# Quantco/tabmat

Measured on AMD Instinct MI355X. Metric: SplitMatrix.sandwich GFLOP/s + effective HBM GB/s, 10M×1k mixed, higher is better.
Workload: dtype f64; 1 GPU; SplitMatrix.sandwich: dense128 + csr512@5% + cats(256,96,32), 10000000 rows/GPU, p=1024, float64 (BASELINE configs[3]); rows_per_gpu=10000000, p=1024, launch=eager, collective=none

## Files before the change

include/tabmat_hip.h:

```cpp
#ifndef TABMAT_HIP_H
#define TABMAT_HIP_H

#include <stddef.h>
#include <stdint.h>

#ifdef __cplusplus
extern "C" {
#endif

#define TM_OK 0
#define TM_EINVAL (-1)
#define TM_ENOMEM (-2)
#define TM_EUNSUPPORTED (-3)

int tm_version(void);
const char *tm_last_error(void);
int tm_device_count(int *count);
int tm_set_device(int device);
int tm_device_info(char *name, int name_len, int *compute_units, int64_t *hbm_bytes);
int tm_malloc(void **ptr, size_t bytes);
int tm_free(void *ptr);
int tm_memcpy_h2d(void *dst, const void *h_src, size_t bytes, void *stream);
int tm_memcpy_d2h(void *h_dst, const void *src, size_t bytes, void *stream);
int tm_memset(void *dst, int value, size_t bytes, void *stream);
// ... 433 lines not shown
                                          int64_t n_sel, int64_t m, const double *d_sel, double *out,
                                          void *stream);
int tm_multi_cat_sparse_sandwich_rows_u8_f32(const void *const *h_codes, const int64_t *h_ncols,
                                             const int32_t *h_drop_first, int n_cats,
                                             const float *cm_data, const uint8_t *cm_col8,
                                             const int32_t *row_ranges, const int32_t *rows,
                                             int64_t n_sel, int64_t m, const float *d_sel, float *out,
                                             void *stream);
int tm_multi_cat_sparse_sandwich_rows_u8_f64(const void *const *h_codes, const int64_t *h_ncols,
                                             const int32_t *h_drop_first, int n_cats,
                                             const double *cm_data, const uint8_t *cm_col8,
                                             const int32_t *row_ranges, const int32_t *rows,
                                             int64_t n_sel, int64_t m, const double *d_sel, double *out,
                                             void *stream);
int tm_multi_cat_sparse_sandwich_ent_f32(const void *const *h_codes, const int64_t *h_ncols,
                                         const int32_t *h_drop_first, int n_cats, int64_t n, const float *d,
                                         const float *vals, const uint16_t *meta, const uint32_t *bstart,
                                         int64_t n_slots, int64_t mk, float *out, void *stream);
int tm_multi_cat_sparse_sandwich_ent_f64(const void *const *h_codes, const int64_t *h_ncols,
                                         const int32_t *h_drop_first, int n_cats, int64_t n, const double *d,
                                         const double *vals, const uint16_t *meta, const uint32_t *bstart,
                                         int64_t n_slots, int64_t mk, double *out, void *stream);
int tm_multi_cat_pack_codes(const void *const *h_codes, const int64_t *h_ncols, const int32_t *h_drop_first, int n_cats,
                            int64_t n, uint32_t *packed, void *stream);
int tm_multi_cat_sparse_sandwich_entp_f32(const void *const *h_codes, const int64_t *h_ncols,
                                          const int32_t *h_drop_first, int n_cats, int64_t n, const float *d,
                                          const float *vals, const uint16_t *meta, const uint32_t *bstart,
                                          int64_t n_slots, int64_t mk, const uint32_t *packed, float *out, void *stream);
int tm_multi_cat_sparse_sandwich_entp_f64(const void *const *h_codes, const int64_t *h_ncols,
                                          const int32_t *h_drop_first, int n_cats, int64_t n, const double *d,
                                          const double *vals, const uint16_t *meta, const uint32_t *bstart,
                                          int64_t n_slots, int64_t mk, const uint32_t *packed, double *out, void *stream);

int tm_multi_cat_sparse_sandwich_slab_f32(const void *const *h_codes, const int64_t *h_ncols,
                                          const int32_t *h_drop_first, int n_cats, int64_t n,
                                          const float *d, const float *vals, const uint32_t *koff,
                                          const uint8_t *ecol, const int64_t *gptr, int64_t m,
                                          float *out, void *stream);
int tm_multi_cat_sparse_sandwich_slab_f64(const void *const *h_codes, const int64_t *h_ncols,
                                          const int32_t *h_drop_first, int n_cats, int64_t n,
                                          const double *d, const double *vals, const uint32_t *koff,
                                          const uint8_t *ecol, const int64_t *gptr, int64_t m,
                                          double *out, void *stream);

int tm_multi_cat_pairs_max_bins(void);
int tm_multi_cat_pairs_max_slots(void);
int tm_multi_cat_pairs_row_words(void);
int tm_multi_cat_pairs_f32(const int64_t *cat_tab, int64_t n, const float *d, const int32_t *rows,
                           int64_t n_rows, const int32_t *bundles, int n_bundles,
                           const int32_t *wg_map, int n_wg, int slots, int64_t bins,
                           const int64_t *desc, int64_t n_pairs, const int64_t *pos, double *tables,
                           double *out, int64_t p, void *stream);
int tm_multi_cat_pairs_f64(const int64_t *cat_tab, int64_t n, const double *d, const int32_t *rows,
                           int64_t n_rows, const int32_t *bundles, int n_bundles,
                           const int32_t *wg_map, int n_wg, int slots, int64_t bins,
                           const int64_t *desc, int64_t n_pairs, const int64_t *pos, double *tables,
                           double *out, int64_t p, void *stream);

int tm_multi_cat_matvec_f32(const int64_t *cat_tab, int n_cats, const int64_t *pos, const float *v,
                            int64_t n, float *out, void *stream);
int tm_multi_cat_matvec_f64(const int64_t *cat_tab, int n_cats, const int64_t *pos, const double *v,
                            int64_t n, double *out, void *stream);

int tm_csr_densify_cols_f32(const float *data, const int32_t *indices, const int64_t *indptr, int64_t n,
                            const int32_t *colmap, float *T, int64_t ld, void *stream);
int tm_csr_densify_cols_f64(const double *data, const int32_t *indices, const int64_t *indptr, int64_t n,
                            const int32_t *colmap, double *T, int64_t ld, void *stream);
int tm_csc_densify_cols_f32(const int32_t *rows, const float *vals, const int64_t *seg, const int32_t *tcol,
                            int64_t n_sel, int64_t max_len, float *T, int64_t ld, void *stream);
int tm_csc_densify_cols_f64(const int32_t *rows, const double *vals, const int64_t *seg, const int32_t *tcol,
                            int64_t n_sel, int64_t max_len, double *T, int64_t ld, void *stream);
int tm_dense_gather_cols_f32(const float *X, int64_t n, int64_t m, int order_f, const int32_t *cols,
                             int64_t n_sel, float *T, int64_t ld, int64_t t0, void *stream);
int tm_dense_gather_cols_f64(const double *X, int64_t n, int64_t m, int order_f, const int32_t *cols,
                             int64_t n_sel, double *T, int64_t ld, int64_t t0, void *stream);

int tm_scatter_block_f32(const float *src, int64_t nr, int64_t nc, const int64_t *ri,
                         const int64_t *ci, double *out, int64_t p, int mirror, int diag,
                         void *stream);
int tm_scatter_block_f64(const double *src, int64_t nr, int64_t nc, const int64_t *ri,
                         const int64_t *ci, double *out, int64_t p, int mirror, int diag,
                         void *stream);

int tm_sparse_sandwich_chunked_rows_f32(const float *cm_data, const int32_t *cm_indices,
                                        const int32_t *row_ranges, int64_t n_sel, int64_t m,
                                        int64_t nnz, const float *d_sel, float *out, void *stream);
int tm_sparse_sandwich_chunked_rows_f64(const double *cm_data, const int32_t *cm_indices,
                                        const int32_t *row_ranges, int64_t n_sel, int64_t m,
                                        int64_t nnz, const double *d_sel, double *out, void *stream);

int tm_sparse_sandwich_chunked_u8_f32(const float *cm_data, const uint8_t *cm_col8, const int32_t *cptr, int64_t n,
                                      int64_t m, int64_t nnz, const float *d, float *out, void *stream);
int tm_sparse_sandwich_chunked_u8_f64(const double *cm_data, const uint8_t *cm_col8, const int32_t *cptr, int64_t n,
                                      int64_t m, int64_t nnz, const double *d, double *out, void *stream);
int tm_sparse_sandwich_chunked_rows_u8_f32(const float *cm_data, const uint8_t *cm_col8, const int32_t *row_ranges,
                                           int64_t n_sel, int64_t m, int64_t nnz, const float *d_sel, float *out,
                                           void *stream);
int tm_sparse_sandwich_chunked_rows_u8_f64(const double *cm_data, const uint8_t *cm_col8, const int32_t *row_ranges,
                                           int64_t n_sel, int64_t m, int64_t nnz, const double *d_sel, double *out,
                                           void *stream);
int tm_sparse_sandwich_direct_f32(const float *csr_data, const int32_t *csr_indices,
                                  const int64_t *csr_indptr, int64_t n, int64_t m, const float *d,
                                  float *out, void *stream);
int tm_sparse_sandwich_direct_f64(const double *csr_data, const int32_t *csr_indices,
                                  const int64_t *csr_indptr, int64_t n, int64_t m, const double *d,
                                  double *out, void *stream);
int tm_csr_dense_sandwich_rows_f32(const float *cm_data, const int32_t *cm_indices,
                                   const int32_t *row_ranges, int64_t n_sel, const int32_t *rows,
                                   const float *d_sel, int64_t n, int64_t m, const float *B, int64_t r,
                                   int order_f, float *out, void *stream);
int tm_csr_dense_sandwich_rows_f64(const double *cm_data, const int32_t *cm_indices,
                                   const int32_t *row_ranges, int64_t n_sel, const int32_t *rows,
                                   const double *d_sel, int64_t n, int64_t m, const double *B, int64_t r,
                                   int order_f, double *out, void *stream);
int tm_csr_dense_sandwich_rows_u8_f32(const float *cm_data, const uint8_t *cm_col8,
                                      const int32_t *row_ranges, int64_t n_sel, const int32_t *rows,
                                      const float *d_sel, int64_t n, int64_t m, const float *B, int64_t r,
                                      int order_f, float *out, void *stream);
int tm_csr_dense_sandwich_rows_u8_f64(const double *cm_data, const uint8_t *cm_col8,
                                      const int32_t *row_ranges, int64_t n_sel, const int32_t *rows,
                                      const double *d_sel, int64_t n, int64_t m, const double *B, int64_t r,
                                      int order_f, double *out, void *stream);

int tm_cat_det_block_rows(void);
int tm_cat_transpose_matvec_det_f32(const int32_t *perm, const int64_t *bstart, int64_t n_blocks,
                                    const int64_t *cat_bptr, int64_t n_cols, const float *v,
                                    float *out, int accumulate, void *stream);
int tm_cat_transpose_matvec_det_f64(const int32_t *perm, const int64_t *bstart, int64_t n_blocks,
                                    const int64_t *cat_bptr, int64_t n_cols, const double *v,
                                    double *out, int accumulate, void *stream);

int tm_cat_dense_sandwich_sorted_f32(const int32_t *perm, const int64_t *bstart, int64_t n_blocks,
                                     const int64_t *cat_bptr, int64_t n_cols, const float *d,
                                     const float *Y, int64_t m, float *out, void *stream);
int tm_cat_dense_sandwich_sorted_f64(const int32_t *perm, const int64_t *bstart, int64_t n_blocks,
                                     const int64_t *cat_bptr, int64_t n_cols, const double *d,
                                     const double *Y, int64_t m, double *out, void *stream);
int tm_csc_dense_sandwich_sorted_f32(const int32_t *rows, const float *vals, const int64_t *bstart,
                                     int64_t n_blocks, const int64_t *col_bptr, int64_t n_cols,
                                     const float *d, const float *Y, int64_t m, float *out,
                                     void *stream);
int tm_csc_dense_sandwich_sorted_f64(const int32_t *rows, const double *vals, const int64_t *bstart,
                                     int64_t n_blocks, const int64_t *col_bptr, int64_t n_cols,
                                     const double *d, const double *Y, int64_t m, double *out,
                                     void *stream);
int tm_cat_sparse_sandwich_sorted_f32(const int32_t *perm, const int64_t *bstart, int64_t n_blocks,
                                      const int64_t *cat_bptr, int64_t n_cols, const float *d,
                                      const float *csr_data, const int32_t *csr_indices,
                                      const int64_t *csr_indptr, int64_t m, float *out, void *stream);
int tm_cat_sparse_sandwich_sorted_f64(const int32_t *perm, const int64_t *bstart, int64_t n_blocks,
                                      const int64_t *cat_bptr, int64_t n_cols, const double *d,
                                      const double *csr_data, const int32_t *csr_indices,
                                      const int64_t *csr_indptr, int64_t m, double *out, void *stream);

int tm_csr_matvec_multi_f32(const float *csr_data, const int32_t *csr_indices,
                            const int64_t *csr_indptr, int64_t n, int64_t m, const float *V,
                            int64_t K, const int32_t *rows, int64_t n_rows, const int32_t *cols,
                            int64_t n_cols, float *out, void *stream);
int tm_csr_rmatvec_multi_f32(const float *csr_data, const int32_t *csr_indices,
                             const int64_t *csr_indptr, int64_t n, int64_t m, const float *V,
                             int64_t K, const int32_t *rows, int64_t n_rows, const int32_t *cols,
                             int64_t n_cols, float *out, void *stream);
int tm_dense_matvec_multi_f32(const float *X, int64_t n, int64_t m, int order_f, const float *V,
                              int64_t K, const int32_t *rows, int64_t n_rows, const int32_t *cols,
                              int64_t n_cols, float *out, void *stream);
int tm_dense_rmatvec_multi_f32(const float *X, int64_t n, int64_t m, int order_f, const float *V,
// ... 31 lines not shown
```

tabmat_amd/csrc/cat.hip:

```cpp
#include <algorithm>

#include "common.hpp"
#include "reduce.hpp"

namespace tmh {

__global__ void fill_i32_kernel(int32_t *p, int64_t n, int32_t v) {
    int64_t i = (int64_t)blockIdx.x * blockDim.x + threadIdx.x;
    if (i < n) p[i] = v;
}

__global__ void scatter_iota_i32_kernel(int32_t *map, const int32_t *cols, int64_t n_cols) {
    int64_t i = (int64_t)blockIdx.x * blockDim.x + threadIdx.x;
    if (i < n_cols) map[cols[i]] = (int32_t)i;
}

int build_col_map(int32_t *map, int64_t m, const int32_t *cols, int64_t n_cols, hipStream_t st) {
    if (m > 0) {
        hipLaunchKernelGGL(fill_i32_kernel, dim3((unsigned)ceil_div(m, 256)), dim3(256), 0, st, map,
                           m, -1);
        TM_LAUNCH_CHECK();
    }
    if (n_cols > 0) {
        hipLaunchKernelGGL(scatter_iota_i32_kernel, dim3((unsigned)ceil_div(n_cols, 256)),
                           dim3(256), 0, st, map, cols, n_cols);
        TM_LAUNCH_CHECK();
    }
    return TM_OK;
}

template <typename F, bool TWO>
__global__ __launch_bounds__(1024) void hist_lds_kernel(
    const int32_t *__restrict__ ci, const int32_t *__restrict__ cj, const F *__restrict__ w,
    const int32_t *__restrict__ rows, int64_t n_iter, int64_t rows_per_block, int drop_i,
    int drop_j, int i_ncol, int j_ncol, int ti, const int32_t *__restrict__ col_map,
    F *__restrict__ ws, int64_t stride) {
    extern __shared__ __attribute__((aligned(16))) unsigned char smem_raw[];
    lds_acc_t *bins = reinterpret_cast<lds_acc_t *>(smem_raw);
    const int part = blockIdx.y;
    const int i0 = part * ti;
    const int i1 = min(i0 + ti, i_ncol);
    const int nbins = TWO ? (i1 - i0) * j_ncol : (i1 - i0);
    for (int b = threadIdx.x; b < nbins; b += blockDim.x) bins[b] = 0.0;
    __syncthreads();

    const int64_t t0 = (int64_t)blockIdx.x * rows_per_block;
    const int64_t t1 = min(t0 + rows_per_block, n_iter);
    int64_t tbeg = t0;
    if (!TWO && rows == nullptr && (t0 & 3) == 0 &&
        ((reinterpret_cast<uintptr_t>(ci) | reinterpret_cast<uintptr_t>(w)) & 15) == 0) {
        typedef int i4 __attribute__((ext_vector_type(4)));
        const int64_t nvec = (t1 - t0) / 4;
        for (int64_t q = threadIdx.x; q < nvec; q += blockDim.x) {
            const int64_t k = t0 + q * 4;
            const i4 cc = *reinterpret_cast<const i4 *>(ci + k);
            F ww[4];
#pragma unroll
            for (int e = 0; e < 4; ++e) ww[e] = w[k + e];
#pragma unroll
            for (int e = 0; e < 4; ++e) {
                const int c = cc[e] - drop_i;
                if (c >= i0 && c < i1 && !(col_map && col_map[c] < 0)) atomic_add(&bins[c - i0], (lds_acc_t)ww[e]);
            }
        }
        tbeg = t0 + nvec * 4;
    }
    for (int64_t t = tbeg + threadIdx.x; t < t1; t += blockDim.x) {
        const int64_t k = rows ? (int64_t)rows[t] : t;
        const int c = ci[k] - drop_i;
        if (c < i0 || c >= i1) continue;
        if (TWO) {
            const int c2 = cj[k] - drop_j;
            if (c2 < 0) continue;
            atomic_add(&bins[(c - i0) * j_ncol + c2], (lds_acc_t)w[k]);
        } else {
            if (col_map && col_map[c] < 0) continue;
            atomic_add(&bins[c - i0], (lds_acc_t)w[k]);
        }
    }
    __syncthreads();
    F *dst = ws + ((int64_t)part * gridDim.x + blockIdx.x) * stride;
    for (int b = threadIdx.x; b < nbins; b += blockDim.x) dst[b] = (F)bins[b];
}

template <typename F, bool TWO>
__global__ __launch_bounds__(256) void hist_global_kernel(
// ... 1133 lines not shown
                process(p[j]);
                request(s + DEPTH + j, q[j], p[j]);
                request_bounds(s + 2 * DEPTH + j, q[j]);
            }
        }
    }
    __syncthreads();
    F *dst = ws + ((int64_t)blockIdx.y * gridDim.x + blockIdx.x) * stride;
    for (int b = threadIdx.x; b < cs.total * GC; b += blockDim.x)
        dst[b] = (F)tile[(b / GC) * TSTR + (b % GC)];
}

template <typename F, typename IX>
__global__ __launch_bounds__(1024) void multi_cat_sparse_rows_kernel(
    CatSet cs, const F *__restrict__ cm_data, const IX *__restrict__ cm_ind,
    const int32_t *__restrict__ ranges, const int32_t *__restrict__ rows, const F *__restrict__ d_sel,
    int64_t n_sel, int64_t rows_per_block, F *__restrict__ ws, int64_t stride) {
    constexpr int GC = 32;
    extern __shared__ __attribute__((aligned(16))) unsigned char smem_raw[];
    lds_acc_t *tile = reinterpret_cast<lds_acc_t *>(smem_raw);
    constexpr int tstr = GC + 1;
    const int nel = cs.total * tstr;
    for (int b = threadIdx.x; b < nel; b += blockDim.x) tile[b] = 0.0;
    __syncthreads();
    static_assert(SPARSE_CHUNK_COLS == 4 * GC, "the chunk of the chunk-major twin must hold four 32-column groups");
    const int g = blockIdx.y;
    const int ch = g >> 2;
    const int lane = threadIdx.x & 63, wave = threadIdx.x >> 6, nwave = blockDim.x >> 6;
    const int lr = lane >> 3, lt = lane & 7;
    const int64_t t0 = (int64_t)blockIdx.x * rows_per_block;
    const int64_t t1 = min(t0 + rows_per_block, n_sel);
    const int32_t *rg = ranges + (int64_t)ch * n_sel * 2;
    for (int64_t k0 = t0 + wave * 8; k0 < t1; k0 += (int64_t)nwave * 8) {
        const int64_t k = k0 + lr;
        if (k >= t1) continue;
        const F dk = d_sel[k];
        if (dk == F(0)) continue;
        const int e0 = rg[2 * k], e1 = rg[2 * k + 1];
        if (e0 >= e1) continue;
        const int64_t row = rows[k];
        int off[MAX_CATS];
#pragma unroll
        for (int c = 0; c < MAX_CATS; ++c) {
            off[c] = -1;
            if (c < cs.n_cats) {
                const int col = cs.codes[c][row] - cs.drop[c];
                off[c] = col >= 0 ? (cs.off[c] + col) * tstr : -1;
            }
        }
        for (int e = e0 + lt; e < e1; e += 8) {
            const int col = (int)cm_ind[e] - (sizeof(IX) == 1 ? (g & 3) : g) * GC;
            if (col < 0 || col >= GC) continue;
            const lds_acc_t x = (lds_acc_t)(dk * cm_data[e]);
#pragma unroll
            for (int c = 0; c < MAX_CATS; ++c)
                if (off[c] >= 0) atomic_add(&tile[off[c] + col], x);
        }
    }
    __syncthreads();
    F *dst = ws + ((int64_t)blockIdx.y * gridDim.x + blockIdx.x) * stride;
    for (int b = threadIdx.x; b < cs.total * GC; b += blockDim.x)
        dst[b] = (F)tile[(b / GC) * tstr + (b % GC)];
}

static int make_catset(const void *const *h_codes, const int64_t *h_ncols, const int32_t *h_drop,
                       int n_cats, CatSet *cs) {
    if (n_cats < 1 || n_cats > MAX_CATS) {
        set_error("multi-cat call supports 1..%d categoricals, got %d", MAX_CATS, n_cats);
        return TM_EINVAL;
    }
    int off = 0;
    for (int c = 0; c < MAX_CATS; ++c) {
        cs->codes[c] = c < n_cats ? reinterpret_cast<const int32_t *>(h_codes[c]) : nullptr;
        cs->ncol[c] = c < n_cats ? (int)h_ncols[c] : 0;
        cs->drop[c] = c < n_cats ? h_drop[c] : 0;
        cs->off[c] = off;
        off += cs->ncol[c];
    }
    cs->n_cats = n_cats;
    cs->total = off;
    return TM_OK;
}

template <typename F>
static int run_multi_cat_dense(const void *const *h_codes, const int64_t *h_ncols,
                               const int32_t *h_drop, int n_cats, int64_t n, const F *d, const F *M,
                               int64_t m, int order_f, F *out, hipStream_t st,
                               const int32_t *rows = nullptr, int64_t n_rows = 0) {
    CatSet cs;
    int rc = make_catset(h_codes, h_ncols, h_drop, n_cats, &cs);
    if (rc) return rc;
    const int64_t total = (int64_t)cs.total * m;
    if (total == 0) return TM_OK;
    if (rows != nullptr) n = n_rows;
    if (n == 0) {
        TM_HIP(hipMemsetAsync(out, 0, sizeof(F) * (size_t)total, st));
        return TM_OK;
    }
    {
        constexpr int VEC = MCW_VEC;
        constexpr int TJW = 16 * VEC;
        const size_t tile_b = ((sizeof(lds_acc_t) * (size_t)cs.total * TJW + 15) / 16) * 16;
        const size_t lds_w = tile_b + (size_t)16 * MCW_RS * (sizeof(F) + (size_t)n_cats * sizeof(int));
        if (!order_f && n_cats <= 8 && m >= VEC && m % VEC == 0 &&
            (reinterpret_cast<uintptr_t>(M) & 15) == 0 && lds_w <= 150 * 1024 &&
            (int64_t)cs.total * TJW * (int64_t)sizeof(lds_acc_t) < (1ll << 30)) {
            const int64_t n_parts = ceil_div(m, TJW);
            const int64_t stride = (int64_t)cs.total * TJW;
            int64_t nblk = std::max<int64_t>(1, tune("catdense_rounds", 1) * NUM_CU / n_parts);
            nblk = std::min<int64_t>(nblk, std::max<int64_t>(1, ceil_div(n, 4096)));
            const int64_t rpb = ceil_div(ceil_div(n, nblk), MCW_RS) * MCW_RS;
            nblk = ceil_div(n, rpb);
            const size_t tmp_bytes = ((sizeof(F) * (size_t)(n_parts * stride) + 255) / 256) * 256;
            void *wsv = nullptr;
            rc = get_workspace(tmp_bytes + sizeof(F) * (size_t)(n_parts * nblk * stride) + 256, &wsv, st);
            if (rc) return rc;
            F *tmp = reinterpret_cast<F *>(wsv);
            F *ws = reinterpret_cast<F *>(reinterpret_cast<char *>(wsv) + tmp_bytes);
            auto gow = [&](auto kern) -> int {
                TM_HIP(hipFuncSetAttribute(reinterpret_cast<const void *>(kern),
                                           hipFuncAttributeMaxDynamicSharedMemorySize, (int)lds_w));
                prof_begin(st);
                const int nw_dflt = (sizeof(F) == 8 && tile_b > 64 * 1024) ? 8 : 16;
                const int nw = (int)std::min<int64_t>(16, std::max<int64_t>(4, tune("catdense_waves", nw_dflt)));
                hipLaunchKernelGGL(kern, dim3((unsigned)nblk, (unsigned)n_parts), dim3(nw * 64), lds_w, st,
                                   cs, d, M, n, m, rpb, ws, stride, rows, wg_log_ptr());
                prof_end(st);
                TM_LAUNCH_CHECK();
                return TM_OK;
            };
            if (n_cats == 1) rc = gow(&multi_cat_dense_wide_kernel<F, 1>);
            else if (n_cats == 2) rc = gow(&multi_cat_dense_wide_kernel<F, 2>);
            else if (n_cats == 3) rc = gow(&multi_cat_dense_wide_kernel<F, 3>);
            else if (n_cats == 4) rc = gow(&multi_cat_dense_wide_kernel<F, 4>);
            else if (n_cats == 5) rc = gow(&multi_cat_dense_wide_kernel<F, 5>);
            else if (n_cats == 6) rc = gow(&multi_cat_dense_wide_kernel<F, 6>);
            else if (n_cats == 7) rc = gow(&multi_cat_dense_wide_kernel<F, 7>);
            else rc = gow(&multi_cat_dense_wide_kernel<F, 8>);
            if (rc) return rc;
            rc = launch_reduce_partials<F>(ws, stride, (int)nblk, (int)n_parts, tmp, n_parts * stride,
                                           false, st);
            if (rc) return rc;
            hipLaunchKernelGGL((multi_cat_untile_kernel<F>), dim3((unsigned)ceil_div(total, 256)),
                               dim3(256), 0, st, tmp, (int64_t)cs.total, m, TJW, out);
            TM_LAUNCH_CHECK();
            return TM_OK;
        }
    }
    if (rows != nullptr) {
        set_error("multi_cat_dense: the row-list form needs the wide-load path");
        return TM_EUNSUPPORTED;
    }
    int TJ = 64;
    while (TJ > 1 && sizeof(lds_acc_t) * (size_t)cs.total * TJ > HIST_LDS_MAX) TJ >>= 1;
    while (TJ > 1 && TJ / 2 >= m) TJ >>= 1;
    if (sizeof(lds_acc_t) * (size_t)cs.total * TJ > HIST_LDS_MAX) {
        set_error("multi_cat_dense: %d stacked categories exceed the LDS tile", cs.total);
        return TM_EUNSUPPORTED;
    }
    const int64_t n_parts = ceil_div(m, TJ);
    const int64_t stride = (int64_t)cs.total * TJ;
    const size_t lds = sizeof(lds_acc_t) * (size_t)stride;
    int64_t nblk = std::max<int64_t>(1, NUM_CU / n_parts);
    nblk = std::min<int64_t>(nblk, std::max<int64_t>(1, ceil_div(n, 4096)));
    const int64_t rpb = ceil_div(n, nblk);
    nblk = ceil_div(n, rpb);
    const size_t tmp_bytes = ((sizeof(F) * (size_t)(n_parts * stride) + 255) / 256) * 256;
    void *wsv = nullptr;
    rc = get_workspace(tmp_bytes + sizeof(F) * (size_t)(n_parts * nblk * stride) + 256, &wsv, st);
    if (rc) return rc;
    F *tmp = reinterpret_cast<F *>(wsv);
    F *ws = reinterpret_cast<F *>(reinterpret_cast<char *>(wsv) + tmp_bytes);
    auto go = [&](auto kern) -> int {
        if (lds > 48 * 1024)
            TM_HIP(hipFuncSetAttribute(reinterpret_cast<const void *>(kern),
                                       hipFuncAttributeMaxDynamicSharedMemorySize, (int)lds));
        prof_begin(st);
        hipLaunchKernelGGL(kern, dim3((unsigned)nblk, (unsigned)n_parts), dim3(1024), lds, st, cs, d,
                           M, n, m, rpb, ws, stride);
        prof_end(st);
        TM_LAUNCH_CHECK();
        return TM_OK;
    };
#define TM_MCD_CASE(V)                                                                       \
    case V:                                                                                  \
        if (order_f) rc = go(&multi_cat_dense_f_kernel<F, V>);                               \
        else if (n_cats == 1) rc = go(&multi_cat_dense_c_kernel<F, V, 1>);                   \
        else if (n_cats == 2) rc = go(&multi_cat_dense_c_kernel<F, V, 2>);                   \
        else if (n_cats == 3) rc = go(&multi_cat_dense_c_kernel<F, V, 3>);                   \
        else if (n_cats == 4) rc = go(&multi_cat_dense_c_kernel<F, V, 4>);                   \
        else rc = go(&multi_cat_dense_c_kernel<F, V, 0>);                                    \
        break;
    switch (TJ) {
        TM_MCD_CASE(64)
        TM_MCD_CASE(32)
        TM_MCD_CASE(16)
        TM_MCD_CASE(8)
        TM_MCD_CASE(4)
        TM_MCD_CASE(2)
        TM_MCD_CASE(1)
        default:
            rc = TM_EINVAL;
    }
#undef TM_MCD_CASE
    if (rc) return rc;
    rc = launch_reduce_partials<F>(ws, stride, (int)nblk, (int)n_parts, tmp, n_parts * stride, false,
                                   st);
    if (rc) return rc;
    hipLaunchKernelGGL((multi_cat_untile_kernel<F>), dim3((unsigned)ceil_div(total, 256)),
                       dim3(256), 0, st, tmp, (int64_t)cs.total, m, TJ, out);
    TM_LAUNCH_CHECK();
    return TM_OK;
}

template <typename F, typename IX>
static int run_multi_cat_sparse_rows(const void *const *h_codes, const int64_t *h_ncols,
                                     const int32_t *h_drop, int n_cats, const F *cm_data,
                                     const IX *cm_ind, const int32_t *ranges, const int32_t *rows,
                                     int64_t n_sel, int64_t m, const F *d_sel, F *out, hipStream_t st);

template <typename F>
static int run_multi_cat_sparse(const void *const *h_codes, const int64_t *h_ncols,
                                const int32_t *h_drop, int n_cats, int64_t n, const F *d,
                                const F *vals, const unsigned *koff, const unsigned char *ecol,
                                const int64_t *gptr, int64_t m, int slab_rows, int group_cols,
                                F *out, hipStream_t st) {
    CatSet cs;
    int rc = make_catset(h_codes, h_ncols, h_drop, n_cats, &cs);
    if (rc) return rc;
    const int64_t total = (int64_t)cs.total * m;
    if (total == 0) return TM_OK;
    if (n == 0) {
        TM_HIP(hipMemsetAsync(out, 0, sizeof(F) * (size_t)total, st));
        return TM_OK;
    }
    const int64_t stride = (int64_t)cs.total * group_cols;
    const size_t tile_bytes = ((sizeof(lds_acc_t) * (size_t)cs.total * (group_cols + 1) + 15) / 16) * 16;
    if (tile_bytes > HIST_LDS_MAX) {
        set_error("multi_cat_sparse: %d stacked categories exceed the LDS tile", cs.total);
        return TM_EUNSUPPORTED;
    }
    const int nw = (int)std::min<int64_t>(16, std::max<int64_t>(4, tune("catsparse_waves", 16)));
    const size_t stage_bytes = (size_t)nw * slab_rows * (sizeof(F) + sizeof(int32_t) * (size_t)n_cats);
    const bool stage = tile_bytes + stage_bytes <= 150 * 1024;
    const size_t lds = tile_bytes + (stage ? stage_bytes : 0);
    const int n_groups = (int)ceil_div(m, group_cols);
    const int64_t n_slabs = ceil_div(n, slab_rows);
    int64_t nblk = std::max<int64_t>(1, tune("catsparse_rounds", 1) * NUM_CU / n_groups);
    nblk = std::min<int64_t>(nblk, n_slabs);
    const int64_t spb = ceil_div(n_slabs, nblk);
    nblk = ceil_div(n_slabs, spb);
    const size_t tmp_bytes = ((sizeof(F) * (size_t)(n_groups * stride) + 255) / 256) * 256;
    void *wsv = nullptr;
    rc = get_workspace(tmp_bytes + sizeof(F) * (size_t)((int64_t)n_groups * nblk * stride) + 256,
                       &wsv, st);
    if (rc) return rc;
    F *tmp = reinterpret_cast<F *>(wsv);
    F *ws = reinterpret_cast<F *>(reinterpret_cast<char *>(wsv) + tmp_bytes);
    if (stage && n_cats <= 8 && slab_rows == 128) {
        auto kpf = n_cats == 1   ? &multi_cat_sparse_pf_kernel<F, 1>
                   : n_cats == 2 ? &multi_cat_sparse_pf_kernel<F, 2>
                   : n_cats == 3 ? &multi_cat_sparse_pf_kernel<F, 3>
                   : n_cats == 4 ? &multi_cat_sparse_pf_kernel<F, 4>
                   : n_cats == 5 ? &multi_cat_sparse_pf_kernel<F, 5>
                   : n_cats == 6 ? &multi_cat_sparse_pf_kernel<F, 6>
                   : n_cats == 7 ? &multi_cat_sparse_pf_kernel<F, 7>
                                 : &multi_cat_sparse_pf_kernel<F, 8>;
        if (lds > 48 * 1024)
            TM_HIP(hipFuncSetAttribute(reinterpret_cast<const void *>(kpf),
                                       hipFuncAttributeMaxDynamicSharedMemorySize, (int)lds));
        prof_begin(st);
        hipLaunchKernelGGL(kpf, dim3((unsigned)nblk, (unsigned)n_groups), dim3(nw * 64), lds, st, cs, d,
                           vals, koff, ecol, gptr, n_groups, n_slabs, spb, group_cols, n, ws, stride,
                           wg_log_ptr());
        prof_end(st);
        TM_LAUNCH_CHECK();
    } else {
        auto kern = stage ? &multi_cat_sparse_kernel<F, true> : &multi_cat_sparse_kernel<F, false>;
        if (lds > 48 * 1024)
            TM_HIP(hipFuncSetAttribute(reinterpret_cast<const void *>(kern),
                                       hipFuncAttributeMaxDynamicSharedMemorySize, (int)lds));
        prof_begin(st);
        hipLaunchKernelGGL(kern, dim3((unsigned)nblk, (unsigned)n_groups), dim3(nw * 64), lds, st, cs,
                           d, vals, koff, ecol, gptr, n_groups, n_slabs, spb, slab_rows, group_cols,
                           n, ws, stride);
        prof_end(st);
        TM_LAUNCH_CHECK();
    }
    rc = launch_reduce_partials<F>(ws, stride, (int)nblk, n_groups, tmp,
                                   (int64_t)n_groups * stride, false, st);
    if (rc) return rc;
    hipLaunchKernelGGL((multi_cat_untile_kernel<F>), dim3((unsigned)ceil_div(total, 256)),
                       dim3(256), 0, st, tmp, (int64_t)cs.total, m, group_cols, out);
    TM_LAUNCH_CHECK();
    return TM_OK;
}

__global__ __launch_bounds__(256) void multi_cat_pack_codes_kernel(CatSet cs, int64_t n, unsigned *__restrict__ out) {
    for (int64_t r = (int64_t)blockIdx.x * blockDim.x + threadIdx.x; r < n; r += (int64_t)gridDim.x * blockDim.x) {
        unsigned pk = 0u;
#pragma unroll
        for (int c = 0; c < 3; ++c) {
            unsigned f = 1023u;
            if (c < cs.n_cats) {
                const int col = cs.codes[c][r] - cs.drop[c];
                if (col >= 0 && col < cs.ncol[c]) f = (unsigned)(cs.off[c] + col);
            }
            pk |= f << (10 * c);
        }
        out[r] = pk;
    }
}

template <typename F>
static int run_multi_cat_sparse_ent(const void *const *h_codes, const int64_t *h_ncols, const int32_t *h_drop,
                                    int n_cats, int64_t n, const F *d, const F *vals, const unsigned short *meta,
                                    const unsigned *bstart, int64_t mk, F *out, hipStream_t st,
                                    const unsigned *packed = nullptr, int64_t n_slots = 0) {
    CatSet cs;
    int rc = make_catset(h_codes, h_ncols, h_drop, n_cats, &cs);
    if (rc) return rc;
    const int64_t total = (int64_t)cs.total * mk;
    if (total == 0) return TM_OK;
    if (n == 0) {
        TM_HIP(hipMemsetAsync(out, 0, sizeof(F) * (size_t)total, st));
        return TM_OK;
    }
    TM_REQUIRE(mk % 16 == 0 && n_cats >= 1 && n_cats <= 8, "kernel columns in groups of 16, 1 .. 8 categoricals");
    TM_REQUIRE(n < (1ll << 28), "at most 2^28 - 1 rows per block");
    constexpr int GC = 32;
    const int64_t stride = (int64_t)cs.total * GC;
    const size_t lds = ((sizeof(lds_acc_t) * (size_t)cs.total * (GC + 1) + 15) / 16) * 16;
    if (lds > HIST_LDS_MAX) {
        set_error("multi_cat_sparse_ent: %d stacked categories exceed the LDS tile", cs.total);
        return TM_EUNSUPPORTED;
    }
    const int nw = (int)std::min<int64_t>(16, std::max<int64_t>(4, tune("catsparse_waves", 16)));
    const int n_groups = (int)(mk / 16);
    const int n_pairs = (n_groups + 1) / 2;
    const int64_t n_slabs = ceil_div(n, 64);
    int64_t nblk = std::max<int64_t>(1, tune("catsparse_rounds", 1) * NUM_CU / n_pairs);
    nblk = std::min<int64_t>(nblk, n_slabs);
    const int64_t spb = ceil_div(n_slabs, nblk);
    nblk = ceil_div(n_slabs, spb);
    const size_t tmp_bytes = ((sizeof(F) * (size_t)(n_pairs * stride) + 255) / 256) * 256;
    void *wsv = nullptr;
    rc = get_workspace(tmp_bytes + sizeof(F) * (size_t)((int64_t)n_pairs * nblk * stride) + 256, &wsv, st);
    if (rc) return rc;
    F *tmp = reinterpret_cast<F *>(wsv);
    F *ws = reinterpret_cast<F *>(reinterpret_cast<char *>(wsv) + tmp_bytes);
    auto kern = n_cats == 1   ? &multi_cat_sparse_ent_kernel<F, 1>
                : n_cats == 2 ? &multi_cat_sparse_ent_kernel<F, 2>
                : n_cats == 3 ? &multi_cat_sparse_ent_kernel<F, 3>
                : n_cats == 4 ? &multi_cat_sparse_ent_kernel<F, 4>
                : n_cats == 5 ? &multi_cat_sparse_ent_kernel<F, 5>
                : n_cats == 6 ? &multi_cat_sparse_ent_kernel<F, 6>
                : n_cats == 7 ? &multi_cat_sparse_ent_kernel<F, 7>
                              : &multi_cat_sparse_ent_kernel<F, 8>;
    TM_REQUIRE(packed == nullptr || (n_cats <= 3 && cs.total < 1023), "packed codes: at most 3 categoricals, 1022 levels");
    const int ncw = packed != nullptr ? 1 : n_cats;
    const size_t lds_staged = lds + (size_t)nw * 64 * (sizeof(F) + 4 * (size_t)ncw);
    const double fill = (double)n_slots / ((double)std::max(n_groups, 1) * (double)n_slabs);
    if (tune("catsparse_staged", 1) != 0 && lds_staged <= 156 * 1024 &&
        fill >= (double)tune("catsparse_staged_fill", 44)) {
        using KS = void (*)(CatSet, const F *, const F *, const unsigned short *, const unsigned *, int, int64_t, int64_t,
                            int64_t, F *, int64_t, const unsigned *, int);
        KS ks = nullptr;
        if (packed != nullptr) {
            ks = n_cats == 1 ? &multi_cat_sparse_ent_staged_kernel<F, 1, true>
                 : n_cats == 2 ? &multi_cat_sparse_ent_staged_kernel<F, 2, true>
                               : &multi_cat_sparse_ent_staged_kernel<F, 3, true>;
        } else {
            ks = n_cats == 1   ? &multi_cat_sparse_ent_staged_kernel<F, 1, false>
                 : n_cats == 2 ? &multi_cat_sparse_ent_staged_kernel<F, 2, false>
                 : n_cats == 3 ? &multi_cat_sparse_ent_staged_kernel<F, 3, false>
                 : n_cats == 4 ? &multi_cat_sparse_ent_staged_kernel<F, 4, false>
                 : n_cats == 5 ? &multi_cat_sparse_ent_staged_kernel<F, 5, false>
                 : n_cats == 6 ? &multi_cat_sparse_ent_staged_kernel<F, 6, false>
                 : n_cats == 7 ? &multi_cat_sparse_ent_staged_kernel<F, 7, false>
                               : &multi_cat_sparse_ent_staged_kernel<F, 8, false>;
        }
        if (lds_staged > 48 * 1024)
            TM_HIP(hipFuncSetAttribute(reinterpret_cast<const void *>(ks),
                                       hipFuncAttributeMaxDynamicSharedMemorySize, (int)lds_staged));
        prof_begin(st);
        hipLaunchKernelGGL(ks, dim3((unsigned)nblk, (unsigned)n_pairs), dim3(nw * 64), lds_staged, st, cs, d, vals,
                           meta, bstart, n_groups, n, n_slabs, spb, ws, stride, packed, (int)lds);
        prof_end(st);
        TM_LAUNCH_CHECK();
    } else {
        if (lds > 48 * 1024)
            TM_HIP(hipFuncSetAttribute(reinterpret_cast<const void *>(kern),
                                       hipFuncAttributeMaxDynamicSharedMemorySize, (int)lds));
        prof_begin(st);
        hipLaunchKernelGGL(kern, dim3((unsigned)nblk, (unsigned)n_pairs), dim3(nw * 64), lds, st, cs, d, vals, meta,
                           bstart, n_groups, n, n_slabs, spb, ws, stride, packed);
        prof_end(st);
        TM_LAUNCH_CHECK();
    }
    rc = launch_reduce_partials<F>(ws, stride, (int)nblk, n_pairs, tmp, (int64_t)n_pairs * stride, false, st);
    if (rc) return rc;
    hipLaunchKernelGGL((multi_cat_untile_kernel<F>), dim3((unsigned)ceil_div(total, 256)), dim3(256), 0, st, tmp,
                       (int64_t)cs.total, mk, GC, out);
    TM_LAUNCH_CHECK();
    return TM_OK;
}

}

using namespace tmh;

#define TM_CHECK_COMMON(nn) \
    TM_REQUIRE((nn) >= 0, "negative size")

extern "C" {

int tm_cat_transpose_matvec_f32(const int32_t *codes, int64_t n, int64_t n_cols, int drop_first,
                                const float *v, const int32_t *rows, int64_t n_rows,
                                const int32_t *cols, int64_t n_cols_sel, float *out, void *stream) {
    TM_CHECK_COMMON(n);
    return run_cat_tmv<float>(codes, n, n_cols, drop_first, v, rows, n_rows, cols, n_cols_sel, out,
                              as_stream(stream));
}
int tm_cat_transpose_matvec_f64(const int32_t *codes, int64_t n, int64_t n_cols, int drop_first,
                                const double *v, const int32_t *rows, int64_t n_rows,
                                const int32_t *cols, int64_t n_cols_sel, double *out,
                                void *stream) {
    TM_CHECK_COMMON(n);
    return run_cat_tmv<double>(codes, n, n_cols, drop_first, v, rows, n_rows, cols, n_cols_sel,
                               out, as_stream(stream));
}

int tm_cat_matvec_f32(const int32_t *codes, int64_t n, int64_t n_cols, int drop_first,
                      const float *v, const int32_t *cols, int64_t n_cols_sel, float *out,
                      void *stream) {
    TM_CHECK_COMMON(n);
    return run_cat_matvec<float>(codes, n, n_cols, drop_first, v, cols, n_cols_sel, out,
                                 as_stream(stream));
}
int tm_cat_matvec_f64(const int32_t *codes, int64_t n, int64_t n_cols, int drop_first,
                      const double *v, const int32_t *cols, int64_t n_cols_sel, double *out,
                      void *stream) {
    TM_CHECK_COMMON(n);
    return run_cat_matvec<double>(codes, n, n_cols, drop_first, v, cols, n_cols_sel, out,
                                  as_stream(stream));
}

int tm_cat_matvec_assign_f32(const int32_t *codes, int64_t n, int64_t n_cols, int drop_first,
                             const float *v, const int32_t *cols, int64_t n_cols_sel, float *out,
                             void *stream) {
    TM_CHECK_COMMON(n);
    return run_cat_matvec<float>(codes, n, n_cols, drop_first, v, cols, n_cols_sel, out,
                                 as_stream(stream), true);
}
int tm_cat_matvec_assign_f64(const int32_t *codes, int64_t n, int64_t n_cols, int drop_first,
                             const double *v, const int32_t *cols, int64_t n_cols_sel, double *out,
                             void *stream) {
    TM_CHECK_COMMON(n);
    return run_cat_matvec<double>(codes, n, n_cols, drop_first, v, cols, n_cols_sel, out,
                                  as_stream(stream), true);
}

int tm_cat_cat_sandwich_f32(const int32_t *i_codes, const int32_t *j_codes, int64_t n,
                            const float *d, const int32_t *rows, int64_t n_rows, int64_t i_ncol,
                            int64_t j_ncol, int i_drop_first, int j_drop_first, float *out,
                            void *stream) {
    TM_CHECK_COMMON(n);
    return run_hist<float, true>(i_codes, j_codes, d, rows, rows ? n_rows : n, i_drop_first,
                                 j_drop_first, i_ncol, j_ncol, nullptr, out, false,
                                 as_stream(stream));
}
int tm_cat_cat_sandwich_f64(const int32_t *i_codes, const int32_t *j_codes, int64_t n,
                            const double *d, const int32_t *rows, int64_t n_rows, int64_t i_ncol,
                            int64_t j_ncol, int i_drop_first, int j_drop_first, double *out,
                            void *stream) {
    TM_CHECK_COMMON(n);
    return run_hist<double, true>(i_codes, j_codes, d, rows, rows ? n_rows : n, i_drop_first,
                                  j_drop_first, i_ncol, j_ncol, nullptr, out, false,
                                  as_stream(stream));
}

int tm_cat_cat_sandwich_atomic_f32(const int32_t *i_codes, const int32_t *j_codes, int64_t n,
                                   const float *d, const int32_t *rows, int64_t n_rows, int64_t i_ncol,
                                   int64_t j_ncol, int i_drop_first, int j_drop_first, float *out,
                                   void *stream) {
    TM_CHECK_COMMON(n);
    return run_hist<float, true>(i_codes, j_codes, d, rows, rows ? n_rows : n, i_drop_first,
                                 j_drop_first, i_ncol, j_ncol, nullptr, out, false,
                                 as_stream(stream), 12);
}
int tm_cat_cat_sandwich_atomic_f64(const int32_t *i_codes, const int32_t *j_codes, int64_t n,
                                   const double *d, const int32_t *rows, int64_t n_rows, int64_t i_ncol,
                                   int64_t j_ncol, int i_drop_first, int j_drop_first, double *out,
                                   void *stream) {
    TM_CHECK_COMMON(n);
    return run_hist<double, true>(i_codes, j_codes, d, rows, rows ? n_rows : n, i_drop_first,
                                  j_drop_first, i_ncol, j_ncol, nullptr, out, false,
                                  as_stream(stream), 12);
}

int tm_cat_cat_sandwich_sorted_f32(const int32_t *ci_sorted, const int32_t *cj_sorted, const int32_t *perm,
                                   const int64_t *lptr, int64_t n_sorted, const float *d, int64_t i_ncol,
                                   int64_t j_ncol, float *out, void *stream) {
    TM_CHECK_COMMON(n_sorted);
    return run_hist_sorted<float>(ci_sorted, cj_sorted, perm, lptr, n_sorted, d, i_ncol, j_ncol, out,
                                  as_stream(stream));
}
int tm_cat_cat_sandwich_sorted_f64(const int32_t *ci_sorted, const int32_t *cj_sorted, const int32_t *perm,
                                   const int64_t *lptr, int64_t n_sorted, const double *d, int64_t i_ncol,
                                   int64_t j_ncol, double *out, void *stream) {
    TM_CHECK_COMMON(n_sorted);
    return run_hist_sorted<double>(ci_sorted, cj_sorted, perm, lptr, n_sorted, d, i_ncol, j_ncol, out,
                                   as_stream(stream));
}

int tm_cat_dense_sandwich_f32(const int32_t *codes, int64_t n, int64_t i_ncol, int drop_first,
                              const float *d, const int32_t *rows, int64_t n_rows, const float *M,
                              int64_t M_ncol, int order_f, const int32_t *j_cols, int64_t n_j,
                              float *out, void *stream) {
    TM_CHECK_COMMON(n);
    return run_cat_dense<float>(codes, n, i_ncol, drop_first, d, rows, n_rows, M, M_ncol, order_f,
                                j_cols, j_cols ? n_j : M_ncol, out, as_stream(stream));
}
int tm_cat_dense_sandwich_f64(const int32_t *codes, int64_t n, int64_t i_ncol, int drop_first,
                              const double *d, const int32_t *rows, int64_t n_rows,
                              const double *M, int64_t M_ncol, int order_f, const int32_t *j_cols,
                              int64_t n_j, double *out, void *stream) {
    TM_CHECK_COMMON(n);
    return run_cat_dense<double>(codes, n, i_ncol, drop_first, d, rows, n_rows, M, M_ncol, order_f,
                                 j_cols, j_cols ? n_j : M_ncol, out, as_stream(stream));
}

int tm_cat_sparse_sandwich_f32(const int32_t *codes, int64_t n, int64_t i_ncol, int drop_first,
                               const float *csr_data, const int32_t *csr_indices,
                               const int64_t *csr_indptr, int64_t s_ncol, const float *d,
                               const int32_t *rows, int64_t n_rows, const int32_t *cols,
                               int64_t n_cols, float *out, void *stream) {
    TM_CHECK_COMMON(n);
    return run_cat_sparse<float>(codes, n, i_ncol, drop_first, csr_data, csr_indices, csr_indptr,
                                 s_ncol, d, rows, n_rows, cols, n_cols, out, as_stream(stream));
}
int tm_cat_sparse_sandwich_f64(const int32_t *codes, int64_t n, int64_t i_ncol, int drop_first,
                               const double *csr_data, const int32_t *csr_indices,
                               const int64_t *csr_indptr, int64_t s_ncol, const double *d,
                               const int32_t *rows, int64_t n_rows, const int32_t *cols,
                               int64_t n_cols, double *out, void *stream) {
    TM_CHECK_COMMON(n);
    return run_cat_sparse<double>(codes, n, i_ncol, drop_first, csr_data, csr_indices, csr_indptr,
                                  s_ncol, d, rows, n_rows, cols, n_cols, out, as_stream(stream));
}

int tm_multi_cat_dense_sandwich_f32(const void *const *h_codes, const int64_t *h_ncols,
                                    const int32_t *h_drop_first, int n_cats, int64_t n,
                                    const float *d, const float *M, int64_t M_ncol, int order_f,
                                    float *out, void *stream) {
    return run_multi_cat_dense<float>(h_codes, h_ncols, h_drop_first, n_cats, n, d, M, M_ncol,
                                      order_f, out, as_stream(stream));
}
int tm_multi_cat_dense_sandwich_f64(const void *const *h_codes, const int64_t *h_ncols,
                                    const int32_t *h_drop_first, int n_cats, int64_t n,
                                    const double *d, const double *M, int64_t M_ncol, int order_f,
                                    double *out, void *stream) {
    return run_multi_cat_dense<double>(h_codes, h_ncols, h_drop_first, n_cats, n, d, M, M_ncol,
                                       order_f, out, as_stream(stream));
}
int tm_multi_cat_dense_sandwich_rows_f32(const void *const *h_codes, const int64_t *h_ncols,
                                         const int32_t *h_drop_first, int n_cats, int64_t n,
                                         const float *d, const float *M, int64_t M_ncol,
                                         const int32_t *rows, int64_t n_rows, float *out,
                                         void *stream) {
    return run_multi_cat_dense<float>(h_codes, h_ncols, h_drop_first, n_cats, n, d, M, M_ncol, 0, out,
                                      as_stream(stream), rows, n_rows);
}
int tm_multi_cat_dense_sandwich_rows_f64(const void *const *h_codes, const int64_t *h_ncols,
                                         const int32_t *h_drop_first, int n_cats, int64_t n,
                                         const double *d, const double *M, int64_t M_ncol,
                                         const int32_t *rows, int64_t n_rows, double *out,
                                         void *stream) {
    return run_multi_cat_dense<double>(h_codes, h_ncols, h_drop_first, n_cats, n, d, M, M_ncol, 0, out,
                                       as_stream(stream), rows, n_rows);
}
int tm_multi_cat_sparse_sandwich_ent_f32(const void *const *h_codes, const int64_t *h_ncols,
                                         const int32_t *h_drop_first, int n_cats, int64_t n, const float *d,
                                         const float *vals, const uint16_t *meta, const uint32_t *bstart,
                                         int64_t n_slots, int64_t mk, float *out, void *stream) {
    return run_multi_cat_sparse_ent<float>(h_codes, h_ncols, h_drop_first, n_cats, n, d, vals, meta, bstart, mk,
                                           out, as_stream(stream), nullptr, n_slots);
}
int tm_multi_cat_sparse_sandwich_ent_f64(const void *const *h_codes, const int64_t *h_ncols,
                                         const int32_t *h_drop_first, int n_cats, int64_t n, const double *d,
                                         const double *vals, const uint16_t *meta, const uint32_t *bstart,
                                         int64_t n_slots, int64_t mk, double *out, void *stream) {
    return run_multi_cat_sparse_ent<double>(h_codes, h_ncols, h_drop_first, n_cats, n, d, vals, meta, bstart, mk,
                                            out, as_stream(stream), nullptr, n_slots);
}
int tm_multi_cat_pack_codes(const void *const *h_codes, const int64_t *h_ncols, const int32_t *h_drop_first, int n_cats,
                            int64_t n, uint32_t *packed, void *stream) {
    CatSet cs;
    int rc = make_catset(h_codes, h_ncols, h_drop_first, n_cats, &cs);
    if (rc) return rc;
    TM_REQUIRE(n_cats <= 3 && cs.total < 1023, "packed codes: at most 3 categoricals, 1022 stacked levels");
    if (n == 0) return TM_OK;
    hipLaunchKernelGGL(multi_cat_pack_codes_kernel, dim3((unsigned)std::min<int64_t>(4 * NUM_CU, ceil_div(n, 256))),
                       dim3(256), 0, as_stream(stream), cs, n, packed);
    TM_LAUNCH_CHECK();
    return TM_OK;
}
int tm_multi_cat_sparse_sandwich_entp_f32(const void *const *h_codes, const int64_t *h_ncols,
                                          const int32_t *h_drop_first, int n_cats, int64_t n, const float *d,
                                          const float *vals, const uint16_t *meta, const uint32_t *bstart,
                                          int64_t n_slots, int64_t mk, const uint32_t *packed, float *out, void *stream) {
    return run_multi_cat_sparse_ent<float>(h_codes, h_ncols, h_drop_first, n_cats, n, d, vals, meta, bstart, mk, out,
                                           as_stream(stream), packed, n_slots);
}
int tm_multi_cat_sparse_sandwich_entp_f64(const void *const *h_codes, const int64_t *h_ncols,
                                          const int32_t *h_drop_first, int n_cats, int64_t n, const double *d,
                                          const double *vals, const uint16_t *meta, const uint32_t *bstart,
                                          int64_t n_slots, int64_t mk, const uint32_t *packed, double *out, void *stream) {
    return run_multi_cat_sparse_ent<double>(h_codes, h_ncols, h_drop_first, n_cats, n, d, vals, meta, bstart, mk,
                                            out, as_stream(stream), packed, n_slots);
}
int tm_multi_cat_sparse_sandwich_slab_f32(const void *const *h_codes, const int64_t *h_ncols,
                                          const int32_t *h_drop_first, int n_cats, int64_t n,
                                          const float *d, const float *vals, const uint32_t *koff,
                                          const uint8_t *ecol, const int64_t *gptr, int64_t m,
                                          float *out, void *stream) {
    return run_multi_cat_sparse<float>(h_codes, h_ncols, h_drop_first, n_cats, n, d, vals, koff,
                                       ecol, gptr, m, tm_slab_rows(), tm_slab_group_cols(), out,
                                       as_stream(stream));
}
int tm_multi_cat_sparse_sandwich_slab_f64(const void *const *h_codes, const int64_t *h_ncols,
                                          const int32_t *h_drop_first, int n_cats, int64_t n,
                                          const double *d, const double *vals, const uint32_t *koff,
                                          const uint8_t *ecol, const int64_t *gptr, int64_t m,
                                          double *out, void *stream) {
    return run_multi_cat_sparse<double>(h_codes, h_ncols, h_drop_first, n_cats, n, d, vals, koff,
                                        ecol, gptr, m, tm_slab_rows(), tm_slab_group_cols(), out,
                                        as_stream(stream));
}

}

namespace tmh {
template <typename F, typename IX>
static int run_multi_cat_sparse_rows(const void *const *h_codes, const int64_t *h_ncols,
                                     const int32_t *h_drop, int n_cats, const F *cm_data,
                                     const IX *cm_ind, const int32_t *ranges, const int32_t *rows,
// ... 89 lines not shown
```

tabmat_amd/csrc/sparse_blocks.hip:

```cpp
#include <algorithm>

#include "common.hpp"
#include "reduce.hpp"

namespace tmh {

constexpr int KB_WAVES = 16;
constexpr int KB_TS = 128;

template <typename F>
__global__ void blocks_assemble_kernel(const F *__restrict__ tiles, int n_out, F *__restrict__ out) {
    const int j = blockIdx.x * blockDim.x + threadIdx.x;
    const int i = blockIdx.y;
    if (i >= n_out || j >= n_out) return;
    const int hi = max(i, j), lo = min(i, j);
    const int I = hi / KB_TS, J = lo / KB_TS;
    const int part = I * (I + 1) / 2 + J;
    out[(int64_t)i * n_out + j] = tiles[(int64_t)part * KB_TS * KB_TS + (hi % KB_TS) * KB_TS + (lo % KB_TS)];
}

constexpr int KB_FLAG_REP_A = 1 << 16;
constexpr int KB_FLAG_REP_B = 1 << 17;

template <typename F, bool U8, bool D12 = false>
__global__ __launch_bounds__(KB_WAVES * 64) void sparse_sandwich_blocks_kernel(
    const F *__restrict__ data, const int32_t *__restrict__ ind, const int32_t *__restrict__ cptr,
    int64_t n, int64_t nnz1, const int32_t *__restrict__ blocks, const int4 *__restrict__ wg_tab,
    const F *__restrict__ d, int max_nb, F *__restrict__ ws, WgLogBuf *__restrict__ wglog) {
    constexpr int TS = KB_TS;
    const unsigned long long t_begin = wg_log_begin(wglog);
    extern __shared__ __attribute__((aligned(16))) unsigned char smem_raw[];
    lds_acc_t *tile = reinterpret_cast<lds_acc_t *>(smem_raw);
    const int4 w = wg_tab[2 * blockIdx.x], x = wg_tab[2 * blockIdx.x + 1];
    const int part = __builtin_amdgcn_readfirstlane(w.x), slot = __builtin_amdgcn_readfirstlane(w.y);
    const int b0 = __builtin_amdgcn_readfirstlane(w.z), b1 = __builtin_amdgcn_readfirstlane(w.w);
    const int bfull = __builtin_amdgcn_readfirstlane(x.x);
    int wfull = __builtin_amdgcn_readfirstlane(x.y);
    {
        const int nwv = (int)(blockDim.x >> 6);
        if (nwv != KB_WAVES) {
            wfull = (wfull * nwv + KB_WAVES / 2) / KB_WAVES;
            if (bfull > b0) wfull = max(wfull, 1);
            if (b1 > bfull) wfull = min(wfull, nwv - 1);
            if (bfull == b0) wfull = 0;
            if (b1 == bfull) wfull = nwv;
        }
    }
    int I = (int)((sqrtf(8.0f * (float)part + 1.0f) - 1.0f) * 0.5f);
    while ((I + 1) * (I + 2) / 2 <= part) ++I;
    while (I * (I + 1) / 2 > part) --I;
    const int J = part - I * (I + 1) / 2;
    const int i0 = I * TS, j0 = J * TS;
    for (int b = threadIdx.x; b < TS * TS; b += blockDim.x) tile[b] = 0.0;
    __syncthreads();

    const int lane = threadIdx.x & 63;
    const int wave = __builtin_amdgcn_readfirstlane(threadIdx.x >> 6);
    const int lr = lane >> 3, lt = lane & 7;
    if (b1 > b0) {
        const int row_first = __builtin_amdgcn_readfirstlane(x.z), row_last = __builtin_amdgcn_readfirstlane(x.w);
        const int32_t *cpA = cptr + (int64_t)I * (n + 1), *cpB = cptr + (int64_t)J * (n + 1);
        const int baseA = __builtin_amdgcn_readfirstlane(cpA[row_first]);
        const int baseB = __builtin_amdgcn_readfirstlane(cpB[row_first]);
        const unsigned spanA1 = (unsigned)max(__builtin_amdgcn_readfirstlane(cpA[row_last + 1]) - baseA - 1, 0);
        const unsigned spanB1 = (unsigned)max(__builtin_amdgcn_readfirstlane(cpB[row_last + 1]) - baseB - 1, 0);
        const F *dataA = data + min((int64_t)baseA, nnz1), *dataB = data + min((int64_t)baseB, nnz1);
        const int32_t *indA = ind + min((int64_t)baseA, nnz1), *indB = ind + min((int64_t)baseB, nnz1);
        const unsigned char *ind8 = reinterpret_cast<const unsigned char *>(ind);
        const unsigned char *ind8A = ind8 + min((int64_t)baseA, nnz1), *ind8B = ind8 + min((int64_t)baseB, nnz1);
        const int i0c = U8 ? 0 : i0, j0c = U8 ? 0 : j0;
        const unsigned nrow1 = (unsigned)max(n - 1, (int64_t)0);
        auto ldi = [](const int32_t *base, unsigned i) {
            return *reinterpret_cast<const int32_t *>(reinterpret_cast<const char *>(base) + (i << 2));
        };
        auto ldf = [](const F *base, unsigned i) {
            return *reinterpret_cast<const F *>(reinterpret_cast<const char *>(base) + (i * (unsigned)sizeof(F)));
        };
        constexpr int SH = 3;
        constexpr int BIGKEY = 0x7ffffff0;
        char *const tile_bytes = reinterpret_cast<char *>(tile);
        auto add_pair = [&](int kb, int la, int ba, F prod) {
            if (kb <= la)
                atomic_add(reinterpret_cast<lds_acc_t *>(tile_bytes + (unsigned)(kb ^ ba)), (lds_acc_t)prod);
        };

        auto run_list = [&](auto diag_c, auto full_c, int s0, int s1, int w0, int nw) {
            constexpr bool DIAG = decltype(diag_c)::value;
            constexpr bool FULL = decltype(full_c)::value;
            constexpr int offmask = DIAG ? 0 : 0x70000000;
            const int nseg = s1 - s0;
            if (nseg <= 0) return;
            constexpr int DW = D12 ? 3 : 4;
            const int32_t *blk = blocks + (int64_t)s0 * DW;
            struct Dsc { int4 q; bool valid; };
            struct Grp { int nA, nB, ta, tb; F d, va, vb; int ca, cb; };
            auto load_desc = [&](int g) {
                Dsc r;
                const int k = g + lr;
                r.valid = k < nseg;
                const unsigned kc = (unsigned)min(k, nseg - 1);
                if constexpr (D12) {
                    const int32_t *b = reinterpret_cast<const int32_t *>(reinterpret_cast<const char *>(blk) + kc * 12u);
// ... 15 lines not shown
                e.nB = on ? ((sd.q.w >> 8) & 0xff) : 0;
                e.ta = (!FULL && (sd.q.w & KB_FLAG_REP_A)) ? (lt & 3) : lt;
                e.tb = (!FULL && (sd.q.w & KB_FLAG_REP_B)) ? (lt & 3) : lt;
                const unsigned iA = min((unsigned)(sd.q.x - baseA) + min((unsigned)e.ta, (unsigned)max(e.nA - 1, 0)), spanA1);
                const unsigned iB = min((unsigned)(sd.q.y - baseB) + min((unsigned)e.tb, (unsigned)max(e.nB - 1, 0)), spanB1);
#ifdef KB_ABL_WRAP
                const unsigned iAw = iA & (unsigned)(KB_ABL_WRAP), iBw = iB & (unsigned)(KB_ABL_WRAP);
                e.ca = ldi(indA, min(iAw, spanA1));
                e.va = ldf(dataA, min(iAw, spanA1));
                e.cb = ldi(indB, min(iBw, spanB1));
                e.vb = ldf(dataB, min(iBw, spanB1));
                return e;
#endif
                e.ca = U8 ? (int)ind8A[iA] : ldi(indA, iA);
                e.va = ldf(dataA, iA);
                e.cb = U8 ? (int)ind8B[iB] : ldi(indB, iB);
                e.vb = ldf(dataB, iB);
                return e;
            };
            auto process = [&](const Grp &cur) {
                __builtin_amdgcn_s_setprio(1);
                const int colA = cur.ta < cur.nA ? cur.ca - i0c : -1;
                const int colB = cur.tb < cur.nB ? cur.cb - j0c : -1;
                const int la = (colA < 0 ? -8 : colA << SH) | offmask;
                const int ba = (int)(((unsigned)colA << (7 + SH)) | ((colA & 15) << (3 + SH)));
                const int kb = colB < 0 ? BIGKEY : colB << SH;
                const F av = cur.va * cur.d, vb = cur.vb;
                add_pair(kb, la, ba, av * vb);
                add_pair(dpp_xor_i32<1>(kb), la, ba, av * dpp_xor<1>(vb));
                add_pair(dpp_xor_i32<2>(kb), la, ba, av * dpp_xor<2>(vb));
                add_pair(dpp_xor_i32<3>(kb), la, ba, av * dpp_xor<3>(vb));
#ifndef KB_ABL_HALFSTEPS
                if constexpr (FULL) {
                    const int kb4 = dpp_xor_i32<4>(kb);
                    const F vb4 = dpp_xor<4>(vb);
                    add_pair(kb4, la, ba, av * vb4);
                    add_pair(dpp_xor_i32<1>(kb4), la, ba, av * dpp_xor<1>(vb4));
                    add_pair(dpp_xor_i32<2>(kb4), la, ba, av * dpp_xor<2>(vb4));
                    add_pair(dpp_xor_i32<3>(kb4), la, ba, av * dpp_xor<3>(vb4));
                }
#endif
                __builtin_amdgcn_s_setprio(0);
            };
            const int gstep = nw * 8;
            const int gw = (wave - w0) * 8;
            Grp ea[2], eb[2];
            Dsc ps[2];
            ea[0] = load_entries(load_desc(gw));
            ea[1] = load_entries(load_desc(gw + gstep));
            ps[0] = load_desc(gw + 2 * gstep);
            ps[1] = load_desc(gw + 3 * gstep);
            for (int g = gw; g < nseg; g += 4 * gstep) {
                eb[0] = load_entries(ps[0]);
                eb[1] = load_entries(ps[1]);
                ps[0] = load_desc(g + 4 * gstep);
                ps[1] = load_desc(g + 5 * gstep);
                process(ea[0]);
                if (g + gstep < nseg) process(ea[1]);
                if (g + 2 * gstep >= nseg) break;
                ea[0] = load_entries(ps[0]);
                ea[1] = load_entries(ps[1]);
                ps[0] = load_desc(g + 6 * gstep);
                ps[1] = load_desc(g + 7 * gstep);
                process(eb[0]);
                if (g + 3 * gstep < nseg) process(eb[1]);
            }
        };
        auto run_tile = [&](auto diag_c) {
            if (wave < wfull) run_list(diag_c, std::true_type{}, b0, bfull, 0, wfull);
            else run_list(diag_c, std::false_type{}, bfull, b1, wfull, (int)(blockDim.x >> 6) - wfull);
        };
        if (I == J) run_tile(std::true_type{});
        else run_tile(std::false_type{});
    }
    __syncthreads();
    if (threadIdx.x == 0) wg_log_end(wglog, t_begin, WG_K2);
    F *dst = ws + ((int64_t)part * max_nb + slot) * (TS * TS);
    for (int b = threadIdx.x; b < TS * TS; b += blockDim.x) {
        const int r = b / TS, c = b % TS;
        dst[b] = (F)tile[r * TS + (c ^ ((r & 15) << 3))];
    }
}

template <typename F, bool U8 = false, bool D12 = false>
static int run_sparse_sandwich_blocks(const F *data, const int32_t *ind, const int32_t *cptr, int64_t n,
                                      int64_t m, int64_t nnz, const int32_t *blocks, const int32_t *wg_tab,
                                      int n_wg, int max_nb, const F *d, F *out, hipStream_t st) {
    if (m == 0) return TM_OK;
    if (n == 0 || nnz == 0 || n_wg == 0) {
        TM_HIP(hipMemsetAsync(out, 0, sizeof(F) * (size_t)(m * m), st));
        return TM_OK;
    }
    constexpr int TS = KB_TS;
    const int nchunk = (int)ceil_div(m, TS);
    const int n_parts = nchunk * (nchunk + 1) / 2;
    TM_REQUIRE(nnz < (1ll << 31) && n < (1ll << 29), "sparse block too large for the block-list sandwich");
    TM_REQUIRE(!D12 || n < (1ll << 24), "12-byte block descriptors hold 24 bits of row");
    TM_REQUIRE(max_nb >= 1 && n_wg >= 1, "empty workgroup table");
    const size_t lds = sizeof(lds_acc_t) * (size_t)(TS * TS);
    const size_t tmp_bytes = (sizeof(F) * (size_t)n_parts * TS * TS + 255) / 256 * 256;
    const size_t ws_bytes = sizeof(F) * (size_t)n_parts * (size_t)max_nb * TS * TS;
    void *wsv = nullptr;
    int rc = get_workspace(tmp_bytes + ws_bytes + 256, &wsv, st);
    if (rc) return rc;
    F *tmp = reinterpret_cast<F *>(wsv);
    F *ws = reinterpret_cast<F *>(reinterpret_cast<char *>(wsv) + tmp_bytes);
    TM_HIP(hipMemsetAsync(ws, 0, ws_bytes, st));
    auto kern = &sparse_sandwich_blocks_kernel<F, U8, D12>;
    TM_HIP(hipFuncSetAttribute(reinterpret_cast<const void *>(kern),
                               hipFuncAttributeMaxDynamicSharedMemorySize, (int)lds));
    prof_begin(st);
    const int kb_waves = (int)std::min<int64_t>(KB_WAVES, std::max<int64_t>(2, tune("k2b_waves", KB_WAVES)));
    hipLaunchKernelGGL(kern, dim3((unsigned)n_wg), dim3(kb_waves * 64), lds, st, data, ind, cptr, n, nnz - 1,
                       blocks, reinterpret_cast<const int4 *>(wg_tab), d,
                       max_nb, ws, wg_log_ptr());
    prof_end(st);
    TM_LAUNCH_CHECK();
    rc = launch_reduce_partials<F>(ws, (int64_t)TS * TS, max_nb, n_parts, tmp, (int64_t)n_parts * TS * TS,
                                   false, st);
    if (rc) return rc;
    hipLaunchKernelGGL((blocks_assemble_kernel<F>), dim3((unsigned)ceil_div(m, 64), (unsigned)m), dim3(64),
                       0, st, tmp, (int)m, out);
    TM_LAUNCH_CHECK();
    return TM_OK;
}

}

extern "C" {

int tm_sparse_sandwich_blocks_f32(const float *cm_data, const int32_t *cm_indices, const int32_t *cptr,
                                  int64_t n, int64_t m, int64_t nnz, const int32_t *blocks,
                                  const int32_t *wg_tab, int n_wg, int max_nb, const float *d, float *out,
                                  void *stream) {
    return tmh::run_sparse_sandwich_blocks<float>(cm_data, cm_indices, cptr, n, m, nnz, blocks, wg_tab, n_wg,
                                                  max_nb, d, out, tmh::as_stream(stream));
}
int tm_sparse_sandwich_blocks_f64(const double *cm_data, const int32_t *cm_indices, const int32_t *cptr,
                                  int64_t n, int64_t m, int64_t nnz, const int32_t *blocks,
                                  const int32_t *wg_tab, int n_wg, int max_nb, const double *d, double *out,
                                  void *stream) {
    return tmh::run_sparse_sandwich_blocks<double>(cm_data, cm_indices, cptr, n, m, nnz, blocks, wg_tab, n_wg,
                                                   max_nb, d, out, tmh::as_stream(stream));
}

int tm_sparse_sandwich_blocks_u8_f32(const float *cm_data, const uint8_t *cm_col8, const int32_t *cptr,
                                     int64_t n, int64_t m, int64_t nnz, const int32_t *blocks,
                                     const int32_t *wg_tab, int n_wg, int max_nb, const float *d, float *out,
                                     void *stream) {
    return tmh::run_sparse_sandwich_blocks<float, true>(cm_data, reinterpret_cast<const int32_t *>(cm_col8), cptr, n, m,
                                                        nnz, blocks, wg_tab, n_wg, max_nb, d, out,
                                                        tmh::as_stream(stream));
}
int tm_sparse_sandwich_blocks_u8_f64(const double *cm_data, const uint8_t *cm_col8, const int32_t *cptr,
                                     int64_t n, int64_t m, int64_t nnz, const int32_t *blocks,
                                     const int32_t *wg_tab, int n_wg, int max_nb, const double *d, double *out,
                                     void *stream) {
    return tmh::run_sparse_sandwich_blocks<double, true>(cm_data, reinterpret_cast<const int32_t *>(cm_col8), cptr, n, m,
                                                         nnz, blocks, wg_tab, n_wg, max_nb, d, out,
                                                         tmh::as_stream(stream));
}

int tm_sparse_sandwich_blocks_p12_f32(const float *cm_data, const uint8_t *cm_col8, const int32_t *cptr,
                                      int64_t n, int64_t m, int64_t nnz, const int32_t *blocks12,
                                      const int32_t *wg_tab, int n_wg, int max_nb, const float *d, float *out,
                                      void *stream) {
    return tmh::run_sparse_sandwich_blocks<float, true, true>(cm_data, reinterpret_cast<const int32_t *>(cm_col8), cptr,
                                                              n, m, nnz, blocks12, wg_tab, n_wg, max_nb, d, out,
                                                              tmh::as_stream(stream));
}
int tm_sparse_sandwich_blocks_p12_f64(const double *cm_data, const uint8_t *cm_col8, const int32_t *cptr,
                                      int64_t n, int64_t m, int64_t nnz, const int32_t *blocks12,
                                      const int32_t *wg_tab, int n_wg, int max_nb, const double *d, double *out,
                                      void *stream) {
    return tmh::run_sparse_sandwich_blocks<double, true, true>(cm_data, reinterpret_cast<const int32_t *>(cm_col8), cptr,
                                                               n, m, nnz, blocks12, wg_tab, n_wg, max_nb, d, out,
                                                               tmh::as_stream(stream));
}

}
```

tabmat_amd/csrc/sparse_ent.hip:

```cpp
#include "common.hpp"
#include "reduce.hpp"

namespace tmh {

constexpr int EN_R = 64;
constexpr int EN_C = 16;
constexpr int EN_NW = 16;
constexpr int EN_THREADS = EN_NW * 64;
constexpr int EN_W = 128;
constexpr int EN_B = 16;
constexpr int EN_SB = 64;

template <typename F>
struct EnLds {
    static constexpr int ROWB = EN_W * (int)sizeof(F);
    static constexpr int SLABB = EN_R * ROWB;
    static constexpr int SCR_OFF = ROWB + 2 * SLABB;
    static constexpr int CS_OFF = SCR_OFF + EN_NW * EN_SB * 16;
    static constexpr int TOTAL = CS_OFF + EN_NW * EN_C * (int)sizeof(double);
};

constexpr int EN_CVGPR = 24;
#define EN_LD "40"

#if defined(__HIP_DEVICE_COMPILE__)
typedef __amdgpu_buffer_rsrc_t en_rsrc_t;
__device__ __forceinline__ en_rsrc_t en_rsrc(const void *base, int64_t bytes) {
    const unsigned nb = bytes <= 0 ? 0u : (bytes > 0xFFFFFFFFll ? 0xFFFFFFFFu : (unsigned)bytes);
    return __builtin_amdgcn_make_buffer_rsrc(const_cast<void *>(base), 0, (int)nb, 0x00020000);
}
__device__ __forceinline__ void en_buf_to_lds16(en_rsrc_t rs, void *lds, int voff, int soff) {
    __builtin_amdgcn_raw_ptr_buffer_load_lds(rs, (__attribute__((address_space(3))) void *)lds, 16, voff,
                                             soff, 0, 0);
}
template <typename F>
__device__ __forceinline__ void en_zero_acc() {
    if constexpr (sizeof(F) == 8) {
        static_for<16>([&](auto jc) {
            asm volatile("v_mov_b32 v[64+4*%0], 0\n\tv_mov_b32 v[64+4*%0+1], 0\n\t"
                         "v_mov_b32 v[64+4*%0+2], 0\n\tv_mov_b32 v[64+4*%0+3], 0"
                         :: "n"(decltype(jc)::value) : "v127");
        });
    } else {
        static_for<16>([&](auto jc) {
            asm volatile("v_mov_b32 v[64+2*%0], 0\n\tv_mov_b32 v[64+2*%0+1], 0" :: "n"(decltype(jc)::value) : "v95");
        });
    }
}
template <int K>
__device__ __forceinline__ unsigned en_read_acc() {
    unsigned x;
    asm volatile("v_mov_b32 %0, v[64+%1]" : "=v"(x) : "n"(K));
    return x;
}
template <typename F>
__device__ __forceinline__ void en_load_stream(unsigned voff_v, const F *vp, unsigned voff_m, const unsigned short *mp) {
    if constexpr (sizeof(F) == 8)
        asm volatile("global_load_dwordx2 v[" EN_LD ":" EN_LD "+1], %0, %1\n\t"
                     "global_load_ushort v[" EN_LD "+2], %2, %3" :: "v"(voff_v), "s"(vp), "v"(voff_m), "s"(mp) : "memory");
    else
        asm volatile("global_load_dword v[" EN_LD "], %0, %1\n\t"
                     "global_load_ushort v[" EN_LD "+2], %2, %3" :: "v"(voff_v), "s"(vp), "v"(voff_m), "s"(mp) : "memory");
}
template <typename F>
__device__ __forceinline__ void en_load_d(unsigned voff, const F *dp) {
    if constexpr (sizeof(F) == 8)
        asm volatile("global_load_dwordx2 v[" EN_LD "+4:" EN_LD "+5], %0, %1" :: "v"(voff), "s"(dp) : "memory");
    else
        asm volatile("global_load_dword v[" EN_LD "+4], %0, %1" :: "v"(voff), "s"(dp) : "memory");
}
template <int N>
__device__ __forceinline__ void en_take(double &v, unsigned &m, double &dd) {
    unsigned vl, vh, dl, dh;
    asm volatile("s_waitcnt vmcnt(%5)\n\t"
                 "v_mov_b32 %0, v[" EN_LD "]\n\tv_mov_b32 %1, v[" EN_LD "+1]\n\tv_mov_b32 %2, v[" EN_LD "+2]\n\t"
                 "v_mov_b32 %3, v[" EN_LD "+4]\n\tv_mov_b32 %4, v[" EN_LD "+5]"
                 : "=v"(vl), "=v"(vh), "=v"(m), "=v"(dl), "=v"(dh) : "n"(N) : "memory");
    v = __hiloint2double((int)vh, (int)vl);
    dd = __hiloint2double((int)dh, (int)dl);
}
template <int N>
__device__ __forceinline__ void en_take(float &v, unsigned &m, float &dd) {
    unsigned vl, dl;
    asm volatile("s_waitcnt vmcnt(%3)\n\t"
// ... 176 lines not shown
        if (lsince == 0) asm volatile("s_waitcnt vmcnt(0) lgkmcnt(0)" EN_BAR ::: "memory");
        else if (lsince == 3) asm volatile("s_waitcnt vmcnt(3) lgkmcnt(0)" EN_BAR ::: "memory");
        else asm volatile("s_waitcnt vmcnt(6) lgkmcnt(0)" EN_BAR ::: "memory");
#endif
        EN_TICK(pt_bar)
        ncopied = 0;
        ++w;
    };
    u4 enext = u4{0u, 0u, 0u, 0u};
    for (int b = 0; b < nbw; ++b) {
        const int q = b & 3;
        u4 e;
        if (q == 0) {
            boundary(b >> 2);
            e = scratch[l16];
        } else {
            e = enext;
        }
        if (q != 3) enext = scratch[(q + 1) * EN_B + l16];
        EN_TICK(pt_a)
        const int slab = __builtin_amdgcn_readlane((int)e[3], 1);
        while (w < slab) end_slab();
        if (ncopied == 0 && w + 1 < ns) {
            issue_pieces((w & 1) ^ 1, 0, NV);

            ncopied = NV;
            psince += NV;
            lsince = 0;
        }
        EN_TICK(pt_p)
        F a;
        if constexpr (sizeof(F) == 8) a = __hiloint2double((int)e[1], (int)e[0]);
        else a = __uint_as_float(e[0]);
#if defined(EN_ABL_NOBATCH)
        asm volatile("" ::"v"(a), "v"(e[2]), "v"(e[3]));
#else
        const unsigned live = (unsigned)__builtin_amdgcn_ballot_w64(a != F(0)) & 0xffffu;
        const int nq = live ? ((31 - __builtin_clz(live)) >> 2) + 1 : 0;
        unsigned p0 = (unsigned)__builtin_amdgcn_readlane((int)e[3], 0);
        unsigned p1 = (unsigned)__builtin_amdgcn_readlane((int)e[3], 4);
        unsigned p2 = (unsigned)__builtin_amdgcn_readlane((int)e[3], 8);
        unsigned p3 = (unsigned)__builtin_amdgcn_readlane((int)e[3], 12);
        if (nq == 4) en_batch_asm<16, F>(p0, p1, p2, p3, a, e[2], lane_off);
        else if (nq == 3) en_batch_asm<12, F>(p0, p1, p2, p3, a, e[2], lane_off);
        else if (nq == 2) en_batch_asm<8, F>(p0, p1, p2, p3, a, e[2], lane_off);
        else if (nq == 1) en_batch_asm<4, F>(p0, p1, p2, p3, a, e[2], lane_off);
#endif
        EN_TICK(pt_x)
#if defined(EN_PROF)
        ++pt_n;
#endif
    }
    while (w < ns) end_slab();
    wait_loads(std::integral_constant<int, 0>{});
#if defined(EN_PROF)
    if (prof != nullptr && lane == 0) {
        long long *o = prof + (((int64_t)blockIdx.z * gridDim.y + blockIdx.y) * gridDim.x + blockIdx.x) * (EN_NW * 8) + wave * 8;
        o[0] = pt_a; o[1] = pt_p; o[2] = pt_x; o[3] = pt_b; o[4] = pt_bar; o[5] = pt_n; o[6] = clock64() - pt_start; o[7] = ns;
    }
#endif

    if (active) {
        F *dst = ws + (((int64_t)blockIdx.y * gridDim.x + blockIdx.x) * n_groups + group) * (EN_C * EN_W);
        static_for<EN_C>([&](auto jc) {
            constexpr int j = decltype(jc)::value;
            if constexpr (sizeof(F) == 8) {
                const u4 o = u4{en_read_acc<4 * j>(), en_read_acc<4 * j + 1>(), en_read_acc<4 * j + 2>(),
                                en_read_acc<4 * j + 3>()};
                *reinterpret_cast<u4 *>(dst + j * EN_W + 2 * lane) = o;
            } else {
                typedef unsigned u2 __attribute__((ext_vector_type(2)));
                const u2 o = u2{en_read_acc<2 * j>(), en_read_acc<2 * j + 1>()};
                *reinterpret_cast<u2 *>(dst + j * EN_W + 2 * lane) = o;
            }
        });
        if constexpr (CSUM) {
            if (blockIdx.y == 0 && lane < EN_C)
                ws_csum[(int64_t)blockIdx.x * (n_groups * EN_C) + group * EN_C + lane] = (F)cs_lds[lane];
        }
    }
}

template <typename F>
__global__ void en_untile_kernel(const F *__restrict__ tmp, int64_t m, int64_t nB, F *__restrict__ out) {
    const int64_t e = (int64_t)blockIdx.x * blockDim.x + threadIdx.x;
    if (e >= m * nB) return;
    const int64_t i = e / nB, j = e % nB;
    out[e] = tmp[((j / EN_W) * m + i) * EN_W + (j % EN_W)];
}

template <typename F>
__global__ void en_csum_kernel(const F *__restrict__ part, int nblk, int64_t m, F *__restrict__ csum) {
    const int64_t c = (int64_t)blockIdx.x * blockDim.x + threadIdx.x;
    if (c >= m) return;
    double a = 0.0;
    for (int b = 0; b < nblk; ++b) a += (double)part[(int64_t)b * m + c];
    csum[c] = (F)a;
}

template <typename F>
static int run_csr_dense_ent(const F *vals, const uint16_t *meta, const uint32_t *bstart, int64_t n, int64_t m,
                             const F *B, int64_t r, const F *d, F *out, F *colsum, hipStream_t st) {
    const int64_t nB = r;
    const int64_t total = m * nB;
    if (total == 0) return TM_OK;
    constexpr int VEC = 16 / (int)sizeof(F);
    if ((reinterpret_cast<uintptr_t>(B) & 15) != 0 || r % VEC != 0 || nB < VEC) {
        set_error("tm_csr_dense_sandwich_ent: B must be C-ordered with 16-byte aligned rows");
        return TM_EUNSUPPORTED;
    }
    if (m % EN_C != 0) {
        set_error("tm_csr_dense_sandwich_ent: m must be a multiple of tm_ent_group_cols()");
        return TM_EINVAL;
    }
    if (n >= (1ll << 28)) {
        set_error("tm_csr_dense_sandwich_ent: at most 2^28 - 1 rows per block (work in row parts)");
        return TM_EUNSUPPORTED;
    }
    const int64_t n_slabs = ceil_div(n, EN_R);
    const int n_groups = (int)(m / EN_C);
    const int n_parts = (int)ceil_div(nB, EN_W);
    const int nz = (int)ceil_div(n_groups, EN_NW);
    const bool want_csum = colsum != nullptr;
    if (n_slabs == 0) {
        TM_HIP(hipMemsetAsync(out, 0, sizeof(F) * (size_t)total, st));
        if (want_csum) TM_HIP(hipMemsetAsync(colsum, 0, sizeof(F) * (size_t)m, st));
        return TM_OK;
    }
    int64_t nblk = std::max<int64_t>(1, tune("ent_rounds", 1) * NUM_CU / ((int64_t)n_parts * nz));
    nblk = std::min<int64_t>(nblk, n_slabs);
    const int64_t spb = ceil_div(n_slabs, nblk);
    nblk = ceil_div(n_slabs, spb);
    const int64_t stride = m * EN_W;
    const size_t tmp_bytes = (sizeof(F) * (size_t)(n_parts * stride) + 255) / 256 * 256;
    const size_t part_bytes = (sizeof(F) * (size_t)((int64_t)n_parts * nblk * stride) + 255) / 256 * 256;
    const size_t csum_bytes = ((want_csum ? sizeof(F) * (size_t)(nblk * m) : 0) + 255) / 256 * 256 + 256;
    void *wsv = nullptr;
    int rc = get_workspace(tmp_bytes + part_bytes + csum_bytes + 256, &wsv, st);
    if (rc) return rc;
    F *tmp = reinterpret_cast<F *>(wsv);
    F *ws = reinterpret_cast<F *>(reinterpret_cast<char *>(wsv) + tmp_bytes);
    F *ws_csum = reinterpret_cast<F *>(reinterpret_cast<char *>(wsv) + tmp_bytes + part_bytes);
    const size_t lds = (size_t)EnLds<F>::TOTAL;
    auto kern = want_csum ? &csr_dense_ent_kernel<F, true> : &csr_dense_ent_kernel<F, false>;
    TM_HIP(hipFuncSetAttribute(reinterpret_cast<const void *>(kern),
                               hipFuncAttributeMaxDynamicSharedMemorySize, (int)lds));
    prof_begin(st);
    hipLaunchKernelGGL(kern, dim3((unsigned)nblk, (unsigned)n_parts, (unsigned)nz), dim3(EN_THREADS), lds, st,
                       vals, meta, bstart, n_groups, n_slabs, spb, B, n, r, (int)nB, d, ws, ws_csum,
                       reinterpret_cast<long long *>((uintptr_t)tune("ent_prof", 0)));
    prof_end(st);
    TM_LAUNCH_CHECK();
    rc = launch_reduce_partials<F>(ws, stride, (int)nblk, n_parts, tmp, n_parts * stride, false, st);
    if (rc) return rc;
    hipLaunchKernelGGL((en_untile_kernel<F>), dim3((unsigned)ceil_div(total, 256)), dim3(256), 0, st, tmp, m,
                       nB, out);
    TM_LAUNCH_CHECK();
    if (want_csum) {
        hipLaunchKernelGGL((en_csum_kernel<F>), dim3((unsigned)ceil_div(m, 256)), dim3(256), 0, st, ws_csum,
                           (int)nblk, m, colsum);
        TM_LAUNCH_CHECK();
    }
    return TM_OK;
}

}

extern "C" {
int tm_ent_rows(void) { return tmh::EN_R; }
int tm_ent_group_cols(void) { return tmh::EN_C; }
int tm_ent_batch_slots(void) { return tmh::EN_B; }

int tm_csr_dense_sandwich_ent_f32(const float *vals, const uint16_t *meta, const uint32_t *bstart, int64_t n,
                                  int64_t m, const float *B, int64_t r, const float *d, float *out,
                                  float *colsum, void *stream) {
    return tmh::run_csr_dense_ent<float>(vals, meta, bstart, n, m, B, r, d, out, colsum, tmh::as_stream(stream));
}
int tm_csr_dense_sandwich_ent_f64(const double *vals, const uint16_t *meta, const uint32_t *bstart, int64_t n,
                                  int64_t m, const double *B, int64_t r, const double *d, double *out,
                                  double *colsum, void *stream) {
    return tmh::run_csr_dense_ent<double>(vals, meta, bstart, n, m, B, r, d, out, colsum, tmh::as_stream(stream));
}
}
```

tabmat_amd/ext/_types.py:

```python
from __future__ import annotations

import os
from dataclasses import dataclass

import numpy as np
import torch

from .. import _device as D


@dataclass
class DenseDev:

    buf: torch.Tensor
    n: int
    m: int
    order_f: int

    @property
    def dtype(self):
        return self.buf.dtype

    @staticmethod
    def from_host(X: np.ndarray) -> "DenseDev":
# ... 604 lines not shown
        del key
        cnt64 = torch.bincount(key_sorted, minlength=S * mpad) if nnz else \
            torch.zeros(S * mpad, dtype=torch.int64, device=dev)
        rounds = torch.div(cnt64.view(S * G, C).max(dim=1).values + (P - 1), P, rounding_mode="floor") \
            if S else torch.zeros(0, dtype=torch.int64, device=dev)
        if S * G and max_extra is not None and int((rounds > 1).sum().item()) > max_extra * S * G \
                and total0 > (1 << 22):
            return None
        del rounds
        vals = torch.zeros(total0, dtype=csr.data.dtype, device=dev)
        koff = torch.zeros(total0, dtype=torch.int32, device=dev)
        xptr = torch.zeros(S * G + 1, dtype=torch.int64, device=dev)
        xvals = torch.zeros(1, dtype=csr.data.dtype, device=dev)
        xkoff = torch.zeros(4, dtype=torch.int32, device=dev)
        if nnz:
            rank = torch.arange(nnz, device=dev, dtype=torch.int64) - \
                (torch.cumsum(cnt64, dim=0) - cnt64)[key_sorted]
            blk = torch.div(key_sorted, C, rounding_mode="floor")
            w = torch.remainder(key_sorted, C)
            j = torch.remainder(w, 8)
            slot = torch.div(w, 8, rounding_mode="floor") * 16 + torch.remainder(j, 2) * P \
                + torch.remainder(rank, P)
            chunk = torch.div(j, 2, rounding_mode="floor")
            rnd = torch.div(rank, P, rounding_mode="floor")
            del rank, w, j
            rloc = rows[perm] - torch.div(key_sorted, mpad, rounding_mode="floor") * R
            kv = ((rloc + 1) * int(lib().tm_lg_row_bytes(fbytes))).to(torch.int32)
            del rloc
            v = csr.data[perm]
            first = rnd == 0
            dst0 = (blk * CH + chunk) * SL + slot
            vals[dst0[first]] = v[first]
            koff[dst0[first]] = kv[first]
            later = ~first
            if bool(later.any().item()):
                nrec = torch.bincount(blk[later], minlength=S * G)
                torch.cumsum(nrec, dim=0, out=xptr[1:])
                ne = int(later.sum().item())
                xent = torch.zeros((ne, 4), dtype=torch.int32, device=dev)
                vl = v[later].contiguous()
                if fbytes == 8:
                    xent[:, 0:2] = vl.view(torch.int32).view(ne, 2)
                else:
                    xent[:, 0] = vl.view(torch.int32)
                xent[:, 2] = kv[later]
                xent[:, 3] = torch.remainder(key_sorted[later], C).to(torch.int32)
                xkoff = xent.reshape(-1).contiguous()
                hdr = koff.view(S * G, CH * SL)
                hdr[:, 0] |= (nrec << 20).to(torch.int32)
                start = xptr[:-1]
                for t in range(3):
                    part = torch.bitwise_and(torch.bitwise_right_shift(start, 12 * t), 0xFFF)
                    hdr[:, 1 + t] |= torch.where(nrec > 0, part << 20, torch.zeros_like(part)).to(torch.int32)
                del nrec, xent, vl, hdr, start
            del dst0, blk, slot, chunk, rnd, v, kv, first, later
        del cnt64, key_sorted, perm, rows
        return SlabLg(vals, koff, xptr, xvals, xkoff, inv, n, m, mpad, 2)


@dataclass
class SlabEnt:

    vals: torch.Tensor
    meta: torch.Tensor
    bstart: torch.Tensor
    inv: torch.Tensor
    n: int
    m: int
    mk: int

    SLACK = 192
    CONT_PERIOD = 15

    @property
    def dtype(self):
        return self.vals.dtype

    def nbytes(self) -> int:
        return sum(int(t.numel()) * t.element_size() for t in (self.vals, self.meta, self.bstart))

    def n_slots(self) -> int:
        return int(self.vals.numel()) - SlabEnt.SLACK

    @staticmethod
    def from_csr(csr: CsrDev, max_pad: float = None) -> "SlabEnt":
        from .._lib import lib

        R = int(lib().tm_ent_rows())
        C = int(lib().tm_ent_group_cols())
        U = int(lib().tm_ent_batch_slots())
        n, m = csr.n, csr.m
        if n >= (1 << 28):
            return None
        dev = csr.data.device
        S = (n + R - 1) // R
        G = max(1, (m + C - 1) // C)
        nnz = int(csr.data.numel())
        idx64 = csr.indices.to(torch.int64)
        colcnt = torch.bincount(idx64, minlength=m) if nnz else torch.zeros(m, dtype=torch.int64, device=dev)
        order = torch.sort(colcnt, descending=True, stable=True).indices
        rank = torch.empty(m, dtype=torch.int64, device=dev)
        rank[order] = torch.arange(m, device=dev, dtype=torch.int64)
        grp_of = torch.remainder(rank, G)
        jloc_of = torch.div(rank, G, rounding_mode="floor")
        inv = grp_of * C + jloc_of
        del order, colcnt, rank
        SL = SlabEnt.SLACK
        if nnz == 0 or S == 0:
            return SlabEnt(torch.zeros(SL, dtype=csr.data.dtype, device=dev),
                           torch.zeros(SL, dtype=torch.int16, device=dev),
                           torch.zeros((G, S + 1), dtype=torch.int32, device=dev), inv, n, m, G * C)
        counts = csr.indptr[1:] - csr.indptr[:-1]
        rows = torch.repeat_interleave(torch.arange(n, device=dev, dtype=torch.int64), counts)
        key = grp_of[idx64] * S + torch.div(rows, R, rounding_mode="floor")
        cnt = torch.bincount(key, minlength=G * S)
        nb = torch.div(cnt + (U - 1), U, rounding_mode="floor")
        slab_of = torch.arange(G * S, device=dev, dtype=torch.int64) % S
        nb = nb + ((cnt == 0) & (slab_of % SlabEnt.CONT_PERIOD == 0)).to(nb.dtype)
        total_b = int(nb.sum().item())
        if max_pad is not None and total_b * U > max_pad * nnz and total_b * U > (1 << 22):
            return None
        if total_b >= 2**31 // U:
            return None
        bst = torch.zeros(G * S + 1, dtype=torch.int64, device=dev)
        torch.cumsum(nb, dim=0, out=bst[1:])
        key_sorted, perm = torch.sort(key, stable=True)
        del key
        first = torch.cumsum(cnt, dim=0) - cnt
        pos = bst[key_sorted] * U + (torch.arange(nnz, device=dev, dtype=torch.int64) - first[key_sorted])
        del key_sorted
        T = total_b * U
        rows_p = rows[perm]
        del rows
        def word16(row, col):
            w = (((row >> 6) & 63) << 10) | ((row & 63) << 4) | col
            return torch.where(w >= 32768, w - 65536, w).to(torch.int16)

        has = nb > 0
        frow = torch.where(cnt > 0, rows_p[first.clamp(max=nnz - 1)], slab_of * R)[has]
        meta = torch.zeros(T + SL, dtype=torch.int16, device=dev)
        meta[:T] = torch.repeat_interleave(word16(frow, torch.zeros_like(frow)), nb[has] * U)
        del frow, has, first, cnt, nb, slab_of
        vals = torch.zeros(T + SL, dtype=csr.data.dtype, device=dev)
        vals[pos] = csr.data[perm]
        meta[pos] = word16(rows_p, jloc_of[idx64[perm]])
        del pos, perm, rows_p, idx64
        gi = torch.arange(G, device=dev, dtype=torch.int64)[:, None] * S + \
            torch.arange(S + 1, device=dev, dtype=torch.int64)[None, :]
        bstart = bst[gi].to(torch.int32).contiguous()
        return SlabEnt(vals, meta, bstart, inv, n, m, G * C)


def onehot_slab(cats, n: int, dtype: torch.dtype):
    from .._lib import lib

    C = int(lib().tm_slab_group_cols())
    dev = cats[0][0].device
    total = sum(int(c[1]) for c in cats)
    G = max(1, (total + C - 1) // C)
    c_all = torch.arange(total, device=dev, dtype=torch.int64)
    perm_pos = (c_all % G) * C + torch.div(c_all, G, rounding_mode="floor")
    cols, valid = [], []
    off = 0
    for codes, ncol, drop in cats:
        c = codes.to(torch.int64) - int(bool(drop))
        ok = (c >= 0) & (c < ncol)
# ... 16 lines not shown
```

tabmat_amd/ext/sparse.py:

```python
from __future__ import annotations

import os


from .. import _device as D
from .._lib import call
from ._types import CsrDev, DenseDev, SlabCsc, SlabEll, SlabEnt, SlabLg


def _csr_args(A: CsrDev):
    return (D.p(A.data), D.p(A.indices), D.p(A.indptr), A.n, A.m)


def sparse_sandwich(A: CsrDev, d, rows, cols):
    m = A.m if cols is None else D.nlen(cols)
    out = D.zeros((m, m), A.dtype)
    if m == 0 or (rows is not None and D.nlen(rows) == 0):
        return out
    D.same_float("sparse_sandwich", A.data, d)
    call(f"tm_sparse_sandwich_{D.fsuf(A.data)}", *_csr_args(A), D.p(d), D.p(rows), D.nlen(rows),
         D.p(cols), D.nlen(cols), D.p(out), D.stream_ptr())
    return out


# ... 55 lines not shown

def csr_matvec_multi(X: CsrDev, V, rows, cols, transpose):
    K = int(V.shape[1])
    n_cols = X.m if cols is None else D.nlen(cols)
    n_rows = X.n if rows is None else D.nlen(rows)
    out = D.zeros((n_cols if transpose else n_rows, K), X.dtype)
    if K == 0 or n_rows == 0 or n_cols == 0:
        return out
    D.same_float("csr_matvec_multi", X.data, V)
    Vc = V.contiguous()
    fn = "tm_csr_rmatvec_multi_" if transpose else "tm_csr_matvec_multi_"
    call(fn + D.fsuf(X.data), *_csr_args(X), D.p(Vc), K, D.p(rows), D.nlen(rows), D.p(cols),
         D.nlen(cols), D.p(out), D.stream_ptr())
    return out


def csr_dense_sandwich_slab(A: SlabCsc, B: DenseDev, d):
    assert B.n == A.n
    out = D.zeros((A.m, B.m), A.vals.dtype)
    if A.m == 0 or B.m == 0 or A.n == 0:
        return out
    D.same_float("csr_dense_sandwich_slab", A.vals, B.buf, d)
    call(f"tm_csr_dense_sandwich_slab_{D.fsuf(A.vals)}", D.p(A.vals), D.p(A.koff), D.p(A.cnt),
         D.p(A.gptr), A.n, A.m, D.p(B.buf), B.m, B.order_f, D.p(d), D.p(out), D.stream_ptr())
    return out


def ell_supported(B: DenseDev) -> bool:
    vec = 16 // B.buf.element_size()
    return (not B.order_f) and B.m % vec == 0 and B.m >= vec and B.buf.data_ptr() % 16 == 0


def csr_dense_sandwich_ell(A: SlabEll, B: DenseDev, d):
    assert B.n == A.n and ell_supported(B)
    if A.m == 0 or B.m == 0 or A.n == 0:
        return D.zeros((A.m, B.m), A.vals.dtype)
    out = D.zeros((A.mk, B.m), A.vals.dtype)
    D.same_float("csr_dense_sandwich_ell", A.vals, B.buf, d)
    fn = "tm_csr_dense_sandwich_ellw_" if A.wide else "tm_csr_dense_sandwich_ell_"
    call(fn + D.fsuf(A.vals), D.p(A.vals), D.p(A.koff), D.p(A.gptr),
         A.n, A.mk, D.p(B.buf), B.m, D.p(d), D.p(out), D.stream_ptr())
    return out[A.inv]


def csr_dense_sandwich_lg(A: SlabLg, B: DenseDev, d, unc=None, want_colsum=False):
    assert B.n == A.n and ell_supported(B)
    dt = A.dtype
    if A.m == 0 or B.m == 0 or A.n == 0:
        z = D.zeros((A.m, B.m), dt)
        return (z, D.zeros((A.m,), dt)) if want_colsum else z
    out = D.out_buf((A.mk, B.m), dt)
    u = int(A.unc if unc is None else unc)
    cs = D.out_buf((A.mk,), dt) if want_colsum else None
    if A.cvals is not None:
        D.same_float("csr_dense_sandwich_lg", A.cvals, B.buf, d)
        call("tm_csr_dense_sandwich_lgc_" + D.fsuf(A.cvals), D.p(A.cvals), D.p(A.cmap), D.p(A.crec),
             D.p(A.xkoff), A.n, A.mk, D.p(B.buf), B.m, D.p(d), u, D.p(out), D.p(cs), D.stream_ptr())
    elif want_colsum:
        D.same_float("csr_dense_sandwich_lg", A.vals, B.buf, d)
        call("tm_csr_dense_sandwich_lg_xtd_" + D.fsuf(A.vals), D.p(A.vals), D.p(A.koff), D.p(A.xptr),
             D.p(A.xvals), D.p(A.xkoff), A.n, A.mk, D.p(B.buf), B.m, D.p(d), u, D.p(out), D.p(cs),
             D.stream_ptr())
    else:
        D.same_float("csr_dense_sandwich_lg", A.vals, B.buf, d)
        call("tm_csr_dense_sandwich_lg_" + D.fsuf(A.vals), D.p(A.vals), D.p(A.koff), D.p(A.xptr),
             D.p(A.xvals), D.p(A.xkoff), A.n, A.mk, D.p(B.buf), B.m, D.p(d), u, D.p(out), D.stream_ptr())
    return (out[A.inv], cs[A.inv]) if want_colsum else out[A.inv]


def csr_dense_sandwich_ent(A: SlabEnt, B: DenseDev, d, want_colsum=False):
    assert B.n == A.n and ell_supported(B)
    dt = A.dtype
    if A.m == 0 or B.m == 0 or A.n == 0:
        z = D.zeros((A.m, B.m), dt)
        return (z, D.zeros((A.m,), dt)) if want_colsum else z
    out = D.out_buf((A.mk, B.m), dt)
    cs = D.out_buf((A.mk,), dt) if want_colsum else None
    D.same_float("csr_dense_sandwich_ent", A.vals, B.buf, d)
    call("tm_csr_dense_sandwich_ent_" + D.fsuf(A.vals), D.p(A.vals), D.p(A.meta), D.p(A.bstart), A.n, A.mk,
         D.p(B.buf), B.m, D.p(d), D.p(out), D.p(cs), D.stream_ptr())
    return (out[A.inv], cs[A.inv]) if want_colsum else out[A.inv]


def _row_table(A: CsrDev, rows, d, as_set: bool):
    import weakref

    import torch

    cm_data, cm_c8, cptr = A.chunk_major()
    cached = getattr(A, "_row_table", None)
    stamp = (rows.data_ptr(), rows._version, int(rows.numel()))
    if cached is not None and cached[0]() is rows and cached[4] == stamp:
        _, r64, dup, tabs, _ = cached
    else:
        r64 = torch.sort(rows.to(torch.int64)).values
        dup = bool((r64[1:] == r64[:-1]).any().item()) if r64.numel() > 1 else False
        tabs = {}
        A._row_table = (weakref.ref(rows), r64, dup, tabs, stamp)
    key = bool(as_set and dup)
    if key not in tabs:
        rr = torch.unique_consecutive(r64) if key else r64
        tabs[key] = (rr, torch.stack([cptr[:, rr], cptr[:, rr + 1]], dim=2).contiguous())
    rr, ranges = tabs[key]
    return cm_data, cm_c8, ranges, rr.to(torch.int32).contiguous(), d[rr].contiguous()


def sparse_sandwich_rows(A: CsrDev, d, rows):
    out = D.zeros((A.m, A.m), A.dtype)
    if A.m == 0 or D.nlen(rows) == 0 or A.data.numel() == 0:
        return out
    D.same_float("sparse_sandwich_rows", A.data, d)
    cm_data, cm_c8, ranges, r32, d_sel = _row_table(A, rows, d, True)
    cols = cm_c8 if K2B_U8 else A.chunk_cols32()
    call(f"tm_sparse_sandwich_chunked_rows_{'u8_' if K2B_U8 else ''}{D.fsuf(A.data)}", D.p(cm_data),
         D.p(cols), D.p(ranges),
         int(r32.numel()), A.m, int(cm_data.numel()), D.p(d_sel), D.p(out), D.stream_ptr())
    return out


def csr_dense_sandwich_rows(A: CsrDev, B: DenseDev, d, rows):
    out = D.zeros((A.m, B.m), A.dtype)
    if A.m == 0 or B.m == 0 or D.nlen(rows) == 0 or A.data.numel() == 0:
        return out
    D.same_float("csr_dense_sandwich_rows", A.data, B.buf, d)
    cm_data, cm_c8, ranges, r32, d_sel = _row_table(A, rows, d, False)
    call(f"tm_csr_dense_sandwich_rows_u8_{D.fsuf(A.data)}", D.p(cm_data), D.p(cm_c8), D.p(ranges),
         int(r32.numel()), D.p(r32), D.p(d_sel), A.n, A.m, D.p(B.buf), B.m, B.order_f, D.p(out),
         D.stream_ptr())
    return out


def sparse_sandwich_chunked(A: CsrDev, d):
    if A.m == 0 or A.n == 0:
        return D.zeros((A.m, A.m), A.dtype)
    out = D.out_buf((A.m, A.m), A.dtype)
    D.same_float("sparse_sandwich_chunked", A.data, d)
    cm_data, cm_c8, cptr = A.chunk_major()
    cols = cm_c8 if K2B_U8 else A.chunk_cols32()
    call(f"tm_sparse_sandwich_chunked_{'u8_' if K2B_U8 else ''}{D.fsuf(A.data)}", D.p(cm_data),
         D.p(cols), D.p(cptr),
         A.n, A.m, int(cm_data.numel()), D.p(d), D.p(out), D.stream_ptr())
    return out


K2_BLOCKS = True


def blocks_sandwich_pays(A: CsrDev) -> bool:
    import torch

    if not K2_BLOCKS or A.n == 0 or A.m == 0 or A.n >= 2**29:
        return False
    nnz = int(A.data.numel())
    nch = -(-A.m // 128)
    if not (0 < nnz < 2**31) or nnz / (A.n * nch) <= 4.5 or nch > 32:
        return False
    est = 16 * 2 * A.n * nch * (nch + 1) // 2
    return est * 3 < torch.cuda.mem_get_info(A.data.device)[0] or bool(getattr(A, "_pb", None))


K2B_U8 = os.environ.get("TABMAT_AMD_K2B_U8", "1") == "1"


def sparse_sandwich_blocks(A: CsrDev, d):
    if A.m == 0 or A.n == 0:
        return D.zeros((A.m, A.m), A.dtype)
    out = D.out_buf((A.m, A.m), A.dtype)
    D.same_float("sparse_sandwich_blocks", A.data, d)
    cm_data, cm_c8, cptr = A.chunk_major()
    blocks, wg_tab, max_nb = A.pair_blocks(d12=None if K2B_U8 else False)
    if int(blocks.shape[1]) == 3:
        call(f"tm_sparse_sandwich_blocks_p12_{D.fsuf(A.data)}", D.p(cm_data), D.p(cm_c8), D.p(cptr), A.n, A.m,
             int(cm_data.numel()), D.p(blocks), D.p(wg_tab), int(wg_tab.shape[0]), int(max_nb), D.p(d),
             D.p(out), D.stream_ptr())
        return out
    if K2B_U8:
        call(f"tm_sparse_sandwich_blocks_u8_{D.fsuf(A.data)}", D.p(cm_data), D.p(cm_c8), D.p(cptr), A.n, A.m,
             int(cm_data.numel()), D.p(blocks), D.p(wg_tab), int(wg_tab.shape[0]), int(max_nb), D.p(d),
             D.p(out), D.stream_ptr())
        return out
    cm_ind = A.chunk_cols32()
    call(f"tm_sparse_sandwich_blocks_{D.fsuf(A.data)}", D.p(cm_data), D.p(cm_ind), D.p(cptr), A.n, A.m,
         int(cm_data.numel()), D.p(blocks), D.p(wg_tab), int(wg_tab.shape[0]), int(max_nb), D.p(d),
         D.p(out), D.stream_ptr())
    return out


def sparse_sandwich_pairs(A: CsrDev, d):
    if A.m == 0 or A.n == 0:
        return D.zeros((A.m, A.m), A.dtype)
    out = D.out_buf((A.m, A.m), A.dtype)
    D.same_float("sparse_sandwich_pairs", A.data, d)
    _, _, cptr = A.chunk_major()
    if K2_PAIRS_PACKED and A.n < 2**25:
        rec = A.chunk_records_packed()
        call(f"tm_sparse_sandwich_pairs_pk_{D.fsuf(A.data)}", D.p(rec), D.p(cptr), A.n, A.m, int(A.data.numel()), D.p(d),
             D.p(out), D.stream_ptr())
        return out
    rec = A.chunk_records()
    call(f"tm_sparse_sandwich_pairs_{D.fsuf(A.data)}", D.p(rec), D.p(cptr), A.n, A.m, int(rec.shape[0]), D.p(d),
         D.p(out), D.stream_ptr())
    return out


def csc_dense_sandwich_sorted(A: CsrDev, B: DenseDev, d):
    if A.m == 0 or B.m == 0:
        return D.zeros((A.m, B.m), A.dtype)
    rows, vals, bstart, n_blocks, col_bptr = A.csc_blocks()
    out = D.out_buf((A.m, B.m), A.dtype)
    D.same_float("csc_dense_sandwich_sorted", vals, B.buf, d)
    call(f"tm_csc_dense_sandwich_sorted_{D.fsuf(vals)}", D.p(rows), D.p(vals), D.p(bstart),
         int(n_blocks), D.p(col_bptr), A.m, D.p(d), D.p(B.buf), B.m, D.p(out), D.stream_ptr())
    return out


def sparse_sandwich_direct(A: CsrDev, d):
    if A.m == 0 or A.n == 0:
        return D.zeros((A.m, A.m), A.dtype)
    out = D.out_buf((A.m, A.m), A.dtype)
    D.same_float("sparse_sandwich_direct", A.data, d)
    call(f"tm_sparse_sandwich_direct_{D.fsuf(A.data)}", D.p(A.data), D.p(A.indices), D.p(A.indptr),
         A.n, A.m, D.p(d), D.p(out), D.stream_ptr())
    return out


def direct_sandwich_pays(A: CsrDev) -> bool:
    nnz, n, m = int(A.data.numel()), A.n, A.m
    if n == 0 or nnz == 0 or m <= 1024:
        return False
    nch = (m + 127) // 128
    per_row = nnz / n
    pairs = n * per_row * (per_row + 1.0) / 2.0 * 1.3
    if nch > 32:
        return pairs / 15e9 < n * (nch * (nch + 1) / 2) * 0.3e-9
    if per_row / nch > 0.6:
        return False
    return pairs / 15e9 < n * (nch * (nch + 1) / 2) * 15e-12


K2_PAIRS = "auto"
K2_PAIRS_PACKED = os.environ.get("TABMAT_AMD_K2_PAIRS_PACKED", "1") == "1"
K2_PAIRS_MAX_M = 16384
K2_PAIRS_MAX_NNZ = 2**31 - 4 * 16 * 64


def pairs_sandwich_pays(A: CsrDev) -> bool:
    if K2_PAIRS != "auto":
        return K2_PAIRS == "1" and A.m <= K2_PAIRS_MAX_M and 0 < int(A.data.numel()) < K2_PAIRS_MAX_NNZ
    nnz, n, m = int(A.data.numel()), A.n, A.m
    if n == 0 or nnz == 0 or m <= 512 or m > K2_PAIRS_MAX_M or nnz >= K2_PAIRS_MAX_NNZ:
        return False
    nch = (m + 127) // 128
    parts = nch * (nch + 1) / 2
    per_row = nnz / n
    k = per_row / nch
    pairs = n * per_row * (per_row + 2.0) / 2.0
    pk = 0.75 if (K2_PAIRS_PACKED and n < 2**25) else 1.0
    t_pairs = (nnz * (nch + 1) / 2.0 * 2.3e-12 * pk * min(6.0, max(1.0, (1.6 / k) ** 0.8)) + pairs * 2.7e-12 * pk
               + min(parts, 768) * 0.8e-6 + max(0.0, parts - 768) * 0.1e-6)
    t_direct = pairs / 21e9
    if nch > 32:
        t_tiled = n * parts * 0.3e-9
    else:
        t_tiled = pairs * 1.15e-12 if k > 4.5 else n * parts * 17e-12 + pairs * 0.8e-12
    return t_pairs < 0.9 * min(t_direct, t_tiled)


def transpose_square_dot_weights(A: CsrDev, weights):
# ... 51 lines not shown
```

tabmat_amd/ext/split.py:

```python
from __future__ import annotations

import ctypes as C

import numpy as np

from .. import _device as D
from .._lib import call
from ._types import CsrDev, DenseDev, SlabCsc


def sandwich_cat_dense(i_indices, i_ncol, d, mat_j: DenseDev, rows, j_cols, drop_first=False):
    n_j = mat_j.m if j_cols is None else D.nlen(j_cols)
    res = D.zeros((i_ncol, n_j), mat_j.dtype)
    n_rows = i_indices.numel() if rows is None else D.nlen(rows)
    if d.numel() == 0 or n_rows == 0 or n_j == 0 or i_ncol == 0:
        return res
    D.same_float("sandwich_cat_dense", mat_j.buf, d)
    call(f"tm_cat_dense_sandwich_{D.fsuf(mat_j.buf)}", D.p(i_indices), i_indices.numel(), i_ncol,
         int(drop_first), D.p(d), D.p(rows), D.nlen(rows), D.p(mat_j.buf), mat_j.m, mat_j.order_f,
         D.p(j_cols), D.nlen(j_cols), D.p(res), D.stream_ptr())
    return res


def sandwich_cat_cat(i_indices, j_indices, i_ncol, j_ncol, d, rows, i_drop_first=False,
# ... 262 lines not shown
        order = np.argsort(b, kind="stable").astype(np.int32)
        ends = np.cumsum(np.bincount(b, minlength=n_blocks))
        starts = np.concatenate([[0], ends[:-1]])
        return ([order[s:e] for s, e in zip(starts, ends)],
                [loc[order[s:e]] for s, e in zip(starts, ends)], len(cols))
    next_idx = [0] * n_blocks
    sub_idx = [[] for _ in range(n_blocks)]
    sub_cols = [[] for _ in range(n_blocks)]
    for i, c in enumerate(cols.tolist()):
        for j in range(n_blocks):
            ind = self.indices[j]
            k = next_idx[j]
            while k < len(ind) and ind[k] < c:
                k += 1
            next_idx[j] = k
            if k < len(ind) and ind[k] == c:
                sub_idx[j].append(i)
                sub_cols[j].append(k)
                next_idx[j] = k + 1
                break
    return (
        [np.array(s, dtype=np.int32) for s in sub_idx],
        [np.array(s, dtype=np.int32) for s in sub_cols],
        len(cols),
    )


def is_sorted(a) -> bool:
    a = np.asarray(a)
    return bool(np.all(a[1:] >= a[:-1]))


MAX_FUSED_CATS = 16


def _cat_args(cats):
    n = len(cats)
    codes = (C.c_void_p * n)(*[c[0].data_ptr() for c in cats])
    ncols = (C.c_int64 * n)(*[int(c[1]) for c in cats])
    drop = (C.c_int32 * n)(*[int(bool(c[2])) for c in cats])
    return codes, ncols, drop, n


def multi_cat_dense_wide_ok(cats, mat_j: DenseDev) -> bool:
    fb = mat_j.buf.element_size()
    vec = 2
    total = sum(int(c[1]) for c in cats)
    tile = (total * 16 * vec * 8 + 15) // 16 * 16
    lds = tile + 16 * 32 * (fb + 4 * len(cats))
    return (not mat_j.order_f and 1 <= len(cats) <= 8 and mat_j.m >= vec and mat_j.m % vec == 0
            and mat_j.buf.data_ptr() % 16 == 0 and lds <= 150 * 1024)


def multi_cat_dense_tile_ok(cats, mat_j: DenseDev) -> bool:
    total = sum(int(c[1]) for c in cats)
    m = mat_j.m
    if total == 0 or m == 0 or not 1 <= len(cats) <= 16:
        return False
    tj = 64
    while tj > 1 and 8 * total * tj > 128 * 1024:
        tj >>= 1
    while tj > 1 and tj // 2 >= m:
        tj >>= 1
    return 8 * total * tj <= 128 * 1024 and (m + tj - 1) // tj <= 2


def multi_cat_dense_sandwich(cats, d, mat_j: DenseDev, rows=None):
    total = sum(int(c[1]) for c in cats)
    if total == 0 or mat_j.m == 0 or mat_j.n == 0 or (rows is not None and D.nlen(rows) == 0):
        return D.zeros((total, mat_j.m), mat_j.dtype)
    res = D.out_buf((total, mat_j.m), mat_j.dtype)
    codes, ncols, drop, n = _cat_args(cats)
    if rows is not None:
        D.same_float("multi_cat_dense_sandwich", mat_j.buf, d)
        call(f"tm_multi_cat_dense_sandwich_rows_{D.fsuf(mat_j.buf)}", codes, ncols, drop, n, mat_j.n,
             D.p(d), D.p(mat_j.buf), mat_j.m, D.p(rows), D.nlen(rows), D.p(res), D.stream_ptr())
        return res
    D.same_float("multi_cat_dense_sandwich", mat_j.buf, d)
    call(f"tm_multi_cat_dense_sandwich_{D.fsuf(mat_j.buf)}", codes, ncols, drop, n, mat_j.n,
         D.p(d), D.p(mat_j.buf), mat_j.m, mat_j.order_f, D.p(res), D.stream_ptr())
    return res


def multi_cat_sparse_sandwich(cats, d, S: SlabCsc):
    total = sum(int(c[1]) for c in cats)
    if total == 0 or S.m == 0 or S.n == 0:
        return D.zeros((total, S.m), S.vals.dtype)
    res = D.out_buf((total, S.m), S.vals.dtype)
    codes, ncols, drop, n = _cat_args(cats)
    D.same_float("multi_cat_sparse_sandwich", S.vals, d)
    call(f"tm_multi_cat_sparse_sandwich_slab_{D.fsuf(S.vals)}", codes, ncols, drop, n, S.n, D.p(d),
         D.p(S.vals), D.p(S.koff), D.p(S.ecol), D.p(S.gptr), S.m, D.p(res), D.stream_ptr())
    return res


PACKED_CODES = True


def pack_codes(cats):
    import torch

    total = sum(int(c[1]) for c in cats)
    if not PACKED_CODES or len(cats) > 3 or total >= 1023 or len(cats) == 0:
        return None
    codes, ncols, drop, n = _cat_args(cats)
    nrow = int(cats[0][0].numel())
    out = torch.empty((nrow,), dtype=torch.int32, device=cats[0][0].device)
    call("tm_multi_cat_pack_codes", codes, ncols, drop, n, nrow, D.p(out), D.stream_ptr())
    return out


def multi_cat_sparse_sandwich_ent(cats, d, E, packed=None):
    total = sum(int(c[1]) for c in cats)
    if total == 0 or E.m == 0 or E.n == 0:
        return D.zeros((total, E.m), E.vals.dtype)
    res = D.out_buf((total, E.mk), E.vals.dtype)
    codes, ncols, drop, n = _cat_args(cats)
    D.same_float("multi_cat_sparse_sandwich_ent", E.vals, d)
    if packed is not None:
        call(f"tm_multi_cat_sparse_sandwich_entp_{D.fsuf(E.vals)}", codes, ncols, drop, n, E.n, D.p(d),
             D.p(E.vals), D.p(E.meta), D.p(E.bstart), E.n_slots(), E.mk, D.p(packed), D.p(res), D.stream_ptr())
        return res[:, E.inv]
    call(f"tm_multi_cat_sparse_sandwich_ent_{D.fsuf(E.vals)}", codes, ncols, drop, n, E.n, D.p(d),
         D.p(E.vals), D.p(E.meta), D.p(E.bstart), E.n_slots(), E.mk, D.p(res), D.stream_ptr())
    return res[:, E.inv]


def multi_cat_sparse_sandwich_rows(cats, d, A, rows):
    from . import sparse as xs

    total = sum(int(c[1]) for c in cats)
    if total == 0 or A.m == 0 or D.nlen(rows) == 0 or A.data.numel() == 0:
        return D.zeros((total, A.m), A.data.dtype)
    res = D.out_buf((total, A.m), A.data.dtype)
    codes, ncols, drop, n = _cat_args(cats)
    D.same_float("multi_cat_sparse_sandwich_rows", A.data, d)
    cm_data, cm_c8, ranges, r32, d_sel = xs._row_table(A, rows, d, False)
    call(f"tm_multi_cat_sparse_sandwich_rows_u8_{D.fsuf(A.data)}", codes, ncols, drop, n, D.p(cm_data),
         D.p(cm_c8), D.p(ranges), D.p(r32), int(r32.numel()), A.m, D.p(d_sel), D.p(res), D.stream_ptr())
    return res
```

tabmat_amd/sparse_matrix.py:

```python
from __future__ import annotations

import os

import numpy as np
import torch
from scipy import sparse as sps

from . import _device as D
from .ext import sparse as xs
from .ext._types import CsrDev, SlabCsc, SlabEll, SlabEnt, SlabLg
from .matrix_base import MatrixBase
from .util import (
    check_indexer,
    check_matvec_dimensions,
    check_matvec_out_shape,
    check_sandwich_compatible,
    check_transpose_matvec_out_shape,
    normalize_index,
    device_row_index,
    selects_all_columns,
)


ELL_MAX_PAD = 8.0
# ... 228 lines not shown
            for a, b, part in parts:
                r = None
                if rows is not None:
                    r64 = rows.to(torch.int64)
                    sel = r64[(r64 >= a) & (r64 < b)]
                    if sel.numel() == 0:
                        continue
                    r = (sel - a).to(torch.int32)
                res = part._sandwich_dev(d[a:b], r, cols)
                out = res if out is None else out + res
            if out is None:
                k = self.shape[1] if cols is None else D.nlen(cols)
                out = D.zeros((k, k), d.dtype)
            return out
        A = self._dev()
        from . import categorical_matrix as _cm

        if _cm.DETERMINISTIC and A.data.numel() > 0 and self.shape[0] > 0:
            res = self._sandwich_deterministic(d, rows, cols)
            if res is not None:
                return res
            import warnings

            warnings.warn("TABMAT_AMD_DETERMINISTIC=1: this sparse block has no entry twin, its self sandwich "
                          "falls back to the LDS-atomic kernels and is NOT bit-reproducible from run to run",
                          RuntimeWarning, stacklevel=3)
        if getattr(self, "_direct_pays", None) is None:
            self._direct_pays = xs.direct_sandwich_pays(A)
        w = D.nlen(cols) if cols is not None else 0
        if (0 < w <= NARROW_COLS and 2 * w < self.shape[1] and self.shape[0] > 0 and A.data.numel() > 0
                and self._narrow_pays(w)
                and self.shape[0] * w * A.data.element_size() * 4 < torch.cuda.mem_get_info()[0]):
            from .ext import dense as xd
            from .ext._types import DenseDev

            rws, vls, bstart, _, col_bptr = A.csc_blocks()
            mx = getattr(self, "_max_col_len", None)
            if mx is None:
                ends = bstart[col_bptr]
                mx = self._max_col_len = int((ends[1:] - ends[:-1]).max().item())
            cd = cols.to(torch.int64)
            seg = torch.stack([bstart[col_bptr[cd]], bstart[col_bptr[cd + 1]]], dim=1).contiguous()
            T = torch.zeros((self.shape[0], w), dtype=A.data.dtype, device=A.data.device)
            xs.csc_densify_cols(rws, vls, seg, torch.arange(w, dtype=torch.int32, device=A.data.device),
                                mx, T)
            return xd.dense_sandwich(DenseDev(T, self.shape[0], w, 0), d, rows, None)
        pp = getattr(self, "_pairs_pay", None)
        if pp is None:
            pp = self._pairs_pay = xs.pairs_sandwich_pays(A)
        if pp and (rows is None or D.nlen(rows) > 0.3 * self.shape[0]):
            d = D.masked_d(d, rows, as_set=True)
            res = xs.sparse_sandwich_pairs(A, d)
            if cols is not None:
                c64 = cols.to(torch.int64)
                res = res[c64][:, c64].contiguous()
            return res
        pays = getattr(self, "_direct_pays", None)
        if pays is None:
            pays = self._direct_pays = xs.direct_sandwich_pays(A)
        if pays:
            d = D.masked_d(d, rows, as_set=True)
            res = xs.sparse_sandwich_direct(A, d)
            if cols is not None:
                c64 = cols.to(torch.int64)
                res = res[c64][:, c64].contiguous()
            return res
        if A.data.numel() > 0 and A.data.numel() < 2**31 and self.shape[1] <= 128 * 32:
            if rows is not None and 0 < D.nlen(rows) <= ROW_LIST_FRACTION * self.shape[0]:
                res = xs.sparse_sandwich_rows(A, d, rows)
                if cols is not None:
                    c64 = cols.to(torch.int64)
                    res = res[c64][:, c64].contiguous()
                return res
            d = D.masked_d(d, rows, as_set=True)
            bl = getattr(self, "_blocks_pay", None)
            if bl is None:
                bl = self._blocks_pay = xs.blocks_sandwich_pays(A)
            res = xs.sparse_sandwich_blocks(A, d) if bl else xs.sparse_sandwich_chunked(A, d)
            if cols is not None:
                c64 = cols.to(torch.int64)
                res = res[c64][:, c64].contiguous()
            return res
        return xs.sparse_sandwich(A, d, rows, cols)

    def _ent_det(self):
        ent = self._ent()
        if ent is None:
            hit = getattr(self, "_entblk_det", None)
            if hit is None:
                twin = SlabEnt.from_csr(self._dev(), max_pad=None)
                hit = self._entblk_det = twin if twin is not None else False
            ent = hit or None
        return ent

    def _sandwich_deterministic(self, d, rows, cols=None):
        from .ext._types import DenseDev

        ent = self._ent_det()
        if ent is None:
            return None
        n, m = self.shape
        A = self._dev()
        d = D.masked_d(d, rows, as_set=True)
        inv = None
        if cols is None:
            sel = torch.arange(m, dtype=torch.int64, device=d.device)
        else:
            sel, inv = torch.unique(cols.to(torch.int64), return_inverse=True)
            if int(sel.numel()) == int(inv.numel()) and bool((sel == cols.to(torch.int64)).all()):
                inv = None
        k = int(sel.numel())
        out = torch.empty((m, k), dtype=d.dtype, device=d.device)
        W = 128
        for c0 in range(0, k, W):
            w = min(W, k - c0)
            w_pad = (w + 3) // 4 * 4
            colmap = torch.full((m,), -1, dtype=torch.int32, device=d.device)
            colmap[sel[c0:c0 + w]] = torch.arange(w, dtype=torch.int32, device=d.device)
            T = torch.zeros((n, w_pad), dtype=A.data.dtype, device=d.device)
            xs.csr_densify_cols(A, colmap, T)
            res = xs.csr_dense_sandwich_ent(ent, DenseDev(T, n, w_pad, 0), d)
            out[:, c0:c0 + w] = res[:, :w]
            del T
        out = out if cols is None else out[sel]
        low = torch.tril(out)
        full = low + torch.tril(out, -1).T
        if inv is not None:
            full = full.index_select(0, inv).index_select(1, inv)
        return full

    def _sdiag_dev(self, d, rows, want_s1=False):
        parts = self._row_parts()
        if parts is not None:
            s1 = D.zeros((self.shape[1],), d.dtype) if want_s1 else None
            s2 = D.zeros((self.shape[1],), d.dtype)
            for a, b, part in parts:
                r = None
                if rows is not None:
                    r64 = rows.to(torch.int64)
                    sel = r64[(r64 >= a) & (r64 < b)]
                    if sel.numel() == 0:
                        continue
                    r = (sel - a).to(torch.int32)
                p1, p2 = part._sdiag_dev(d[a:b], r, want_s1)
                s2 += p2
                if want_s1:
                    s1 += p1
            return s1, s2
        A = self._dev()
        if rows is not None and A.data.numel() > 0 and not self._values_finite():
            r64 = rows.to(torch.int64)
            return xs.csr_sandwich_diag(A.take_rows("index", r64), d[r64].contiguous(), want_s1)
        return xs.csr_sandwich_diag(A, D.masked_d(d, rows).contiguous(), want_s1)

    def sandwich_diag(self, d, rows=None, cols=None):
        from .matrix_base import _sd_args

        a = _sd_args(self, d, rows, cols)
        if a.trivial is not None:
            return a.finish(a.trivial)
        tdt = D.torch_dtype(self.dtype)
        _, g = self._sdiag_dev(D.to_dev(a.d, tdt), D.idx_dev(a.rows))
        if a.cols is not None:
            g = g[D.idx_dev(a.cols, torch.int64)]
        return a.finish(g)

# ... 136 lines not shown
```

tabmat_amd/split_matrix.py:

```python
from __future__ import annotations

import os
import warnings
from collections.abc import Sequence
from typing import Optional, Union

import numpy as np
import torch
from scipy import sparse as sps

from . import _device as D
from .categorical_matrix import CategoricalMatrix
from .dense_matrix import DenseMatrix, _centre_and_shift
from .ext import split as xsplit
from .ext.dense import dense_glm_loss_grad as xd_glm
from .ext.dense import dense_sandwich_matvec as xd_smv
from .matrix_base import MatrixBase
from .sparse_matrix import SparseMatrix
from .standardized_mat import StandardizedMatrix
from .util import (
    check_matvec_dimensions,
    check_matvec_out_shape,
    check_sandwich_compatible,
    check_transpose_matvec_out_shape,
    collapse_identity,
    normalize_index,
    set_up_rows_or_cols,
)


ROW_LIST_FRACTION_CATSPARSE = 0.04
DIAG_FROM_PAIRS = True
CAT_PAIRS_FUSED = os.environ.get("TABMAT_AMD_CAT_PAIRS", "1") != "0"
FULL_THEN_SELECT = float(os.environ.get("TABMAT_AMD_FULL_THEN_SELECT", "0.5"))
FULL_RESULT_MAX_BYTES = 256 << 20
FULL_UNSELECTED_SHARE = 0.2
FULL_THEN_SELECT_MV = 0.0
NARROW_COLS = int(os.environ.get("TABMAT_AMD_NARROW_COLS", "128"))
from . import categorical_matrix as _cm
from . import sparse_matrix as _spm


class _Centering:
    NARROW_GROUP = 1 << 20

    def __init__(self, vec):
        self.vec = dict(vec)
        self.cs_centered = set()
        self.groups = None

    def get(self, b):
        return self.vec.get(b)


class _Xtv:

    def __init__(self, v):
        self.v = v
        self.out = {}


def as_tabmat(a):
    if isinstance(a, (MatrixBase, StandardizedMatrix)):
        return a
    if sps.issparse(a):
        return SparseMatrix(a.tocsc(copy=False))
    if isinstance(a, np.ndarray):
        return DenseMatrix(a)
    raise ValueError(f"Cannot convert type {type(a)} to Matrix.")


def hstack(tup: Sequence) -> MatrixBase:
    mats = [as_tabmat(a) for a in tup]
    if not mats:
        raise ValueError("Need at least one array to concatenate.")
    if all(isinstance(m, SparseMatrix) for m in mats):
        return SparseMatrix(sps.hstack([m.array_csc for m in mats]))
    if all(isinstance(m, DenseMatrix) for m in mats):
        return DenseMatrix(np.hstack([m.toarray() for m in mats]))
    return SplitMatrix(mats)


def _merge_same_kind(matrices, indices):
    for kind in (DenseMatrix, SparseMatrix):
        which = [i for i, m in enumerate(matrices) if isinstance(m, kind)]
        if len(which) <= 1:
            continue
        gidx = np.concatenate([indices[i] for i in which])
        order = np.argsort(gidx)
        names = np.concatenate([np.array(matrices[i]._colnames, dtype=object) for i in which])
        terms = np.concatenate([np.array(matrices[i]._terms, dtype=object) for i in which])
        if kind is DenseMatrix:
            merged = DenseMatrix(np.hstack([matrices[i].toarray() for i in which])[:, order])
        else:
            merged = SparseMatrix(sps.hstack([matrices[i].array_csc for i in which]).tocsc()[:, order])
        merged._colnames = names[order].tolist()
        merged._terms = terms[order].tolist()
        matrices[which[0]] = merged
        indices[which[0]] = gidx[order]
        drop = set(which[1:])
        matrices = [m for i, m in enumerate(matrices) if i not in drop]
        indices = [x for i, x in enumerate(indices) if i not in drop]
    return matrices, indices


def _block_sdiag(mb, d, rows, center=None, want_s1=False):
    d = d.to(D.torch_dtype(mb.dtype))
    if isinstance(mb, DenseMatrix):
        return mb._sdiag_dev(d, rows, None if center is None else center.to(d.dtype).contiguous()), None
    if isinstance(mb, SparseMatrix):
        s1, s2 = mb._sdiag_dev(d, rows, want_s1)
        return s2, s1
    if isinstance(mb, CategoricalMatrix):
        h = mb._sandwich_diag_dev(d, rows, None)
        return h, (h if want_s1 else None)
    r = None if rows is None else D.to_host(rows)
# ... 237 lines not shown
            xtd[pd] = cs.to(torch.float64)
        if center is not None:
            return out, xtd, cmask, center.groups
        return out, xtd

    FUSED_LEVELS = 496
    FUSED_CATS = 8

    def _cat_groups(self, cat_ids):
        groups, cur, tot = [], [], 0
        for i in cat_ids:
            k = self.matrices[i].shape[1]
            if k > self.FUSED_LEVELS:
                continue
            if cur and (len(cur) == self.FUSED_CATS or tot + k > self.FUSED_LEVELS):
                groups.append(cur)
                cur, tot = [], 0
            cur.append(i)
            tot += k
        if cur:
            groups.append(cur)
        return groups

    def _cat_pairs_plan(self):
        plan = self.__dict__.get("_cp_plan", False)
        if plan is False:
            plan = None
            ids = [i for i, m in enumerate(self.matrices)
                   if isinstance(m, CategoricalMatrix) and m.shape[1] > 0]
            if len(ids) >= 1:
                pos = self._full_dev_indices()
                plan = xsplit.CatPairsPlan([(i, self.matrices[i].shape[1]) for i in ids],
                                           [pos[i] for i in ids])
            self.__dict__["_cp_plan"] = plan
        return plan

    def _cat_hist_plan(self):
        plan = self.__dict__.get("_ch_plan", False)
        if plan is False:
            plan = None
            ids = [i for i, m in enumerate(self.matrices)
                   if isinstance(m, CategoricalMatrix) and m.shape[1] > 0 and m.shape[0] > 0]
            if len(ids) >= 2:
                pos = self._full_dev_indices()
                plan = xsplit.CatPairsPlan([(i, self.matrices[i].shape[1]) for i in ids],
                                           [pos[i] for i in ids], diag_only=True)
            self.__dict__["_ch_plan"] = plan
        return plan

    def _fused_cats(self, mw, cats, cat_ids, d_eff, rows, total, budget, d_rows=None):
        if isinstance(mw, DenseMatrix) and xsplit.multi_cat_dense_wide_ok(cats, mw._dev_c()):
            if rows is not None and D.nlen(rows) <= 0.5 * self.shape[0]:
                return xsplit.multi_cat_dense_sandwich(cats, d_rows, mw._dev_c(), rows)
            return xsplit.multi_cat_dense_sandwich(cats, d_eff, mw._dev_c())
        if isinstance(mw, DenseMatrix) and xsplit.multi_cat_dense_tile_ok(cats, mw._dev_c()):
            return xsplit.multi_cat_dense_sandwich(cats, d_eff, mw._dev_c())
        if isinstance(mw, DenseMatrix):
            if xsplit.cat_dense_sorted_ok(mw._dev_c()):
                return None
            from .ext import sparse as xs

            oh, inv = self._onehot_slab(cat_ids)
            return xs.csr_dense_sandwich_slab(oh, mw._dev_c(), d_eff)[inv]
        if (isinstance(mw, SparseMatrix) and total * 33 <= budget and rows is not None
                and 0 < D.nlen(rows) <= ROW_LIST_FRACTION_CATSPARSE * self.shape[0]
                and 0 < mw._dev().data.numel() < 2**31):
            return xsplit.multi_cat_sparse_sandwich_rows(cats, d_rows, mw._dev(), rows)
        if (isinstance(mw, SparseMatrix) and total * 33 <= budget
                and mw._dev().data.numel() > 0 and (rows is None or mw._values_finite())):
            ent = None
            if len(cats) <= 8 and (getattr(mw, "_entblk", None) or any(
                    isinstance(mo, DenseMatrix) and mo.shape[1] > 64 and mo.dtype == mw.dtype
                    for mo in self.matrices)):
                ent = mw._ent()
            if ent is not None:
                pk_cache = self.__dict__.setdefault("_packed_codes", {})
                key = tuple(cat_ids)
                if key not in pk_cache:
                    pk_cache[key] = xsplit.pack_codes(cats)
                return xsplit.multi_cat_sparse_sandwich_ent(cats, d_eff, ent, pk_cache[key])
            return xsplit.multi_cat_sparse_sandwich(cats, d_eff, mw._slab())
        return None

    def _parts(self):
        parts = self.__dict__.get("_row_parts", False)
        if parts is False:
            parts = None
            big = [m for m in self.matrices
                   if isinstance(m, SparseMatrix) and m._dev().data.numel() >= _spm.PART_NNZ]
            if big:
                n = self.shape[0]
                lead = max(big, key=lambda m: m._dev().data.numel())
                ptr = lead._dev().indptr
                nnz = int(ptr[-1].item())
                k = -(-nnz // max(1, int(0.8 * _spm.PART_NNZ)))
                while True:
                    targets = torch.arange(1, k, device=ptr.device, dtype=torch.int64) * nnz // k
                    cuts = [0] + torch.searchsorted(ptr, targets).clamp_(0, n).tolist() + [n]
                    cuts = sorted(set(int(c) for c in cuts))
                    ok = all(int((m._dev().indptr[cuts[1:]] - m._dev().indptr[cuts[:-1]]).max().item())
                             < _spm.PART_NNZ for m in big)
                    if ok or k >= n:
                        break
                    k += 1
                parts = [(a, b, self[a:b]) for a, b in zip(cuts[:-1], cuts[1:]) if b > a]
            self.__dict__["_row_parts"] = parts
        return parts

    def _sandwich_parts(self, parts, d, rows, cols_host, colsum, center=None):
        out = None
        for a, b, part in parts:
            r = None
            if rows is not None:
                r64 = rows.to(torch.int64)
                sel = r64[(r64 >= a) & (r64 < b)]
                if sel.numel() == 0:
                    continue
                r = (sel - a).to(torch.int32)
            cs = [None] * len(self.matrices) if colsum is not None else None
            sub_cen = None if center is None else _Centering(center.vec)
            res = part._sandwich_dev(d[a:b], r, cols_host, None, cs, center=sub_cen)
            if sub_cen is not None:
                center.groups = sub_cen.groups
            if sub_cen is not None and colsum is not None:
                dsum = (d[a:b] if r is None else d[a:b][r.to(torch.int64)]).sum(dtype=torch.float64)
                _, sub_p, _ = self._sandwich_plan(cols_host)
                for i in sub_cen.cs_centered:
                    if cs[i] is not None and sub_cen.get(i) is not None:
                        cv = sub_cen.get(i).to(torch.float64)
                        if sub_p[i] is not None:
                            cv = cv[sub_p[i].to(torch.int64)]
                        cs[i] = cs[i].to(torch.float64) + cv * dsum
            out = res if out is None else out + res
            if colsum is not None:
                for i, c in enumerate(cs):
                    if c is None:
                        colsum[i] = False
                    elif colsum[i] is not False:
                        colsum[i] = c if colsum[i] is None else colsum[i] + c
        if colsum is not None:
            for i, c in enumerate(colsum):
                if c is False:
                    colsum[i] = None
        if out is None:
            _, _, n_cols = self._sandwich_plan(cols_host)
            out = D.zeros((n_cols, n_cols), torch.float64)
        return out

    def _full_product_pays(self, sub_h) -> bool:
        p = self.shape[1]
        if p * p * 8 > FULL_RESULT_MAX_BYTES:
            return False
        n = max(self.shape[0], 1)
        tot = unsel = 0.0
        for b, mb in enumerate(self.matrices):
            if isinstance(mb, DenseMatrix):
                wb = float(mb.shape[1])
            elif isinstance(mb, SparseMatrix):
                nnz = mb._devblk.data.numel() if mb._devblk is not None else mb._host().nnz
                wb = max(1.0, float(nnz) / n)
            else:
                wb = 1.0 + mb.shape[1] / 256.0
            tot += wb
            if len(sub_h[b]) == 0:
                unsel += wb
        return unsel <= FULL_UNSELECTED_SHARE * tot
# ... 62 lines not shown
        from .ext._types import DenseDev

        n = self.shape[0]
        T = torch.zeros((n, nar["w_pad"]), dtype=d.dtype, device=d.device)
        for b, t0, s, idx in nar["parts"]:
            mb = self.matrices[b]
            if isinstance(mb, SparseMatrix):
                xs.csc_densify_cols(*idx, T)
            else:
                xd.dense_gather_cols(mb._dev(), idx, T, t0)
        tmp = nar["tmp"]
        if tmp is None:
            tmp = nar["tmp"] = SplitMatrix([DenseMatrix(T)] + [self.matrices[i] for i in nar["cat"]],
                                           nar["indices"])
        dm = tmp.matrices[0]
        dm._devblk = DenseDev(T, n, nar["w_pad"], 0)
        sub_cen = None
        if center is not None:
            tc = torch.zeros((nar["w_pad"],), dtype=d.dtype, device=d.device)
            for b, t0, s, idx in nar["parts"]:
                if center.get(b) is not None:
                    tc[t0:t0 + s] = center.get(b)[idx.to(torch.int64)]
            sub_cen = _Centering({0: tc})
        try:
            cs_tmp = [None] * len(tmp.matrices) if colsum is not None else None
            full = tmp._sandwich_dev(d, rows, None, None, cs_tmp, center=sub_cen)
        finally:
            dm._devblk = None
        if colsum is not None:
            if cs_tmp[0] is not None:
                for b, t0, s, _ in nar["parts"]:
                    colsum[b] = cs_tmp[0][t0:t0 + s]
                    if sub_cen is not None and 0 in sub_cen.cs_centered:
                        center.cs_centered.add(b)
            for k, i in enumerate(nar["cat"]):
                if cs_tmp[1 + k] is not None and i in nar["cat_sub"]:
                    colsum[i] = cs_tmp[1 + k][nar["cat_sub"][i]]
        if center is not None:
            g = torch.full_like(nar["sel"], -1, dtype=torch.int32)
            g[nar["sel"] < nar["w_pad"]] = _Centering.NARROW_GROUP
            center.groups = g
        sel = nar["sel"]
        return full.index_select(0, sel).index_select(1, sel)

    def _sandwich_dev(self, d, rows, cols_host, plan=None, colsum=None, center=None, xtv=None):
        if cols_host is not None and len(cols_host) >= FULL_THEN_SELECT * self.shape[1] \
                and len(cols_host) > 0 and self._full_product_pays_cols(cols_host):
            pos_d, sub_d, n_cols = plan if plan is not None else self._sandwich_plan(cols_host)
            cs_full = [None] * len(self.matrices) if colsum is not None else None
            full = self._sandwich_dev(d, rows, None, None, cs_full, center=center, xtv=xtv)
            if colsum is not None:
                for i, c in enumerate(cs_full):
                    if c is not None:
                        colsum[i] = c if sub_d[i] is None else c[sub_d[i].to(torch.int64)]
            cd = self._cols_dev64(cols_host)
            return full.index_select(0, cd).index_select(1, cd)
        parts = self._parts()
        if parts is not None:
            return self._sandwich_parts(parts, d, rows, cols_host, colsum, center)
        if cols_host is not None and plan is None and NARROW_COLS > 0:
            nar = self._narrow_plan(cols_host)
            if nar == "wide":
                cs_full = [None] * len(self.matrices) if colsum is not None else None
                full = self._sandwich_dev(d, rows, None, None, cs_full, center=center, xtv=xtv)
                if colsum is not None:
                    _, sub_sel, _ = self._sandwich_plan(cols_host)
                    for i, c in enumerate(cs_full):
                        if c is not None:
                            colsum[i] = c if sub_sel[i] is None else c[sub_sel[i].to(torch.int64)]
                cd = self._cols_dev64(cols_host)
                return full.index_select(0, cd).index_select(1, cd)
            if nar is not None and d.dtype == D.torch_dtype(self.dtype):
                return self._sandwich_narrow(nar, d, rows, colsum, center)
        pos_d, sub_d, n_cols = plan if plan is not None else self._sandwich_plan(cols_host)
        out = D.zeros((n_cols, n_cols), torch.float64)
        mats = self.matrices
        empty = [sd is not None and D.nlen(sd) == 0 for sd in sub_d]
        done = set()
        return self._sandwich_terms(d, rows, cols_host, colsum, out, pos_d, sub_d, empty, done, center,
                                    xtv if cols_host is None else None)

    def _sandwich_terms(self, d, rows, cols_host, colsum, out, pos_d, sub_d, empty, done, center=None, xtv=None):
        from .ext import dense as xd

        mats = self.matrices
        cat_ids = [i for i, m in enumerate(mats) if isinstance(m, CategoricalMatrix) and not empty[i]
                   and m.shape[1] > 0]
        budget = (128 * 1024) // 8
        groups = self._cat_groups(cat_ids)
        if groups:
            d_eff = D.masked_d(d, rows)
        for grp in groups:
            cats = [(mats[i]._dev(), mats[i].shape[1], mats[i].drop_first) for i in grp]
            total = sum(c[1] for c in cats)
            offs = np.concatenate([[0], np.cumsum([c[1] for c in cats])])
            for w, mw in enumerate(mats):
                if empty[w] or mw.dtype != self.dtype or d.dtype != D.torch_dtype(self.dtype):
                    continue
                stacked = self._fused_cats(mw, cats, grp, d_eff, rows, total, budget, d)
                if stacked is None:
                    continue
                whole = cols_host is None and len(grp) > 1
                if whole:
                    cache = self.__dict__.setdefault("_group_pos", {})
                    gpos = cache.get(tuple(grp))
                    if gpos is None:
                        gpos = cache[tuple(grp)] = torch.cat([pos_d[i] for i in grp])
                    xsplit.scatter_block(stacked.contiguous(), gpos, pos_d[w], out, mirror=True)
                for ci, i in enumerate(grp):
                    res = stacked[int(offs[ci]):int(offs[ci + 1])]
                    if (colsum is not None and colsum[w] is None and not mats[i].drop_first
                            and not mats[i]._has_missings):
                        cs = res.sum(dim=0)
                        colsum[w] = cs if sub_d[w] is None else cs[sub_d[w].to(torch.int64)]
                    if not whole:
                        res = CategoricalMatrix._restrict(res, sub_d[i], sub_d[w])
                        xsplit.scatter_block(res.contiguous(), pos_d[i], pos_d[w], out, mirror=True)
                    done.add((min(i, w), max(i, w)))
        big = [i for i in cat_ids if mats[i].shape[1] > self.FUSED_LEVELS]
        if len(big) >= 2 and len(big) <= 16 and d.dtype == D.torch_dtype(self.dtype):
            cats = [(mats[i]._dev(), mats[i].shape[1], mats[i].drop_first) for i in big]
            offs = np.concatenate([[0], np.cumsum([c[1] for c in cats])])
            d_big = None
            for w, mw in enumerate(mats):
                if (empty[w] or not isinstance(mw, DenseMatrix) or mw.dtype != self.dtype
                        or not xsplit.multi_cat_dense_tile_ok(cats, mw._dev_c())):
                    continue
                if d_big is None:
                    d_big = D.masked_d(d, rows)
                stacked = xsplit.multi_cat_dense_sandwich(cats, d_big, mw._dev_c())
                for ci, i in enumerate(big):
                    res = stacked[int(offs[ci]):int(offs[ci + 1])]
                    if (colsum is not None and colsum[w] is None and not mats[i].drop_first
                            and not mats[i]._has_missings):
                        cs = res.sum(dim=0)
                        colsum[w] = cs if sub_d[w] is None else cs[sub_d[w].to(torch.int64)]
                    res = CategoricalMatrix._restrict(res, sub_d[i], sub_d[w])
                    xsplit.scatter_block(res.contiguous(), pos_d[i], pos_d[w], out, mirror=True)
                    done.add((min(i, w), max(i, w)))
        cat_diag = {}
        diag_scattered = set()
        det = _cm.DETERMINISTIC
        plan = self._cat_pairs_plan() if CAT_PAIRS_FUSED and not det else None
        if (plan is not None and plan.n_pairs > 0
                and d.dtype in (torch.float32, torch.float64)
                and d.dtype == D.torch_dtype(self.dtype)):
            cl = [(mats[i]._dev(), mats[i].shape[1], mats[i].drop_first) for i in plan.cat_ids]
            pos_sel = None if cols_host is None else self._pairs_pos_sel(plan, cols_host)
            tables = xsplit.multi_cat_pairs(plan, cl, d, rows, out, pos=pos_sel)
            for i, j, toff, li, lj, stride in plan.pairs:
                if i == j:
                    if not empty[i]:
                        full = tables[toff:toff + (li - 1) * stride + 1:stride]
                        if sub_d[i] is not None and colsum is not None:
                            full = full[sub_d[i].to(torch.int64)]
                        cat_diag[i] = full.to(d.dtype)
                        diag_scattered.add(i)
                else:
                    done.add((i, j))
        complete = [isinstance(m, CategoricalMatrix) and not m.drop_first and not m._has_missings
                    and sub_d[k] is None and not empty[k] for k, m in enumerate(mats)]
        for i, mi in enumerate(mats):
            if empty[i] or not isinstance(mi, CategoricalMatrix):
                continue
            for j in range(i + 1, len(mats)):
                if empty[j] or not isinstance(mats[j], CategoricalMatrix) or (i, j) in done:
                    continue
                res = mi._cross_sandwich_dev(mats[j], d, rows, sub_d[i], sub_d[j])
                xsplit.scatter_block(res.contiguous(), pos_d[i], pos_d[j], out, mirror=True)
                done.add((i, j))
                if DIAG_FROM_PAIRS and not det and complete[j] and i not in cat_diag:
                    cat_diag[i] = res.sum(dim=1)
                if DIAG_FROM_PAIRS and not det and complete[i] and j not in cat_diag:
                    cat_diag[j] = res.sum(dim=0)
        for i, mi in enumerate(mats):
            if empty[i]:
                continue
            if isinstance(mi, CategoricalMatrix):
                diag = cat_diag[i] if i in cat_diag else mi._sandwich_diag_dev(d, rows, sub_d[i])
                if colsum is not None:
                    colsum[i] = diag
                if i not in diag_scattered:
                    xsplit.scatter_block(diag, pos_d[i], pos_d[i], out, diag=True)
            elif (xtv is not None and colsum is None and center is None and isinstance(mi, DenseMatrix)
                  and sub_d[i] is None and (both := mi._sandwich_xtv_dev(d, xtv.v, rows)) is not None):
                res, xtv.out[i] = both
                xsplit.scatter_block(res, pos_d[i], pos_d[i], out)
            elif (colsum is not None and colsum[i] is None and isinstance(mi, DenseMatrix)
                  and rows is None and sub_d[i] is None
                  and (both := mi._sandwich_xtd_dev(d, cen_i := (center.get(i) if center else None))) is not None):
                res, colsum[i] = both
                if cen_i is not None:
                    center.cs_centered.add(i)
                xsplit.scatter_block(res, pos_d[i], pos_d[i], out)
            elif isinstance(mi, DenseMatrix) and center is not None and center.get(i) is not None:
                res = mi._sandwich_dev(d, rows, sub_d[i], center=center.get(i))
                xsplit.scatter_block(res, pos_d[i], pos_d[i], out)
            else:
                res = mi._sandwich_dev(d, rows, sub_d[i])
                xsplit.scatter_block(res, pos_d[i], pos_d[i], out)
        for i, mi in enumerate(mats):
            if empty[i]:
                continue
            for j in range(i + 1, len(mats)):
                if empty[j] or (i, j) in done:
                    continue
                si, di = (i, j) if isinstance(mi, SparseMatrix) else (j, i)
                if (colsum is not None and colsum[si] is None and isinstance(mats[si], SparseMatrix)
                        and isinstance(mats[di], DenseMatrix)):
                    box = []
                    res = mats[si]._cross_sandwich_dev(mats[di], d, rows, sub_d[si], sub_d[di],
                                                       colsum_box=box)
                    if box:
                        colsum[si] = box[0]
                    if si != i:
                        res = res.T
                else:
                    res = mi._cross_sandwich_dev(mats[j], d, rows, sub_d[i], sub_d[j])
                xsplit.scatter_block(res.contiguous(), pos_d[i], pos_d[j], out, mirror=True)
        return out

    def sandwich_graph(self, d, rows=None, cols=None):
        from .graph import CapturedProduct

        check_sandwich_compatible(self, d)
        rows_d = D.idx_dev(normalize_index(rows, self.shape[0]))
        cols_n = collapse_identity(normalize_index(cols, self.shape[1]), self.shape[1])
        plan = self._sandwich_plan(cols_n)
        return CapturedProduct(lambda dd: self._sandwich_dev(dd, rows_d, cols_n, plan), d)

    def sandwich(self, d, rows=None, cols=None):
        on_dev = D.is_dev(d)
        if not on_dev:
            d = np.asarray(d)
        check_sandwich_compatible(self, d)
        rows_n = normalize_index(rows, self.shape[0])
        cols_n = collapse_identity(normalize_index(cols, self.shape[1]), self.shape[1])
        out = self._sandwich_dev(D.to_dev(d), D.idx_dev(rows_n), cols_n)
        return out if on_dev else D.to_host(out)

    def sandwich_and_transpose_matvec(self, d, v, rows=None, cols=None):
        from .matrix_base import _check_1d

        _check_1d(v)
        d_dev_side, v_dev_side = D.is_dev(d), D.is_dev(v)
        if not d_dev_side:
            d = np.asarray(d)
        if not v_dev_side:
            v = np.asarray(v)
        check_sandwich_compatible(self, d)
        check_matvec_dimensions(self, v, transpose=True)
        rows_n = normalize_index(rows, self.shape[0])
        cols_n = collapse_identity(normalize_index(cols, self.shape[1]), self.shape[1])
        tdt = D.torch_dtype(self.dtype)
        v_dev = D.to_dev(v, tdt)
        acc = None
        if (tdt == torch.float64 and not _cm.DETERMINISTIC
                and (rows_n is None or len(rows_n) < self.shape[0])):
            acc = _Xtv(v_dev)
        H = self._sandwich_dev(D.to_dev(d), D.idx_dev(rows_n), cols_n, xtv=acc)
        g, _ = self._transpose_matvec_dev(v_dev, rows_n, cols_n, done=None if acc is None else acc.out)
        if not v_dev_side:
            g = D.to_host(g)
            if np.issubdtype(v.dtype, np.floating):
                g = g.astype(np.result_type(self.dtype, v.dtype), copy=False)
        return (H if d_dev_side else D.to_host(H)), g

    def sandwich_matvec(self, d, u, rows=None, cols=None):
        from .matrix_base import _smv_args, _smv_compose

        a = _smv_args(self, d, u, rows, cols, h_dtype=np.float64)
        if a.trivial is not None:
            return a.finish(a.trivial)
        tdt = D.torch_dtype(self.dtype)
        res = None
        if (rows is None and cols is None) or self._blocks_finite():
            res = self._smv_dev(a.d_masked(tdt), a.u_full(tdt))
        if res is None:
            return a.finish(_smv_compose(self, a))
        g = res[0]
        if a.cols is not None:
            g = g[self._cols_dev64(a.cols)]
        return a.finish(g)

    def _sdiag_dev(self, d, rows, cols_host=None, centers=None, want_s1=False):
        p = self.shape[1]
        parts = self._parts()
        if parts is not None:
            s2 = D.zeros((p,), torch.float64)
            s1 = D.zeros((p,), torch.float64) if want_s1 else None
# ... 248 lines not shown
```

Baseline: 1032 GB/s.

## Fuse partial reduction and scatter into output for SplitMatrix sandwich blocks

Adds '_into' variants of the multi-categorical, sparse-block and sparse×dense sandwich kernels. Their finish step reduces the per-block partials and writes straight into the final p×p output at the given row/column positions, with optional mirroring. This replaces the separate reduce-partials, untile and scatter_block launches and the temporary result buffers. The SplitMatrix plain path (no rows, cols, centering or colsum) now routes through these, which adds complexity and new eligibility checks.

```diff
diff --git a/include/tabmat_hip.h b/include/tabmat_hip.h
--- a/include/tabmat_hip.h
+++ b/include/tabmat_hip.h
@@ -539,6 +539,54 @@
                          const int64_t *ci, double *out, int64_t p, int mirror, int diag,
                          void *stream);
 
+int tm_csr_dense_sandwich_ent_into_f32(const float *vals, const uint16_t *meta, const uint32_t *bstart, int64_t n,
+                                       int64_t m, const float *B, int64_t r, const float *d, const int64_t *ri,
+                                       const int64_t *ci, double *out, int64_t p, int mirror, int transpose,
+                                       float *colsum, void *stream);
+int tm_csr_dense_sandwich_ent_into_f64(const double *vals, const uint16_t *meta, const uint32_t *bstart, int64_t n,
+                                       int64_t m, const double *B, int64_t r, const double *d, const int64_t *ri,
+                                       const int64_t *ci, double *out, int64_t p, int mirror, int transpose,
+                                       double *colsum, void *stream);
+int tm_sparse_sandwich_blocks_p12_into_f32(const float *cm_data, const uint8_t *cm_col8, const int32_t *cptr,
+                                           int64_t n, int64_t m, int64_t nnz, const int32_t *blocks12,
+                                           const int32_t *wg_tab, int n_wg, int max_nb, const float *d,
+                                           const int64_t *pos, double *out, int64_t p, void *stream);
+int tm_sparse_sandwich_blocks_p12_into_f64(const double *cm_data, const uint8_t *cm_col8, const int32_t *cptr,
+                                           int64_t n, int64_t m, int64_t nnz, const int32_t *blocks12,
+                                           const int32_t *wg_tab, int n_wg, int max_nb, const double *d,
+                                           const int64_t *pos, double *out, int64_t p, void *stream);
+int tm_multi_cat_dense_sandwich_into_f32(const void *const *h_codes, const int64_t *h_ncols,
+                                         const int32_t *h_drop_first, int n_cats, int64_t n,
+                                         const float *d, const float *M, int64_t M_ncol, int order_f,
+                                         const int64_t *ri, const int64_t *ci, double *out, int64_t p, int mirror,
+                                         int transpose, void *stream);
+int tm_multi_cat_dense_sandwich_into_f64(const void *const *h_codes, const int64_t *h_ncols,
+                                         const int32_t *h_drop_first, int n_cats, int64_t n,
+                                         const double *d, const double *M, int64_t M_ncol, int order_f,
+                                         const int64_t *ri, const int64_t *ci, double *out, int64_t p, int mirror,
+                                         int transpose, void *stream);
+int tm_multi_cat_sparse_sandwich_ent_into_f32(const void *const *h_codes, const int64_t *h_ncols,
+                                              const int32_t *h_drop_first, int n_cats, int64_t n, const float *d,
+                                              const float *vals, const uint16_t *meta, const uint32_t *bstart,
+                                              int64_t n_slots, int64_t mk, const uint32_t *packed,
+                                              const int64_t *ri, const int64_t *ci, double *out, int64_t p,
+                                              int mirror, int transpose, void *stream);
+int tm_multi_cat_sparse_sandwich_ent_into_f64(const void *const *h_codes, const int64_t *h_ncols,
+                                              const int32_t *h_drop_first, int n_cats, int64_t n, const double *d,
+                                              const double *vals, const uint16_t *meta, const uint32_t *bstart,
+                                              int64_t n_slots, int64_t mk, const uint32_t *packed,
+                                              const int64_t *ri, const int64_t *ci, double *out, int64_t p,
+                                              int mirror, int transpose, void *stream);
+
+int tm_finish_coltiled_f32(const float *ws, int64_t rows, int W, int nb, int n_parts, int64_t nc, const int64_t *ri,
+                           const int64_t *ci, double *out, int64_t p, int mirror, int transpose, void *stream);
+int tm_finish_coltiled_f64(const double *ws, int64_t rows, int W, int nb, int n_parts, int64_t nc, const int64_t *ri,
+                           const int64_t *ci, double *out, int64_t p, int mirror, int transpose, void *stream);
+int tm_finish_tiles_f32(const float *ws, int max_nb, const int32_t *wg_tab, int n_wg, int64_t m, const int64_t *pos,
+                        double *out, int64_t p, void *stream);
+int tm_finish_tiles_f64(const double *ws, int max_nb, const int32_t *wg_tab, int n_wg, int64_t m, const int64_t *pos,
+                        double *out, int64_t p, void *stream);
+
 int tm_sparse_sandwich_chunked_rows_f32(const float *cm_data, const int32_t *cm_indices,
                                         const int32_t *row_ranges, int64_t n_sel, int64_t m,
                                         int64_t nnz, const float *d_sel, float *out, void *stream);
diff --git a/tabmat_amd/csrc/cat.hip b/tabmat_amd/csrc/cat.hip
--- a/tabmat_amd/csrc/cat.hip
+++ b/tabmat_amd/csrc/cat.hip
@@ -2,6 +2,7 @@
 
 #include "common.hpp"
 #include "reduce.hpp"
+#include "finish.hpp"
 
 namespace tmh {
 
@@ -1301,21 +1302,22 @@
     return TM_OK;
 }
 
-template <typename F>
+template <typename F, typename O = F>
 static int run_multi_cat_dense(const void *const *h_codes, const int64_t *h_ncols,
                                const int32_t *h_drop, int n_cats, int64_t n, const F *d, const F *M,
-                               int64_t m, int order_f, F *out, hipStream_t st,
-                               const int32_t *rows = nullptr, int64_t n_rows = 0) {
+                               int64_t m, int order_f, O *out, hipStream_t st,
+                               const int32_t *rows = nullptr, int64_t n_rows = 0,
+                               const FinishDst *into = nullptr) {
     CatSet cs;
     int rc = make_catset(h_codes, h_ncols, h_drop, n_cats, &cs);
     if (rc) return rc;
     const int64_t total = (int64_t)cs.total * m;
     if (total == 0) return TM_OK;
+    const FinishDst dst = into != nullptr ? *into : finish_plain(m);
     if (rows != nullptr) n = n_rows;
-    if (n == 0) {
-        TM_HIP(hipMemsetAsync(out, 0, sizeof(F) * (size_t)total, st));
-        return TM_OK;
-    }
+    if (n == 0)
+        return launch_finish_coltiled<F, O>(nullptr, (int64_t)cs.total * 32, 0, (int)ceil_div(m, 32), 32, m, out, dst,
+                                            st);
     {
         constexpr int VEC = MCW_VEC;
         constexpr int TJW = 16 * VEC;
@@ -1330,12 +1332,10 @@
             nblk = std::min<int64_t>(nblk, std::max<int64_t>(1, ceil_div(n, 4096)));
             const int64_t rpb = ceil_div(ceil_div(n, nblk), MCW_RS) * MCW_RS;
             nblk = ceil_div(n, rpb);
-            const size_t tmp_bytes = ((sizeof(F) * (size_t)(n_parts * stride) + 255) / 256) * 256;
             void *wsv = nullptr;
-            rc = get_workspace(tmp_bytes + sizeof(F) * (size_t)(n_parts * nblk * stride) + 256, &wsv, st);
+            rc = get_workspace(sizeof(F) * (size_t)(n_parts * nblk * stride) + 256, &wsv, st);
             if (rc) return rc;
-            F *tmp = reinterpret_cast<F *>(wsv);
-            F *ws = reinterpret_cast<F *>(reinterpret_cast<char *>(wsv) + tmp_bytes);
+            F *ws = reinterpret_cast<F *>(wsv);
             auto gow = [&](auto kern) -> int {
                 TM_HIP(hipFuncSetAttribute(reinterpret_cast<const void *>(kern),
                                            hipFuncAttributeMaxDynamicSharedMemorySize, (int)lds_w));
@@ -1357,13 +1357,7 @@
             else if (n_cats == 7) rc = gow(&multi_cat_dense_wide_kernel<F, 7>);
             else rc = gow(&multi_cat_dense_wide_kernel<F, 8>);
             if (rc) return rc;
-            rc = launch_reduce_partials<F>(ws, stride, (int)nblk, (int)n_parts, tmp, n_parts * stride,
-                                           false, st);
-            if (rc) return rc;
-            hipLaunchKernelGGL((multi_cat_untile_kernel<F>), dim3((unsigned)ceil_div(total, 256)),
-                               dim3(256), 0, st, tmp, (int64_t)cs.total, m, TJW, out);
-            TM_LAUNCH_CHECK();
-            return TM_OK;
+            return launch_finish_coltiled<F, O>(ws, stride, (int)nblk, (int)n_parts, TJW, m, out, dst, st);
         }
     }
     if (rows != nullptr) {
@@ -1384,12 +1378,10 @@
     nblk = std::min<int64_t>(nblk, std::max<int64_t>(1, ceil_div(n, 4096)));
     const int64_t rpb = ceil_div(n, nblk);
     nblk = ceil_div(n, rpb);
-    const size_t tmp_bytes = ((sizeof(F) * (size_t)(n_parts * stride) + 255) / 256) * 256;
     void *wsv = nullptr;
-    rc = get_workspace(tmp_bytes + sizeof(F) * (size_t)(n_parts * nblk * stride) + 256, &wsv, st);
+    rc = get_workspace(sizeof(F) * (size_t)(n_parts * nblk * stride) + 256, &wsv, st);
     if (rc) return rc;
-    F *tmp = reinterpret_cast<F *>(wsv);
-    F *ws = reinterpret_cast<F *>(reinterpret_cast<char *>(wsv) + tmp_bytes);
+    F *ws = reinterpret_cast<F *>(wsv);
     auto go = [&](auto kern) -> int {
         if (lds > 48 * 1024)
             TM_HIP(hipFuncSetAttribute(reinterpret_cast<const void *>(kern),
@@ -1423,13 +1415,7 @@
     }
 #undef TM_MCD_CASE
     if (rc) return rc;
-    rc = launch_reduce_partials<F>(ws, stride, (int)nblk, (int)n_parts, tmp, n_parts * stride, false,
-                                   st);
-    if (rc) return rc;
-    hipLaunchKernelGGL((multi_cat_untile_kernel<F>), dim3((unsigned)ceil_div(total, 256)),
-                       dim3(256), 0, st, tmp, (int64_t)cs.total, m, TJ, out);
-    TM_LAUNCH_CHECK();
-    return TM_OK;
+    return launch_finish_coltiled<F, O>(ws, stride, (int)nblk, (int)n_parts, TJ, m, out, dst, st);
 }
 
 template <typename F, typename IX>
@@ -1531,20 +1517,21 @@
     }
 }
 
-template <typename F>
+template <typename F, typename O = F>
 static int run_multi_cat_sparse_ent(const void *const *h_codes, const int64_t *h_ncols, const int32_t *h_drop,
                                     int n_cats, int64_t n, const F *d, const F *vals, const unsigned short *meta,
-                                    const unsigned *bstart, int64_t mk, F *out, hipStream_t st,
-                                    const unsigned *packed = nullptr, int64_t n_slots = 0) {
+                                    const unsigned *bstart, int64_t mk, O *out, hipStream_t st,
+                                    const unsigned *packed = nullptr, int64_t n_slots = 0,
+                                    const FinishDst *into = nullptr) {
     CatSet cs;
     int rc = make_catset(h_codes, h_ncols, h_drop, n_cats, &cs);
     if (rc) return rc;
     const int64_t total = (int64_t)cs.total * mk;
     if (total == 0) return TM_OK;
-    if (n == 0) {
-        TM_HIP(hipMemsetAsync(out, 0, sizeof(F) * (size_t)total, st));
-        return TM_OK;
-    }
+    const FinishDst dst = into != nullptr ? *into : finish_plain(mk);
+    if (n == 0)
+        return launch_finish_coltiled<F, O>(nullptr, (int64_t)cs.total * 32, 0, (int)ceil_div(mk, 32), 32, mk, out,
+                                            dst, st);
     TM_REQUIRE(mk % 16 == 0 && n_cats >= 1 && n_cats <= 8, "kernel columns in groups of 16, 1 .. 8 categoricals");
     TM_REQUIRE(n < (1ll << 28), "at most 2^28 - 1 rows per block");
     constexpr int GC = 32;
@@ -1562,12 +1549,10 @@
     nblk = std::min<int64_t>(nblk, n_slabs);
     const int64_t spb = ceil_div(n_slabs, nblk);
     nblk = ceil_div(n_slabs, spb);
-    const size_t tmp_bytes = ((sizeof(F) * (size_t)(n_pairs * stride) + 255) / 256) * 256;
     void *wsv = nullptr;
-    rc = get_workspace(tmp_bytes + sizeof(F) * (size_t)((int64_t)n_pairs * nblk * stride) + 256, &wsv, st);
+    rc = get_workspace(sizeof(F) * (size_t)((int64_t)n_pairs * nblk * stride) + 256, &wsv, st);
     if (rc) return rc;
-    F *tmp = reinterpret_cast<F *>(wsv);
-    F *ws = reinterpret_cast<F *>(reinterpret_cast<char *>(wsv) + tmp_bytes);
+    F *ws = reinterpret_cast<F *>(wsv);
     auto kern = n_cats == 1   ? &multi_cat_sparse_ent_kernel<F, 1>
                 : n_cats == 2 ? &multi_cat_sparse_ent_kernel<F, 2>
                 : n_cats == 3 ? &multi_cat_sparse_ent_kernel<F, 3>
@@ -1617,12 +1602,7 @@
         prof_end(st);
         TM_LAUNCH_CHECK();
     }
-    rc = launch_reduce_partials<F>(ws, stride, (int)nblk, n_pairs, tmp, (int64_t)n_pairs * stride, false, st);
-    if (rc) return rc;
-    hipLaunchKernelGGL((multi_cat_untile_kernel<F>), dim3((unsigned)ceil_div(total, 256)), dim3(256), 0, st, tmp,
-                       (int64_t)cs.total, mk, GC, out);
-    TM_LAUNCH_CHECK();
-    return TM_OK;
+    return launch_finish_coltiled<F, O>(ws, stride, (int)nblk, n_pairs, GC, mk, out, dst, st);
 }
 
 }
@@ -1782,6 +1762,44 @@
                                     double *out, void *stream) {
     return run_multi_cat_dense<double>(h_codes, h_ncols, h_drop_first, n_cats, n, d, M, M_ncol,
                                        order_f, out, as_stream(stream));
+}
+int tm_multi_cat_dense_sandwich_into_f32(const void *const *h_codes, const int64_t *h_ncols,
+                                         const int32_t *h_drop_first, int n_cats, int64_t n,
+                                         const float *d, const float *M, int64_t M_ncol, int order_f,
+                                         const int64_t *ri, const int64_t *ci, double *out, int64_t p, int mirror,
+                                         int transpose, void *stream) {
+    const FinishDst dst{ri, ci, p, mirror, transpose};
+    return run_multi_cat_dense<float, double>(h_codes, h_ncols, h_drop_first, n_cats, n, d, M, M_ncol, order_f, out,
+                                              as_stream(stream), nullptr, 0, &dst);
+}
+int tm_multi_cat_dense_sandwich_into_f64(const void *const *h_codes, const int64_t *h_ncols,
+                                         const int32_t *h_drop_first, int n_cats, int64_t n,
+                                         const double *d, const double *M, int64_t M_ncol, int order_f,
+                                         const int64_t *ri, const int64_t *ci, double *out, int64_t p, int mirror,
+                                         int transpose, void *stream) {
+    const FinishDst dst{ri, ci, p, mirror, transpose};
+    return run_multi_cat_dense<double, double>(h_codes, h_ncols, h_drop_first, n_cats, n, d, M, M_ncol, order_f, out,
+                                               as_stream(stream), nullptr, 0, &dst);
+}
+int tm_multi_cat_sparse_sandwich_ent_into_f32(const void *const *h_codes, const int64_t *h_ncols,
+                                              const int32_t *h_drop_first, int n_cats, int64_t n, const float *d,
+                                              const float *vals, const uint16_t *meta, const uint32_t *bstart,
+                                              int64_t n_slots, int64_t mk, const uint32_t *packed,
+                                              const int64_t *ri, const int64_t *ci, double *out, int64_t p,
+                                              int mirror, int transpose, void *stream) {
+    const FinishDst dst{ri, ci, p, mirror, transpose};
+    return run_multi_cat_sparse_ent<float, double>(h_codes, h_ncols, h_drop_first, n_cats, n, d, vals, meta, bstart,
+                                                   mk, out, as_stream(stream), packed, n_slots, &dst);
+}
+int tm_multi_cat_sparse_sandwich_ent_into_f64(const void *const *h_codes, const int64_t *h_ncols,
+                                              const int32_t *h_drop_first, int n_cats, int64_t n, const double *d,
+                                              const double *vals, const uint16_t *meta, const uint32_t *bstart,
+                                              int64_t n_slots, int64_t mk, const uint32_t *packed,
+                                              const int64_t *ri, const int64_t *ci, double *out, int64_t p,
+                                              int mirror, int transpose, void *stream) {
+    const FinishDst dst{ri, ci, p, mirror, transpose};
+    return run_multi_cat_sparse_ent<double, double>(h_codes, h_ncols, h_drop_first, n_cats, n, d, vals, meta, bstart,
+                                                    mk, out, as_stream(stream), packed, n_slots, &dst);
 }
 int tm_multi_cat_dense_sandwich_rows_f32(const void *const *h_codes, const int64_t *h_ncols,
                                          const int32_t *h_drop_first, int n_cats, int64_t n,
diff --git a/tabmat_amd/csrc/finish.hip b/tabmat_amd/csrc/finish.hip
--- /dev/null
+++ b/tabmat_amd/csrc/finish.hip
@@ -0,0 +1,52 @@
+#include "finish.hpp"
+
+namespace tmh {
+
+template <typename F>
+static int run_finish_coltiled(const F *ws, int64_t rows, int W, int nb, int n_parts, int64_t nc, const int64_t *ri,
+                               const int64_t *ci, double *out, int64_t p, int mirror, int transpose,
+                               hipStream_t st) {
+    TM_REQUIRE(rows >= 0 && W >= 1 && nb >= 0 && n_parts >= 0 && nc >= 0 && p >= 0, "negative size");
+    TM_REQUIRE(nc <= (int64_t)n_parts * W, "more columns than the parts hold");
+    TM_REQUIRE(nb == 0 || ws != nullptr, "NULL partials");
+    if (rows == 0 || nc == 0) return TM_OK;
+    TM_REQUIRE(out != nullptr, "NULL result");
+    return launch_finish_coltiled<F, double>(ws, rows * W, nb, n_parts, W, nc, out,
+                                             FinishDst{ri, ci, p, mirror, transpose}, st);
+}
+
+template <typename F>
+static int run_finish_tiles(const F *ws, int max_nb, const int32_t *wg_tab, int n_wg, int64_t m, const int64_t *pos,
+                            double *out, int64_t p, hipStream_t st) {
+    TM_REQUIRE(max_nb >= 0 && n_wg >= 0 && m >= 0 && p >= 0, "negative size");
+    TM_REQUIRE(m <= 32 * 128, "at most 32 column chunks");
+    TM_REQUIRE(n_wg == 0 || (ws != nullptr && wg_tab != nullptr), "NULL partials or workgroup table");
+    if (m == 0) return TM_OK;
+    TM_REQUIRE(out != nullptr, "NULL result");
+    return launch_finish_tiles<F, double>(ws, max_nb, wg_tab, n_wg, m, out, FinishDst{pos, pos, p, 1, 0}, st);
+}
+
+}
+
+extern "C" {
+
+int tm_finish_coltiled_f32(const float *ws, int64_t rows, int W, int nb, int n_parts, int64_t nc, const int64_t *ri,
+                           const int64_t *ci, double *out, int64_t p, int mirror, int transpose, void *stream) {
+    return tmh::run_finish_coltiled<float>(ws, rows, W, nb, n_parts, nc, ri, ci, out, p, mirror, transpose,
+                                           tmh::as_stream(stream));
+}
+int tm_finish_coltiled_f64(const double *ws, int64_t rows, int W, int nb, int n_parts, int64_t nc, const int64_t *ri,
+                           const int64_t *ci, double *out, int64_t p, int mirror, int transpose, void *stream) {
+    return tmh::run_finish_coltiled<double>(ws, rows, W, nb, n_parts, nc, ri, ci, out, p, mirror, transpose,
+                                            tmh::as_stream(stream));
+}
+int tm_finish_tiles_f32(const float *ws, int max_nb, const int32_t *wg_tab, int n_wg, int64_t m, const int64_t *pos,
+                        double *out, int64_t p, void *stream) {
+    return tmh::run_finish_tiles<float>(ws, max_nb, wg_tab, n_wg, m, pos, out, p, tmh::as_stream(stream));
+}
+int tm_finish_tiles_f64(const double *ws, int max_nb, const int32_t *wg_tab, int n_wg, int64_t m, const int64_t *pos,
+                        double *out, int64_t p, void *stream) {
+    return tmh::run_finish_tiles<double>(ws, max_nb, wg_tab, n_wg, m, pos, out, p, tmh::as_stream(stream));
+}
+
+}
diff --git a/tabmat_amd/csrc/finish.hpp b/tabmat_amd/csrc/finish.hpp
--- /dev/null
+++ b/tabmat_amd/csrc/finish.hpp
@@ -0,0 +1,140 @@
+#pragma once
+#include "common.hpp"
+
+namespace tmh {
+
+struct FinishDst {
+    const int64_t *ri;
+    const int64_t *ci;
+    int64_t p;
+    int mirror;
+    int transpose;
+};
+
+inline FinishDst finish_plain(int64_t nc) { return FinishDst{nullptr, nullptr, nc, 0, 0}; }
+
+template <typename O>
+__device__ __forceinline__ void finish_store(O *__restrict__ out, const FinishDst &dst, int64_t r, int64_t c,
+                                             double s) {
+    if (dst.mirror || !dst.transpose) out[r * dst.p + c] = (O)s;
+    if (dst.mirror || dst.transpose) out[c * dst.p + r] = (O)s;
+}
+
+template <int NW>
+__device__ __forceinline__ double finish_tree(double (*red)[64], int lane) {
+    double s = 0.0;
+#pragma unroll
+    for (int w = 0; w < NW; w += 4) s += (red[w][lane] + red[w + 1][lane]) + (red[w + 2][lane] + red[w + 3][lane]);
+    return s;
+}
+
+template <typename F, typename O, int NW>
+__global__ __launch_bounds__(NW * 64) void finish_coltiled_kernel(const F *__restrict__ ws, int64_t stride, int nb,
+                                                                  int W, int64_t nc, O *__restrict__ out,
+                                                                  FinishDst dst) {
+    __shared__ double red[NW][64];
+    const int lane = threadIdx.x & 63;
+    const int wave = threadIdx.x >> 6;
+    const int64_t e = (int64_t)blockIdx.x * 64 + lane;
+    const int part = blockIdx.y;
+    int64_t r = -1, c = -1;
+    if (e < stride) {
+        const int64_t a = e / W, b = (int64_t)part * W + e % W;
+        if (b < nc) {
+            r = dst.ri ? dst.ri[a] : a;
+            c = dst.ci ? dst.ci[b] : b;
+        }
+    }
+    const bool live = r >= 0 && c >= 0;
+    double acc = 0.0;
+    if (live) {
+        const F *p = ws + ((int64_t)part * nb) * stride + e;
+        for (int b = wave; b < nb; b += NW) acc += (double)p[(int64_t)b * stride];
+    }
+    red[wave][lane] = acc;
+    __syncthreads();
+    if (wave == 0 && live) finish_store(out, dst, r, c, (double)(F)finish_tree<NW>(red, lane));
+}
+
+inline bool finish_small(int64_t gx, int64_t gy, int nb) { return gx * gy < 1024 && nb > 16; }
+
+template <typename F, typename O>
+inline int launch_finish_coltiled(const F *ws, int64_t stride, int nb, int n_parts, int W, int64_t nc, O *out,
+                                  const FinishDst &dst, hipStream_t st) {
+    if (stride == 0 || n_parts == 0) return TM_OK;
+    dim3 grid((unsigned)ceil_div(stride, 64), (unsigned)n_parts);
+    if (finish_small(grid.x, grid.y, nb))
+        hipLaunchKernelGGL((finish_coltiled_kernel<F, O, 16>), grid, dim3(1024), 0, st, ws, stride, nb, W, nc, out,
+                           dst);
+    else
+        hipLaunchKernelGGL((finish_coltiled_kernel<F, O, 4>), grid, dim3(256), 0, st, ws, stride, nb, W, nc, out,
+                           dst);
+    TM_LAUNCH_CHECK();
+    return TM_OK;
+}
+
+template <typename F, typename O, int NW>
+__global__ __launch_bounds__(NW * 64) void finish_tiles_kernel(const F *__restrict__ ws, int max_nb,
+                                                               const int4 *__restrict__ wg_tab, int n_wg, int m,
+                                                               O *__restrict__ out, FinishDst dst) {
+    constexpr int TS = 128;
+    __shared__ double red[NW][64];
+    extern __shared__ unsigned owned[];
+    const int lane = threadIdx.x & 63;
+    const int wave = threadIdx.x >> 6;
+    const int part = blockIdx.y;
+    for (int w = threadIdx.x; w < (max_nb + 31) / 32; w += blockDim.x) owned[w] = 0u;
+    __syncthreads();
+    for (int g = threadIdx.x; g < n_wg; g += blockDim.x) {
+        const int4 t = wg_tab[2 * g];
+        if (t.x == part && t.y >= 0 && t.y < max_nb) atomicOr(&owned[t.y >> 5], 1u << (t.y & 31));
+    }
+    __syncthreads();
+    int I = (int)((sqrtf(8.0f * (float)part + 1.0f) - 1.0f) * 0.5f);
+    while ((I + 1) * (I + 2) / 2 <= part) ++I;
+    while (I * (I + 1) / 2 > part) --I;
+    const int J = part - I * (I + 1) / 2;
+    const int e = blockIdx.x * 64 + lane;
+    const int tr = e / TS, tc = e % TS;
+    const int i = I * TS + tr, j = J * TS + tc;
+    int64_t r = -1, c = -1;
+    if (i < m && j < m && (I != J || tc <= tr)) {
+        r = dst.ri ? dst.ri[i] : i;
+        c = dst.ci ? dst.ci[j] : j;
+    }
+    const bool live = r >= 0 && c >= 0;
+    double acc = 0.0;
+    if (live) {
+        const F *p = ws + ((int64_t)part * max_nb) * (TS * TS) + e;
+        for (int b = wave; b < max_nb; b += NW)
+            if ((owned[b >> 5] >> (b & 31)) & 1u) acc += (double)p[(int64_t)b * (TS * TS)];
+    }
+    red[wave][lane] = acc;
+    __syncthreads();
+    if (wave == 0 && live) {
+        const double s = (double)(F)finish_tree<NW>(red, lane);
+        out[r * dst.p + c] = (O)s;
+        if (i != j) out[c * dst.p + r] = (O)s;
+    }
+}
+
+template <typename F, typename O>
+inline int launch_finish_tiles(const F *ws, int max_nb, const int32_t *wg_tab, int n_wg, int64_t m, O *out,
+                               const FinishDst &dst, hipStream_t st) {
+    if (m == 0) return TM_OK;
+    const int64_t nchunk = ceil_div(m, 128);
+    const int n_parts = (int)(nchunk * (nchunk + 1) / 2);
+    dim3 grid(128 * 128 / 64, (unsigned)n_parts);
+    const size_t lds = sizeof(unsigned) * (size_t)((max_nb + 31) / 32);
+    const int4 *tab = reinterpret_cast<const int4 *>(wg_tab);
+    if (finish_small(grid.x, grid.y, max_nb))
+        hipLaunchKernelGGL((finish_tiles_kernel<F, O, 16>), grid, dim3(1024), lds, st, ws, max_nb, tab, n_wg, (int)m,
+                           out, dst);
+    else
+        hipLaunchKernelGGL((finish_tiles_kernel<F, O, 4>), grid, dim3(256), lds, st, ws, max_nb, tab, n_wg, (int)m,
+                           out, dst);
+    TM_LAUNCH_CHECK();
+    return TM_OK;
+}
+
+}
diff --git a/tabmat_amd/csrc/sparse_blocks.hip b/tabmat_amd/csrc/sparse_blocks.hip
--- a/tabmat_amd/csrc/sparse_blocks.hip
+++ b/tabmat_amd/csrc/sparse_blocks.hip
@@ -1,23 +1,12 @@
 #include <algorithm>
 
 #include "common.hpp"
-#include "reduce.hpp"
+#include "finish.hpp"
 
 namespace tmh {
 
 constexpr int KB_WAVES = 16;
 constexpr int KB_TS = 128;
-
-template <typename F>
-__global__ void blocks_assemble_kernel(const F *__restrict__ tiles, int n_out, F *__restrict__ out) {
-    const int j = blockIdx.x * blockDim.x + threadIdx.x;
-    const int i = blockIdx.y;
-    if (i >= n_out || j >= n_out) return;
-    const int hi = max(i, j), lo = min(i, j);
-    const int I = hi / KB_TS, J = lo / KB_TS;
-    const int part = I * (I + 1) / 2 + J;
-    out[(int64_t)i * n_out + j] = tiles[(int64_t)part * KB_TS * KB_TS + (hi % KB_TS) * KB_TS + (lo % KB_TS)];
-}
 
 constexpr int KB_FLAG_REP_A = 1 << 16;
 constexpr int KB_FLAG_REP_B = 1 << 17;
@@ -199,15 +188,14 @@
     }
 }
 
-template <typename F, bool U8 = false, bool D12 = false>
+template <typename F, bool U8 = false, bool D12 = false, typename O = F>
 static int run_sparse_sandwich_blocks(const F *data, const int32_t *ind, const int32_t *cptr, int64_t n,
                                       int64_t m, int64_t nnz, const int32_t *blocks, const int32_t *wg_tab,
-                                      int n_wg, int max_nb, const F *d, F *out, hipStream_t st) {
+                                      int n_wg, int max_nb, const F *d, O *out, const FinishDst &dst,
+                                      hipStream_t st) {
     if (m == 0) return TM_OK;
-    if (n == 0 || nnz == 0 || n_wg == 0) {
-        TM_HIP(hipMemsetAsync(out, 0, sizeof(F) * (size_t)(m * m), st));
-        return TM_OK;
-    }
+    if (n == 0 || nnz == 0 || n_wg == 0)
+        return launch_finish_tiles<F, O>(nullptr, 0, wg_tab, 0, m, out, dst, st);
     constexpr int TS = KB_TS;
     const int nchunk = (int)ceil_div(m, TS);
     const int n_parts = nchunk * (nchunk + 1) / 2;
@@ -215,14 +203,11 @@
     TM_REQUIRE(!D12 || n < (1ll << 24), "12-byte block descriptors hold 24 bits of row");
     TM_REQUIRE(max_nb >= 1 && n_wg >= 1, "empty workgroup table");
     const size_t lds = sizeof(lds_acc_t) * (size_t)(TS * TS);
-    const size_t tmp_bytes = (sizeof(F) * (size_t)n_parts * TS * TS + 255) / 256 * 256;
     const size_t ws_bytes = sizeof(F) * (size_t)n_parts * (size_t)max_nb * TS * TS;
     void *wsv = nullptr;
-    int rc = get_workspace(tmp_bytes + ws_bytes + 256, &wsv, st);
+    int rc = get_workspace(ws_bytes + 256, &wsv, st);
     if (rc) return rc;
-    F *tmp = reinterpret_cast<F *>(wsv);
-    F *ws = reinterpret_cast<F *>(reinterpret_cast<char *>(wsv) + tmp_bytes);
-    TM_HIP(hipMemsetAsync(ws, 0, ws_bytes, st));
+    F *ws = reinterpret_cast<F *>(wsv);
     auto kern = &sparse_sandwich_blocks_kernel<F, U8, D12>;
     TM_HIP(hipFuncSetAttribute(reinterpret_cast<const void *>(kern),
                                hipFuncAttributeMaxDynamicSharedMemorySize, (int)lds));
@@ -233,13 +218,7 @@
                        max_nb, ws, wg_log_ptr());
     prof_end(st);
     TM_LAUNCH_CHECK();
-    rc = launch_reduce_partials<F>(ws, (int64_t)TS * TS, max_nb, n_parts, tmp, (int64_t)n_parts * TS * TS,
-                                   false, st);
-    if (rc) return rc;
-    hipLaunchKernelGGL((blocks_assemble_kernel<F>), dim3((unsigned)ceil_div(m, 64), (unsigned)m), dim3(64),
-                       0, st, tmp, (int)m, out);
-    TM_LAUNCH_CHECK();
-    return TM_OK;
+    return launch_finish_tiles<F, O>(ws, max_nb, wg_tab, n_wg, m, out, dst, st);
 }
 
 }
@@ -251,14 +230,14 @@
                                   const int32_t *wg_tab, int n_wg, int max_nb, const float *d, float *out,
                                   void *stream) {
     return tmh::run_sparse_sandwich_blocks<float>(cm_data, cm_indices, cptr, n, m, nnz, blocks, wg_tab, n_wg,
-                                                  max_nb, d, out, tmh::as_stream(stream));
+                                                  max_nb, d, out, tmh::finish_plain(m), tmh::as_stream(stream));
 }
 int tm_sparse_sandwich_blocks_f64(const double *cm_data, const int32_t *cm_indices, const int32_t *cptr,
                                   int64_t n, int64_t m, int64_t nnz, const int32_t *blocks,
                                   const int32_t *wg_tab, int n_wg, int max_nb, const double *d, double *out,
                                   void *stream) {
     return tmh::run_sparse_sandwich_blocks<double>(cm_data, cm_indices, cptr, n, m, nnz, blocks, wg_tab, n_wg,
-                                                   max_nb, d, out, tmh::as_stream(stream));
+                                                   max_nb, d, out, tmh::finish_plain(m), tmh::as_stream(stream));
 }
 
 int tm_sparse_sandwich_blocks_u8_f32(const float *cm_data, const uint8_t *cm_col8, const int32_t *cptr,
@@ -267,7 +246,7 @@
                                      void *stream) {
     return tmh::run_sparse_sandwich_blocks<float, true>(cm_data, reinterpret_cast<const int32_t *>(cm_col8), cptr, n, m,
                                                         nnz, blocks, wg_tab, n_wg, max_nb, d, out,
-                                                        tmh::as_stream(stream));
+                                                        tmh::finish_plain(m), tmh::as_stream(stream));
 }
 int tm_sparse_sandwich_blocks_u8_f64(const double *cm_data, const uint8_t *cm_col8, const int32_t *cptr,
                                      int64_t n, int64_t m, int64_t nnz, const int32_t *blocks,
@@ -275,7 +254,7 @@
                                      void *stream) {
     return tmh::run_sparse_sandwich_blocks<double, true>(cm_data, reinterpret_cast<const int32_t *>(cm_col8), cptr, n, m,
                                                          nnz, blocks, wg_tab, n_wg, max_nb, d, out,
-                                                         tmh::as_stream(stream));
+                                                         tmh::finish_plain(m), tmh::as_stream(stream));
 }
 
 int tm_sparse_sandwich_blocks_p12_f32(const float *cm_data, const uint8_t *cm_col8, const int32_t *cptr,
@@ -284,7 +263,7 @@
                                       void *stream) {
     return tmh::run_sparse_sandwich_blocks<float, true, true>(cm_data, reinterpret_cast<const int32_t *>(cm_col8), cptr,
                                                               n, m, nnz, blocks12, wg_tab, n_wg, max_nb, d, out,
-                                                              tmh::as_stream(stream));
+                                                              tmh::finish_plain(m), tmh::as_stream(stream));
 }
 int tm_sparse_sandwich_blocks_p12_f64(const double *cm_data, const uint8_t *cm_col8, const int32_t *cptr,
                                       int64_t n, int64_t m, int64_t nnz, const int32_t *blocks12,
@@ -292,7 +271,25 @@
                                       void *stream) {
     return tmh::run_sparse_sandwich_blocks<double, true, true>(cm_data, reinterpret_cast<const int32_t *>(cm_col8), cptr,
                                                                n, m, nnz, blocks12, wg_tab, n_wg, max_nb, d, out,
-                                                               tmh::as_stream(stream));
-}
-
-}
+                                                               tmh::finish_plain(m), tmh::as_stream(stream));
+}
+
+
+int tm_sparse_sandwich_blocks_p12_into_f32(const float *cm_data, const uint8_t *cm_col8, const int32_t *cptr,
+                                           int64_t n, int64_t m, int64_t nnz, const int32_t *blocks12,
+                                           const int32_t *wg_tab, int n_wg, int max_nb, const float *d,
+                                           const int64_t *pos, double *out, int64_t p, void *stream) {
+    return tmh::run_sparse_sandwich_blocks<float, true, true, double>(
+        cm_data, reinterpret_cast<const int32_t *>(cm_col8), cptr, n, m, nnz, blocks12, wg_tab, n_wg, max_nb, d, out,
+        tmh::FinishDst{pos, pos, p, 1, 0}, tmh::as_stream(stream));
+}
+int tm_sparse_sandwich_blocks_p12_into_f64(const double *cm_data, const uint8_t *cm_col8, const int32_t *cptr,
+                                           int64_t n, int64_t m, int64_t nnz, const int32_t *blocks12,
+                                           const int32_t *wg_tab, int n_wg, int max_nb, const double *d,
+                                           const int64_t *pos, double *out, int64_t p, void *stream) {
+    return tmh::run_sparse_sandwich_blocks<double, true, true, double>(
+        cm_data, reinterpret_cast<const int32_t *>(cm_col8), cptr, n, m, nnz, blocks12, wg_tab, n_wg, max_nb, d, out,
+        tmh::FinishDst{pos, pos, p, 1, 0}, tmh::as_stream(stream));
+}
+
+}
diff --git a/tabmat_amd/csrc/sparse_ent.hip b/tabmat_amd/csrc/sparse_ent.hip
--- a/tabmat_amd/csrc/sparse_ent.hip
+++ b/tabmat_amd/csrc/sparse_ent.hip
@@ -1,5 +1,5 @@
 #include "common.hpp"
-#include "reduce.hpp"
+#include "finish.hpp"
 
 namespace tmh {
 
@@ -342,14 +342,6 @@
 }
 
 template <typename F>
-__global__ void en_untile_kernel(const F *__restrict__ tmp, int64_t m, int64_t nB, F *__restrict__ out) {
-    const int64_t e = (int64_t)blockIdx.x * blockDim.x + threadIdx.x;
-    if (e >= m * nB) return;
-    const int64_t i = e / nB, j = e % nB;
-    out[e] = tmp[((j / EN_W) * m + i) * EN_W + (j % EN_W)];
-}
-
-template <typename F>
 __global__ void en_csum_kernel(const F *__restrict__ part, int nblk, int64_t m, F *__restrict__ csum) {
     const int64_t c = (int64_t)blockIdx.x * blockDim.x + threadIdx.x;
     if (c >= m) return;
@@ -358,9 +350,10 @@
     csum[c] = (F)a;
 }
 
-template <typename F>
+template <typename F, typename O>
 static int run_csr_dense_ent(const F *vals, const uint16_t *meta, const uint32_t *bstart, int64_t n, int64_t m,
-                             const F *B, int64_t r, const F *d, F *out, F *colsum, hipStream_t st) {
+                             const F *B, int64_t r, const F *d, O *out, const FinishDst &dst, F *colsum,
+                             hipStream_t st) {
     const int64_t nB = r;
     const int64_t total = m * nB;
     if (total == 0) return TM_OK;
@@ -383,24 +376,21 @@
     const int nz = (int)ceil_div(n_groups, EN_NW);
     const bool want_csum = colsum != nullptr;
     if (n_slabs == 0) {
-        TM_HIP(hipMemsetAsync(out, 0, sizeof(F) * (size_t)total, st));
         if (want_csum) TM_HIP(hipMemsetAsync(colsum, 0, sizeof(F) * (size_t)m, st));
-        return TM_OK;
+        return launch_finish_coltiled<F, O>(nullptr, m * EN_W, 0, n_parts, EN_W, nB, out, dst, st);
     }
     int64_t nblk = std::max<int64_t>(1, tune("ent_rounds", 1) * NUM_CU / ((int64_t)n_parts * nz));
     nblk = std::min<int64_t>(nblk, n_slabs);
     const int64_t spb = ceil_div(n_slabs, nblk);
     nblk = ceil_div(n_slabs, spb);
     const int64_t stride = m * EN_W;
-    const size_t tmp_bytes = (sizeof(F) * (size_t)(n_parts * stride) + 255) / 256 * 256;
     const size_t part_bytes = (sizeof(F) * (size_t)((int64_t)n_parts * nblk * stride) + 255) / 256 * 256;
     const size_t csum_bytes = ((want_csum ? sizeof(F) * (size_t)(nblk * m) : 0) + 255) / 256 * 256 + 256;
     void *wsv = nullptr;
-    int rc = get_workspace(tmp_bytes + part_bytes + csum_bytes + 256, &wsv, st);
+    int rc = get_workspace(part_bytes + csum_bytes + 256, &wsv, st);
     if (rc) return rc;
-    F *tmp = reinterpret_cast<F *>(wsv);
-    F *ws = reinterpret_cast<F *>(reinterpret_cast<char *>(wsv) + tmp_bytes);
-    F *ws_csum = reinterpret_cast<F *>(reinterpret_cast<char *>(wsv) + tmp_bytes + part_bytes);
+    F *ws = reinterpret_cast<F *>(wsv);
+    F *ws_csum = reinterpret_cast<F *>(reinterpret_cast<char *>(wsv) + part_bytes);
     const size_t lds = (size_t)EnLds<F>::TOTAL;
     auto kern = want_csum ? &csr_dense_ent_kernel<F, true> : &csr_dense_ent_kernel<F, false>;
     TM_HIP(hipFuncSetAttribute(reinterpret_cast<const void *>(kern),
@@ -411,11 +401,8 @@
                        reinterpret_cast<long long *>((uintptr_t)tune("ent_prof", 0)));
     prof_end(st);
     TM_LAUNCH_CHECK();
-    rc = launch_reduce_partials<F>(ws, stride, (int)nblk, n_parts, tmp, n_parts * stride, false, st);
+    rc = launch_finish_coltiled<F, O>(ws, stride, (int)nblk, n_parts, EN_W, nB, out, dst, st);
     if (rc) return rc;
-    hipLaunchKernelGGL((en_untile_kernel<F>), dim3((unsigned)ceil_div(total, 256)), dim3(256), 0, st, tmp, m,
-                       nB, out);
-    TM_LAUNCH_CHECK();
     if (want_csum) {
         hipLaunchKernelGGL((en_csum_kernel<F>), dim3((unsigned)ceil_div(m, 256)), dim3(256), 0, st, ws_csum,
                            (int)nblk, m, colsum);
@@ -434,11 +421,29 @@
 int tm_csr_dense_sandwich_ent_f32(const float *vals, const uint16_t *meta, const uint32_t *bstart, int64_t n,
                                   int64_t m, const float *B, int64_t r, const float *d, float *out,
                                   float *colsum, void *stream) {
-    return tmh::run_csr_dense_ent<float>(vals, meta, bstart, n, m, B, r, d, out, colsum, tmh::as_stream(stream));
+    return tmh::run_csr_dense_ent<float, float>(vals, meta, bstart, n, m, B, r, d, out, tmh::finish_plain(r), colsum,
+                                                tmh::as_stream(stream));
 }
 int tm_csr_dense_sandwich_ent_f64(const double *vals, const uint16_t *meta, const uint32_t *bstart, int64_t n,
                                   int64_t m, const double *B, int64_t r, const double *d, double *out,
                                   double *colsum, void *stream) {
-    return tmh::run_csr_dense_ent<double>(vals, meta, bstart, n, m, B, r, d, out, colsum, tmh::as_stream(stream));
-}
-}
+    return tmh::run_csr_dense_ent<double, double>(vals, meta, bstart, n, m, B, r, d, out, tmh::finish_plain(r), colsum,
+                                                  tmh::as_stream(stream));
+}
+int tm_csr_dense_sandwich_ent_into_f32(const float *vals, const uint16_t *meta, const uint32_t *bstart, int64_t n,
+                                       int64_t m, const float *B, int64_t r, const float *d, const int64_t *ri,
+                                       const int64_t *ci, double *out, int64_t p, int mirror, int transpose,
+                                       float *colsum, void *stream) {
+    return tmh::run_csr_dense_ent<float, double>(vals, meta, bstart, n, m, B, r, d, out,
+                                                 tmh::FinishDst{ri, ci, p, mirror, transpose}, colsum,
+                                                 tmh::as_stream(stream));
+}
+int tm_csr_dense_sandwich_ent_into_f64(const double *vals, const uint16_t *meta, const uint32_t *bstart, int64_t n,
+                                       int64_t m, const double *B, int64_t r, const double *d, const int64_t *ri,
+                                       const int64_t *ci, double *out, int64_t p, int mirror, int transpose,
+                                       double *colsum, void *stream) {
+    return tmh::run_csr_dense_ent<double, double>(vals, meta, bstart, n, m, B, r, d, out,
+                                                  tmh::FinishDst{ri, ci, p, mirror, transpose}, colsum,
+                                                  tmh::as_stream(stream));
+}
+}
diff --git a/tabmat_amd/ext/_types.py b/tabmat_amd/ext/_types.py
--- a/tabmat_amd/ext/_types.py
+++ b/tabmat_amd/ext/_types.py
@@ -710,6 +710,11 @@
     def n_slots(self) -> int:
         return int(self.vals.numel()) - SlabEnt.SLACK
 
+    def kernel_pos(self, pos: torch.Tensor) -> torch.Tensor:
+        kp = torch.full((self.mk,), -1, dtype=torch.int64, device=self.inv.device)
+        kp[self.inv] = pos.to(torch.int64)
+        return kp
+
     @staticmethod
     def from_csr(csr: CsrDev, max_pad: float = None) -> "SlabEnt":
         from .._lib import lib
diff --git a/tabmat_amd/ext/sparse.py b/tabmat_amd/ext/sparse.py
--- a/tabmat_amd/ext/sparse.py
+++ b/tabmat_amd/ext/sparse.py
@@ -161,6 +161,14 @@
     return (out[A.inv], cs[A.inv]) if want_colsum else out[A.inv]
 
 
+def csr_dense_sandwich_ent_into(A: SlabEnt, B: DenseDev, d, ri, ci, out, mirror=True, transpose=False):
+    assert B.n == A.n and ell_supported(B) and A.m > 0 and B.m > 0 and A.n > 0
+    D.same_float("csr_dense_sandwich_ent_into", A.vals, B.buf, d)
+    call("tm_csr_dense_sandwich_ent_into_" + D.fsuf(A.vals), D.p(A.vals), D.p(A.meta), D.p(A.bstart), A.n, A.mk,
+         D.p(B.buf), B.m, D.p(d), D.p(ri), D.p(ci), D.p(out), out.shape[0], int(mirror), int(transpose), None,
+         D.stream_ptr())
+
+
 def _row_table(A: CsrDev, rows, d, as_set: bool):
     import weakref
 
@@ -263,6 +271,22 @@
          int(cm_data.numel()), D.p(blocks), D.p(wg_tab), int(wg_tab.shape[0]), int(max_nb), D.p(d),
          D.p(out), D.stream_ptr())
     return out
+
+
+def sparse_sandwich_blocks_into_ok(A: CsrDev) -> bool:
+    if not K2B_U8 or A.m == 0 or A.n == 0:
+        return False
+    return int(A.pair_blocks(d12=None)[0].shape[1]) == 3
+
+
+def sparse_sandwich_blocks_into(A: CsrDev, d, pos, out):
+    D.same_float("sparse_sandwich_blocks_into", A.data, d)
+    cm_data, cm_c8, cptr = A.chunk_major()
+    blocks, wg_tab, max_nb = A.pair_blocks(d12=None)
+    assert int(blocks.shape[1]) == 3
+    call(f"tm_sparse_sandwich_blocks_p12_into_{D.fsuf(A.data)}", D.p(cm_data), D.p(cm_c8), D.p(cptr), A.n, A.m,
+         int(cm_data.numel()), D.p(blocks), D.p(wg_tab), int(wg_tab.shape[0]), int(max_nb), D.p(d), D.p(pos),
+         D.p(out), out.shape[0], D.stream_ptr())
 
 
 def sparse_sandwich_pairs(A: CsrDev, d):
diff --git a/tabmat_amd/ext/split.py b/tabmat_amd/ext/split.py
--- a/tabmat_amd/ext/split.py
+++ b/tabmat_amd/ext/split.py
@@ -368,6 +368,14 @@
     return res
 
 
+def multi_cat_dense_sandwich_into(cats, d, mat_j: DenseDev, ri, ci, out):
+    codes, ncols, drop, n = _cat_args(cats)
+    D.same_float("multi_cat_dense_sandwich_into", mat_j.buf, d)
+    call(f"tm_multi_cat_dense_sandwich_into_{D.fsuf(mat_j.buf)}", codes, ncols, drop, n, mat_j.n,
+         D.p(d), D.p(mat_j.buf), mat_j.m, mat_j.order_f, D.p(ri), D.p(ci), D.p(out), out.shape[0], 1, 0,
+         D.stream_ptr())
+
+
 def multi_cat_sparse_sandwich(cats, d, S: SlabCsc):
     total = sum(int(c[1]) for c in cats)
     if total == 0 or S.m == 0 or S.n == 0:
@@ -412,6 +420,14 @@
     return res[:, E.inv]
 
 
+def multi_cat_sparse_sandwich_ent_into(cats, d, E, packed, ri, ci, out):
+    codes, ncols, drop, n = _cat_args(cats)
+    D.same_float("multi_cat_sparse_sandwich_ent_into", E.vals, d)
+    call(f"tm_multi_cat_sparse_sandwich_ent_into_{D.fsuf(E.vals)}", codes, ncols, drop, n, E.n, D.p(d),
+         D.p(E.vals), D.p(E.meta), D.p(E.bstart), E.n_slots(), E.mk, D.p(packed), D.p(ri), D.p(ci), D.p(out),
+         out.shape[0], 1, 0, D.stream_ptr())
+
+
 def multi_cat_sparse_sandwich_rows(cats, d, A, rows):
     from . import sparse as xs
 
diff --git a/tabmat_amd/sparse_matrix.py b/tabmat_amd/sparse_matrix.py
--- a/tabmat_amd/sparse_matrix.py
+++ b/tabmat_amd/sparse_matrix.py
@@ -334,6 +334,37 @@
                 res = res[c64][:, c64].contiguous()
             return res
         return xs.sparse_sandwich(A, d, rows, cols)
+
+    def _sandwich_into_ok(self) -> bool:
+        from . import categorical_matrix as _cm
+
+        if self._row_parts() is not None or _cm.DETERMINISTIC or self.shape[0] == 0 or self.shape[1] == 0:
+            return False
+        A = self._dev()
+        if getattr(self, "_direct_pays", None) is None:
+            self._direct_pays = xs.direct_sandwich_pays(A)
+        if getattr(self, "_pairs_pay", None) is None:
+            self._pairs_pay = xs.pairs_sandwich_pays(A)
+        if self._pairs_pay or self._direct_pays:
+            return False
+        if not (0 < A.data.numel() < 2**31 and self.shape[1] <= 128 * 32):
+            return False
+        if getattr(self, "_blocks_pay", None) is None:
+            self._blocks_pay = xs.blocks_sandwich_pays(A)
+        return bool(self._blocks_pay) and xs.sparse_sandwich_blocks_into_ok(A)
+
+    def _cross_dense_ent(self, other):
+        if other.dtype != self.dtype or self.shape[0] == 0 or self.shape[1] == 0 or other.shape[1] == 0:
+            return None
+        A, Bd = self._dev(), other._dev_c()
+        if A.data.numel() == 0:
+            return None
+        if (A.data.numel() <= SORTED_K3_NNZ_PER_ROW * self.shape[0] and self.shape[1] >= 1024
+                and xs.ell_supported(Bd)):
+            return None
+        if not (Bd.m > 64 and xs.ell_supported(Bd)):
+            return None
+        return self._ent()
 
     def _ent_det(self):
         ent = self._ent()
diff --git a/tabmat_amd/split_matrix.py b/tabmat_amd/split_matrix.py
--- a/tabmat_amd/split_matrix.py
+++ b/tabmat_amd/split_matrix.py
@@ -32,6 +32,7 @@
 ROW_LIST_FRACTION_CATSPARSE = 0.04
 DIAG_FROM_PAIRS = True
 CAT_PAIRS_FUSED = os.environ.get("TABMAT_AMD_CAT_PAIRS", "1") != "0"
+SANDWICH_INTO = os.environ.get("TABMAT_AMD_SANDWICH_INTO", "1") != "0"
 FULL_THEN_SELECT = float(os.environ.get("TABMAT_AMD_FULL_THEN_SELECT", "0.5"))
 FULL_RESULT_MAX_BYTES = 256 << 20
 FULL_UNSELECTED_SHARE = 0.2
@@ -435,6 +436,46 @@
             return xsplit.multi_cat_sparse_sandwich(cats, d_eff, mw._slab())
         return None
 
+    def _group_pos_dev(self, grp, pos_d):
+        cache = self.__dict__.setdefault("_group_pos", {})
+        gpos = cache.get(tuple(grp))
+        if gpos is None:
+            gpos = cache[tuple(grp)] = torch.cat([pos_d[i] for i in grp])
+        return gpos
+
+    def _ent_pos(self, w, ent, pos):
+        cache = self.__dict__.setdefault("_ent_pos_cache", {})
+        hit = cache.get(w)
+        if hit is None or hit[0] is not ent or hit[1] is not pos:
+            hit = cache[w] = (ent, pos, ent.kernel_pos(pos))
+        return hit[2]
+
+    def _fused_cats_into(self, mw, cats, cat_ids, d, total, budget, gpos, w, pos_w, out) -> bool:
+        if total == 0 or mw.shape[0] == 0 or mw.shape[1] == 0:
+            return False
+        if isinstance(mw, DenseMatrix):
+            Bd = mw._dev_c()
+            if xsplit.multi_cat_dense_wide_ok(cats, Bd) or xsplit.multi_cat_dense_tile_ok(cats, Bd):
+                xsplit.multi_cat_dense_sandwich_into(cats, d, Bd, gpos, pos_w, out)
+                return True
+            return False
+        if isinstance(mw, SparseMatrix) and total * 33 <= budget and mw._dev().data.numel() > 0:
+            ent = None
+            if len(cats) <= 8 and (getattr(mw, "_entblk", None) or any(
+                    isinstance(mo, DenseMatrix) and mo.shape[1] > 64 and mo.dtype == mw.dtype
+                    for mo in self.matrices)):
+                ent = mw._ent()
+            if ent is None:
+                return False
+            pk_cache = self.__dict__.setdefault("_packed_codes", {})
+            key = tuple(cat_ids)
+            if key not in pk_cache:
+                pk_cache[key] = xsplit.pack_codes(cats)
+            xsplit.multi_cat_sparse_sandwich_ent_into(cats, d, ent, pk_cache[key], gpos,
+                                                      self._ent_pos(w, ent, pos_w), out)
+            return True
+        return False
+
     def _parts(self):
         parts = self.__dict__.get("_row_parts", False)
         if parts is False:
@@ -663,8 +704,11 @@
 
     def _sandwich_terms(self, d, rows, cols_host, colsum, out, pos_d, sub_d, empty, done, center=None, xtv=None):
         from .ext import dense as xd
+        from .ext import sparse as xs
 
         mats = self.matrices
+        plain = (SANDWICH_INTO and rows is None and cols_host is None and colsum is None and center is None
+                 and xtv is None and d.dtype == D.torch_dtype(self.dtype))
         cat_ids = [i for i, m in enumerate(mats) if isinstance(m, CategoricalMatrix) and not empty[i]
                    and m.shape[1] > 0]
         budget = (128 * 1024) // 8
@@ -678,16 +722,17 @@
             for w, mw in enumerate(mats):
                 if empty[w] or mw.dtype != self.dtype or d.dtype != D.torch_dtype(self.dtype):
                     continue
+                if plain and self._fused_cats_into(mw, cats, grp, d_eff, total, budget,
+                                                   self._group_pos_dev(grp, pos_d), w, pos_d[w], out):
+                    done.update((min(i, w), max(i, w)) for i in grp)
+                    continue
                 stacked = self._fused_cats(mw, cats, grp, d_eff, rows, total, budget, d)
                 if stacked is None:
                     continue
                 whole = cols_host is None and len(grp) > 1
                 if whole:
-                    cache = self.__dict__.setdefault("_group_pos", {})
-                    gpos = cache.get(tuple(grp))
-                    if gpos is None:
-                        gpos = cache[tuple(grp)] = torch.cat([pos_d[i] for i in grp])
-                    xsplit.scatter_block(stacked.contiguous(), gpos, pos_d[w], out, mirror=True)
+                    xsplit.scatter_block(stacked.contiguous(), self._group_pos_dev(grp, pos_d), pos_d[w], out,
+                                         mirror=True)
                 for ci, i in enumerate(grp):
                     res = stacked[int(offs[ci]):int(offs[ci + 1])]
                     if (colsum is not None and colsum[w] is None and not mats[i].drop_first
@@ -777,6 +822,8 @@
             elif isinstance(mi, DenseMatrix) and center is not None and center.get(i) is not None:
                 res = mi._sandwich_dev(d, rows, sub_d[i], center=center.get(i))
                 xsplit.scatter_block(res, pos_d[i], pos_d[i], out)
+            elif plain and isinstance(mi, SparseMatrix) and mi.dtype == self.dtype and mi._sandwich_into_ok():
+                xs.sparse_sandwich_blocks_into(mi._dev(), d, pos_d[i], out)
             else:
                 res = mi._sandwich_dev(d, rows, sub_d[i])
                 xsplit.scatter_block(res, pos_d[i], pos_d[i], out)
@@ -787,6 +834,11 @@
                 if empty[j] or (i, j) in done:
                     continue
                 si, di = (i, j) if isinstance(mi, SparseMatrix) else (j, i)
+                if (plain and isinstance(mats[si], SparseMatrix) and isinstance(mats[di], DenseMatrix)
+                        and (ent := mats[si]._cross_dense_ent(mats[di])) is not None):
+                    xs.csr_dense_sandwich_ent_into(ent, mats[di]._dev_c(), d, self._ent_pos(si, ent, pos_d[si]),
+                                                   pos_d[di], out)
+                    continue
                 if (colsum is not None and colsum[si] is None and isinstance(mats[si], SparseMatrix)
                         and isinstance(mats[di], DenseMatrix)):
                     box = []
```

After: 1029 GB/s. About the same (-0.2%).
